# Chain123/RecGURU

Hardware: AMD Instinct MI355X
Metric: user-sequences/sec (AE+GAN step) (higher is better)
Workload: dtype bf16; 1 GPU; cross-domain RecGURU AE+GAN phase-2 iteration (5 critic + 1 generator update), two 100000-item domains; per_gpu_batch=4096, seq_len=200, d_model=128, n_head=4, n_blocks=3, d_ff=512, n_negs=30, user_lengths=U{5..220}, parallelism=dp1

## Files before the change

### include/recguru_hip.h

```cpp
#ifndef RECGURU_HIP_H
#define RECGURU_HIP_H
#include <stddef.h>
#include <stdint.h>
#ifdef __cplusplus
extern "C" {
#endif

#define RG_F32 0
#define RG_BF16 1
#define RG_X3 2

#define RG_ERR_INVALID (-1)
#define RG_ERR_UNSUPPORTED (-2)
#define RG_ERR_HIP (-3)

const char* rg_last_error(void);
int rg_version(void);

int rg_det_enabled(void);
int rg_det_set_arenas(void* fbase0, void* sbase0, unsigned long long bytes0, int bits0,
                      void* fbase1, void* sbase1, unsigned long long bytes1, int bits1);
int rg_det_fault(int clear);

#define RG_PRO_NONE 0
#define RG_PRO_GELU 1

#define RG_EPI_NONE 0
#define RG_EPI_RELU 1
#define RG_EPI_MUL_POSMASK 2
#define RG_EPI_GELU_GRAD 3
#define RG_EPI_ADD 4
#define RG_EPI_RESID_LN 5
#define RG_EPI_DROP_GELU 6

typedef struct {
  const void* A; int lda;
  const void* W; int ldw;
  const float* bias;
  void* C; int ldc;
  int c_is_f32;
  int M, N, K;
  int prologue, epilogue;
  const void* aux; int ldaux;
  const float* gamma; const float* beta; const float* rowmask; float* rstd_out; float ln_eps;
  int debug_ablate;
  float epi_scale;
  float epi_nonzero_scale;
  float drop_p; unsigned long long drop_seed;
  const int* live16;
  int skip_dead_fill;
  int c_hm_L;
  void* C2;
  int w_packed;
} rg_gemm_nt_args;
int rg_gemm_nt(const rg_gemm_nt_args* args , int dtype, void* stream);

typedef struct {
  const void* Y; int ldy;
  const void* X; int ldx;
  float* dW; int lddw;
  float* colsum;
  int T, N1, N2;
  int prologue_x;
  float scale;
  int splits;
  int use_tr;
  const int* live16;
  float* partials;
  int colsum_T;
} rg_gemm_tn_args;
int rg_gemm_tn(const rg_gemm_tn_args* args , int dtype, void* stream);
size_t rg_gemm_tn_workspace(const rg_gemm_tn_args* args , int dtype);
int rg_gemm_tn_layer_supported(const rg_gemm_tn_args* p , const int* wgs , int dtype);
size_t rg_gemm_tn_layer_workspace(int slot, int wgs);
int rg_gemm_tn_layer(const rg_gemm_tn_args* p , const int* wgs , int dtype, void* stream);
int rg_gemm_nt_plan(const rg_gemm_nt_args* args , int dtype, char* name, int cap);
int rg_gemm_tn_plan(const rg_gemm_tn_args* args , int dtype, char* name, int cap);


typedef struct {
  const void* qkv;
  const int64_t* key_ids; int64_t pad_value; int causal;
  void* ctx; float* lse;
  int B, L, H, dk;
  float scale;
  float drop_p; unsigned long long seed;
  const float* rowmask;
  const void* x; const void* wqkv; const float* bqkv; int d;
  int x_masked;
  const int* first_live;
  int qkv_hm;
  const void* pad_rows;
} rg_attn_args;
int rg_attn_fwd(const rg_attn_args* args , int dtype, void* stream);
int rg_attn_fwd_x_supported(int d, int dtype, float drop_p);

typedef struct {
  const void* qkv; const void* dctx; const void* ctx; const float* lse;
  const int64_t* key_ids; int64_t pad_value; int causal;
  void* dqkv;
  int B, L, H, dk;
  float scale;
  float drop_p; unsigned long long seed;
  const float* rowmask;
  const float* bqkv; int x_masked;
  const int* first_live;
  int qkv_hm;
} rg_attn_bwd_args;
int rg_attn_bwd(const rg_attn_bwd_args* args , int dtype, void* stream);

int rg_embed_pe_fwd(const void* table, const float* pe, const int64_t* ids, const float* mask, void* out,
                    long long ntok, int L, int d, float drop_p, unsigned long long seed, int dtype, void* stream);
int rg_embed_pe_fwd_rows(const void* table, long long table_rows, const float* pe, const int64_t* ids, const float* mask, void* out,
                         long long ntok, int L, int d, float drop_p, unsigned long long seed, int dtype, void* stream);
int rg_embed_pe_fwd2(const void* table, const float* pe, const int64_t* ids, const float* mask, void* out, void* out2,
                     long long ntok, int L, int d, float drop_p, unsigned long long seed, int dtype, void* stream);
int rg_embed_pe_fwd_split(const float* table_f32, const float* pe, const int64_t* ids, const float* mask, void* out,
                          void* out_lo, long long ntok, int L, int d, float drop_p, unsigned long long seed, void* stream);
int rg_embed_scatter_bwd(const void* dx, const int64_t* ids, const float* mask, float* dE, long long ntok, int d,
                         long long skip_row, float drop_p, unsigned long long seed, int dtype, void* stream);
size_t rg_embed_scatter_binned_workspace(long long ntok, int d, long long table_rows);
int rg_embed_scatter_bwd_binned(const void* dx, const int64_t* ids, const float* mask, float* dE, long long ntok, int d,
                                long long table_rows, long long skip_row, float drop_p, unsigned long long seed,
                                void* workspace, size_t workspace_bytes, int dtype, void* stream);

typedef struct {
  const void* dy; const void* y; const float* rstd; const float* gamma; const float* beta;
  const float* rowmask;
  void* dz; float* dgamma; float* dbeta;
  long long M; int N; int ld;
  void* dz_drop; float drop_p; unsigned long long drop_seed;
  const int* live16;
  float* dz_colsum;
  float* partials;
} rg_ln_bwd_args;
int rg_ln_bwd(const rg_ln_bwd_args* args , int dtype, void* stream);
size_t rg_ln_bwd_workspace(long long M, int N);

int rg_bcast_add_ln(const void* x, const float* o, const float* gamma, const float* beta, void* y, float* rstd,
                    long long M, int L, int N, float eps, int dtype, void* stream);
int rg_seq_sum(const void* x, void* out , int B, int L, int N, int dtype, void* stream);
int rg_pad_mask(const int64_t* ids, int64_t pad, float* out, long long n, void* stream);
int rg_last_rows(const void* x, const float* rowmask, void* x_last, float* m_last, int B, int L, int d, int dtype, void* stream);

int rg_colsum(const void* x, const void* aux , const float* coef , float* out,
              long long M, int N, int ld, float scale, int dtype,
              void* stream);
int rg_outer_posmask(const float* coef , const float* w , const void* aux, void* out,
                     long long M, int N, float scale, int dtype,
                     void* stream);
typedef struct {
  const void* real; const void* fake;
  const float* alpha;
  const void *W1, *W2, *W3, *W1t, *W2t, *W3t;
  const float *b1, *b2, *b3, *w4, *b4;
  int B, d, n1, n2, n3;
  float drop_p;
  unsigned long long seed_w[3];
  unsigned long long seed_g[3];
  float coef_real, coef_fake;
  float gp_coef;
  float* out;
  float* scalars;
  void *Y1, *X1, *Y2, *X2, *Y3, *X3;
  float *db1, *db2, *db3, *dw4, *db4;
  void* dx;
  void* hscratch;
  int need_wgrad;
  int debug_ablate;
  long long* stamps;
} rg_disc_args;
int rg_disc_supported(int d, int n1, int n2, int n3, int dtype);
int rg_disc_rows(const rg_disc_args* args , int dtype, void* stream);
int rg_interpolate(const float* alpha, const void* real, const void* fake, void* out, long long B, int d,
                   int dtype, void* stream);
int rg_gp_penalty(const float* g, void* dg, float* gp, long long B, int d, float lambda, int dtype,
                  void* stream);
int rg_sum(const float* x, float* out, long long n, float scale, void* stream);

int rg_adam(float* p, const float* g, float* m, float* v, void* shadow, int shadow_dtype, long long n, float lr,
            float beta1, float beta2, float eps, int step, void* stream);
typedef struct {
  float* p; const float* g; float* m; float* v;
  long long n;
  float step_lr; float inv_bc2_sqrt;
} rg_adam_seg;
int rg_adam_multi(const rg_adam_seg* segs , int nsegs, float beta1, float beta2, float eps, void* stream);
typedef struct {
  float* p; const float* g; float* m; float* v;
  long long n;
  long long step;
} rg_adam_seg_dev;
int rg_adam_multi_dev(rg_adam_seg_dev* segs , int nsegs, double lr, double beta1, double beta2,
                      double eps, void* stream);
#define RG_CAST_TRANSPOSE 1
#define RG_CAST_PACK 2
#define RG_CAST_SPLIT 4
int rg_cast(const float* src, void* dst, int R, int C, int transpose, int dtype, void* stream);
typedef struct {
  const float* src; void* dst;
  int R, C, ld, row_off, col_off, transpose;
} rg_cast_seg;
int rg_cast_multi(const rg_cast_seg* segs , const int* tiles , int ntiles,
                  int dtype, void* stream);

#define RG_LOSS_SAMPLED_CE 0
#define RG_LOSS_BPR 1
#define RG_LOSS_BPR_SAS 2
typedef struct {
  const void* h;
  const void* table;
  const int64_t* pos;
  const int64_t* neg;
  const float* mask;
  float* aux_tok;
  float* sums;
  const float* gout;
  void* dh; float* dE;
  long long ntok; int d; int k; int mode; long long skip_row;
} rg_item_loss_args;
int rg_item_loss_fwd(const rg_item_loss_args* args , int dtype, void* stream);
int rg_item_loss_bwd(const rg_item_loss_args* args , int dtype, void* stream);
size_t rg_item_loss_bwd_binned_workspace(long long ntok, int k, int d, long long table_rows);
int rg_item_loss_bwd_binned(const rg_item_loss_args* args , long long table_rows, void* workspace,
                            size_t workspace_bytes, int dtype, void* stream);
int rg_item_loss_train_supported(int k, int d);
int rg_item_loss_train(const rg_item_loss_args* args , float* coef, int dtype, void* stream);
int rg_item_loss_scatter_binned(const rg_item_loss_args* args , const float* coef, long long table_rows,
// ... 135 lines not shown
```

### recguru_amd/csrc/fused.hip

```cpp
#include <type_traits>
#include "rg_common.hip.h"
#include "rg_det.hip.h"
#include "../../include/recguru_hip.h"

#define FT_M 64
#include <stdlib.h>
#define FD 128
#define FPAD 8
#define FLD (FD + FPAD)

template <typename T> struct Tile {
  static constexpr int LD = sizeof(T) == 2 ? FD : FLD;
  static __device__ __forceinline__ int off(int row, int col) {
    if constexpr (sizeof(T) == 2) return row * FD + ((((col >> 3) ^ row) & 15) << 3) + (col & 7);
    else return row * FLD + col;
  }
};
template <> struct Tile<x3r> {
  static constexpr int LD = FD;
  static __device__ __forceinline__ int off(int row, int col) { return row * FD + ((((col >> 3) ^ row) & 15) << 3) + (col & 7); }
};

template <typename T> struct WSet { typename OpT<T>::type f[4][2]; };

// ... 637 lines not shown
#pragma unroll
    for (int ct = 0; ct < 2; ++ct)
#pragma unroll
      for (int rt = 0; rt < RT; ++rt)
#pragma unroll
        for (int r = 0; r < 4; ++r) acc2[ct][rt][r] *= rm4[rt];
    regs_to_tile<XT>(acc2, Aout, n0, li, lg);
    if constexpr (RES) regs_to_tile_lo<LT>(acc2, Ag, n0, li, lg);
    STAMP(9);
    lds_barrier();
    tile_to_hbm<T>(Aout, out, FD, 0, mb, a.M, tid);
    if constexpr (RES) tile_to_hbm<T>(Ag, outlo, FD, 0, mb, a.M, tid);
    lds_barrier();
    STAMP(10);
#pragma unroll
    for (int rt = 0; rt < RT; ++rt) mb[rt] = mbn[rt];
    have = have_next;
  }
  if (a.live16) {
    const int nrt = (a.M + 15) >> 4, ndead = nrt - a.live16[0];
    constexpr bool cross = CROSS;
    for (int j = RT * (int)blockIdx.x; j < ndead; j += RT * (int)gridDim.x) {
      int md[RT];
#pragma unroll
      for (int rt = 0; rt < RT; ++rt) md[rt] = j + rt < ndead ? a.live16[nrt - (j + rt)] * 16 : a.M;
      zero_to_hbm<T>(out, FD, 0, md, a.M, tid);
      if constexpr (RES) zero_to_hbm<T>(outlo, FD, 0, md, a.M, tid);
      if (a.skip_dead_saves) continue;
      if (ysave) zero_to_hbm<T>(ysave, FD, 0, md, a.M, tid);
      if (cross && y2save) zero_to_hbm<T>(y2save, FD, 0, md, a.M, tid);
      if (h1save)
        for (int ch = 0; ch < nchunk; ++ch) zero_to_hbm<T>(h1save, a.dff, ch * FD, md, a.M, tid);
      if (tid < FTM) {
        const int m = md[tid >> 4] + (tid & 15);
        if (m < a.M) {
          if (rstd1o) rstd1o[m] = 0.f;
          if (rstd2o) rstd2o[m] = 0.f;
          if (rstdco) rstdco[m] = 0.f;
        }
      }
    }
  }
#ifdef RG_STAMP
  if (a.rstd_c == nullptr && a.o_bcast == nullptr && a.y2_save != nullptr && (tid & 63) == 0) {
    unsigned long long* dbg = reinterpret_cast<unsigned long long*>(a.y2_save) + (size_t)(blockIdx.x * 4 + wave) * 12;
    for (int i = 0; i < 12; ++i) dbg[i] = tacc[i];
  }
#endif
}

static int act_tile_bytes(int dtype, int rows) {
  return dtype == RG_BF16 ? rows * FD * 2 : (dtype == RG_X3 ? rows * FD * 2 * 2 : rows * FLD * 4);
}

int rg_post_attn_fwd256(const rg_post_attn_args* a, int dtype, hipStream_t s);
int rg_post_attn_fwd_w8_try(const rg_post_attn_args* a, int dtype, hipStream_t s, int* rc);

extern "C" int rg_post_attn_fwd(const rg_post_attn_args* a, int dtype, void* stream) {
  if (!a || a->M <= 0) return 0;
  if (a->d == 256) return rg_post_attn_fwd256(a, dtype, (hipStream_t)stream);
  {
    int rc8 = 0;
    if (rg_post_attn_fwd_w8_try(a, dtype, (hipStream_t)stream, &rc8)) return rc8;
  }
  if (a->d != FD || a->P != FD || (a->dff % FD) != 0 || a->dff <= 0)
    return rg_set_error_msg(RG_ERR_UNSUPPORTED, "post_attn_fwd: needs d_model == n_heads*32 == 128 and d_ff % 128 == 0");
  if ((long long)a->M * a->dff * (dtype == RG_BF16 ? 2 : 4) >= (1ll << 32))
    return rg_set_error_msg(RG_ERR_UNSUPPORTED, "post_attn_fwd: M * d_ff * element size must be below 4 GiB (32-bit offsets)");
  if ((a->o_bcast || a->cross_s) && a->L <= 0) return rg_set_error_msg(RG_ERR_INVALID, "post_attn_fwd: cross stage needs L");
  if (a->cross_s && (!a->cross_oh || !a->cross_bo || a->H != 4)) return rg_set_error_msg(RG_ERR_INVALID, "post_attn_fwd: cross_s needs cross_oh, cross_bo, H == P / 32 == 4");
  hipStream_t s = (hipStream_t)stream;
  static const int x3_rt = [] { const char* e = getenv("RG_X3_PA_RT"); return (e && atoi(e) == 4) ? 4 : 2; }();
#ifdef RG_PA_RT2
  static const int rt_env = [] { const char* e = getenv("RG_PA_RT"); return e ? atoi(e) : 0; }();
  const int rt = dtype == RG_X3 ? x3_rt : (dtype != RG_BF16 ? 4 : (rt_env == 2 ? 2 : 4));
#else
  const int rt = dtype == RG_X3 ? x3_rt : 4;
#endif
  const int ftm = 16 * rt;
  const int ntiles = (a->M + ftm - 1) / ftm;
  const int act = act_tile_bytes(dtype, ftm);
  const int smem = 3 * act + (8 * FD + a->dff) * 4 + 2 * ftm * 4 * 4 + 64 * 4 + (a->h1_save ? act : 0);
  const int per_cu = (160 * 1024) / smem;
  const int cap_cu = dtype == RG_X3 ? 2 : 3;
  int grid = 256 * (per_cu < 1 ? 1 : (per_cu > cap_cu ? cap_cu : per_cu));
  if (grid > ntiles) grid = ntiles;
  const int dm = a->drop_p <= 0.f ? 0 : (a->drop_p == 0.5f ? 1 : 2);
  const bool cross = a->o_bcast || a->cross_s;
  const bool save = a->y_save || a->y2_save || a->h1_save || a->rstd1 || a->rstd2 || a->rstd_c;
  const bool res = a->x_lo || a->out_lo;
  if (res && (!a->x_lo || !a->out_lo || dtype != RG_BF16))
    return rg_set_error_msg(RG_ERR_INVALID, "post_attn_fwd: the split residual stream needs x_lo AND out_lo, bf16 tier");
  static const int pipe_on = [] { const char* e = getenv("RG_PA_PIPE"); return e ? atoi(e) : 0; }();
  if (pipe_on && dtype == RG_BF16 && !cross && !save && !res && a->dff >= 2 * FD) {
#define RG_PAP(DM)                                                                                                        \
  do {                                                                                                                    \
    hipFuncSetAttribute(reinterpret_cast<const void*>(post_attn_fwd_kernel<__bf16, DM, false, false, false, 4, true>), hipFuncAttributeMaxDynamicSharedMemorySize, smem); \
    hipLaunchKernelGGL((post_attn_fwd_kernel<__bf16, DM, false, false, false, 4, true>), dim3(grid), dim3(256), smem, s, *a); \
  } while (0)
    if (dm == 0) RG_PAP(0);
    else if (dm == 1) RG_PAP(1);
    else RG_PAP(2);
#undef RG_PAP
    RG_CHECK_LAUNCH();
    return 0;
  }
#define RG_PA4(T, DM, C, S, R, RTV)                                                                                       \
  do {                                                                                                                    \
    hipFuncSetAttribute(reinterpret_cast<const void*>(post_attn_fwd_kernel<T, DM, C, S, R, RTV>), hipFuncAttributeMaxDynamicSharedMemorySize, smem); \
    hipLaunchKernelGGL((post_attn_fwd_kernel<T, DM, C, S, R, RTV>), dim3(grid), dim3(256), smem, s, *a);                  \
  } while (0)
#ifdef RG_PA_RT2
#define RG_PA3(T, DM, C, S, R)                                                              \
  do {                                                                                      \
    if constexpr (sizeof(T) == 2 || std::is_same<T, x3>::value) { if (rt == 2) RG_PA4(T, DM, C, S, R, 2); else RG_PA4(T, DM, C, S, R, 4); } \
    else RG_PA4(T, DM, C, S, R, 4);                                                         \
  } while (0)
#else
#define RG_PA3(T, DM, C, S, R)                                                              \
  do {                                                                                      \
    if constexpr (std::is_same<T, x3>::value) { if (rt == 2) RG_PA4(T, DM, C, S, R, 2); else RG_PA4(T, DM, C, S, R, 4); } \
    else RG_PA4(T, DM, C, S, R, 4);                                                         \
  } while (0)
#endif
#define RG_PA2(T, DM, C, S)                                                                       \
  do {                                                                                            \
    if constexpr (sizeof(T) == 2) { if (res) RG_PA3(T, DM, C, S, true); else RG_PA3(T, DM, C, S, false); } \
    else RG_PA3(T, DM, C, S, false);                                                              \
  } while (0)
#define RG_PA(T, DM)                                  \
  do {                                                \
    if (cross) { if (save) RG_PA2(T, DM, true, true); else RG_PA2(T, DM, true, false); }      \
    else { if (save) RG_PA2(T, DM, false, true); else RG_PA2(T, DM, false, false); }          \
  } while (0)
#define RG_PA_T(T)                   \
  do {                               \
    if (dm == 0) RG_PA(T, 0);        \
    else if (dm == 1) RG_PA(T, 1);   \
    else RG_PA(T, 2);                \
  } while (0)
  if (dtype == RG_BF16) RG_PA_T(__bf16);
  else if (dtype == RG_F32) RG_PA_T(float);
  else if (dtype == RG_X3) RG_PA_T(x3);
  else return rg_set_error_msg(RG_ERR_INVALID, "post_attn_fwd: bad dtype");
#undef RG_PA_T
#undef RG_PA
#undef RG_PA2
#undef RG_PA3
#undef RG_PA4
  RG_CHECK_LAUNCH();
  return 0;
}

template <typename T, bool LNF>
__global__ __launch_bounds__(256, (sizeof(T) == 2 ? 2 : 1)) void ffn_bwd_data_kernel(rg_ffn_bwd_args a) {
  constexpr int PL = FT_M * FD * 2;
  typedef typename LdsT<T, PL>::type LT;
  constexpr int ACT_BYTES = FT_M * Tile<LT>::LD * (int)sizeof(LT) * LdsT<T, PL>::PLANES;
  extern __shared__ __align__(16) unsigned char smem[];
  LT* Adl = reinterpret_cast<LT*>(smem);
  typedef typename ResT<T, PL>::type XT;
  XT* Adz = reinterpret_cast<XT*>(smem + ACT_BYTES);
  LT* Adh = reinterpret_cast<LT*>(smem + 2 * ACT_BYTES);
  XT* Ah = reinterpret_cast<XT*>(smem + 3 * ACT_BYTES);
  XT* Ady = reinterpret_cast<XT*>(smem);
  const int tid = threadIdx.x, lane = tid & 63, wave = __builtin_amdgcn_readfirstlane(tid >> 6);
  const int li = lane & 15, lg = lane >> 4;
  const T* __restrict__ dl2 = reinterpret_cast<const T*>(LNF ? a.ln_dout : a.dl2);
  const T* __restrict__ dz = reinterpret_cast<const T*>(LNF ? a.ln_out : a.dz);
  T* __restrict__ dl2o = reinterpret_cast<T*>(a.dl2_out);
  const T* __restrict__ h1 = reinterpret_cast<const T*>(a.h1);
  const T* __restrict__ W2t = reinterpret_cast<const T*>(a.W2t);
  const T* __restrict__ W1t = reinterpret_cast<const T*>(a.W1t);
  T* __restrict__ dh1 = reinterpret_cast<T*>(a.dh1);
  T* __restrict__ dy = reinterpret_cast<T*>(a.dy);
  const int n0 = wave * 32;
  const int ntiles = (a.M + FT_M - 1) / FT_M;
  const int nchunk = a.dff / FD;
  const float nz = a.nz_scale;

  WSet<T> wp, wq;
  Frag<T> cpre[4], xpre[4], hpre[4];
  float rs_pre[4], rm_pre[4];
  float dg[8], db[8];
  const DropCfg ldrop = make_drop(a.ln_drop_p, a.ln_drop_seed);
  float* lnp = reinterpret_cast<float*>(smem + 4 * ACT_BYTES);
  if constexpr (LNF) {
#pragma unroll
    for (int j = 0; j < 8; ++j) { dg[j] = 0.f; db[j] = 0.f; }
    for (int i = tid; i < FD; i += 256) { lnp[i] = a.ln_gamma[i]; lnp[FD + i] = a.ln_beta[i]; lnp[2 * FD + i] = 1.f / a.ln_gamma[i]; }
  }

  LiveWalk lw;
  lw.init(a.live16, a.M);
  const int nwork = a.live16 ? (lw.nlive + 3) >> 2 : ntiles;
  int cur = (int)blockIdx.x, kcur = 0;
  auto next_group = [&](int (&g)[4]) -> bool {
    if (cur >= nwork) {
#pragma unroll
      for (int rt = 0; rt < 4; ++rt) g[rt] = a.M;
      return false;
    }
    if (!a.live16) {
#pragma unroll
      for (int rt = 0; rt < 4; ++rt) g[rt] = cur * FT_M + 16 * rt;
    } else {
      lw.group(kcur, g, a.M);
    }
    cur += gridDim.x;
    ++kcur;
    return true;
  };
  auto prefetch_h = [&](const int (&g)[4], int ch) {
#pragma unroll
    for (int i = 0; i < 4; ++i) {
      const int c8 = (tid & 15) * 8, m = min(g[i] + (tid >> 4), a.M - 1);
      load_frag(hpre[i], gofs(h1, (unsigned int)m * (unsigned int)a.dff + (unsigned int)(ch * FD + c8)));
    }
  };
  auto prefetch_rows = [&](const int (&g)[4]) {
#pragma unroll
    for (int i = 0; i < 4; ++i) {
      const int c8 = (tid & 15) * 8, m = min(g[i] + (tid >> 4), a.M - 1);
      load_frag(cpre[i], gofs(dl2, (unsigned int)(m * FD + c8)));
      load_frag(xpre[i], gofs(dz, (unsigned int)(m * FD + c8)));
      if constexpr (LNF) {
        const float* __restrict__ rmp = a.ln_rowmask ? a.ln_rowmask : a.ln_rstd;
        const float rv = rmp[m];
        rs_pre[i] = a.ln_rstd[m];
        rm_pre[i] = a.ln_rowmask ? rv : 1.f;
      }
    }
  };
  auto h_to_lds = [&]() {
#pragma unroll
    for (int i = 0; i < 4; ++i) {
      const int c = tid + 256 * i, r = c >> 4, c8 = (c & 15) * 8;
      stage8(Ah + Tile<XT>::off(r, c8), hpre[i]);
    }
  };
  int mb[4], mbn[4];
  bool have = next_group(mb);
  if (have) {
    load_wset(wp, W2t, FD, n0, 0, li, lg, a.w_packed);
    prefetch_rows(mb);
    prefetch_h(mb, 0);
  }
  for (; have;) {
    const bool have_next = next_group(mbn);
    if constexpr (LNF) {
      const int c8 = (tid & 15) * 8;
      float gam[8], bet[8], igam[8];
      load8(gam, lnp + c8);
      load8(bet, lnp + FD + c8);
      load8(igam, lnp + 2 * FD + c8);
#pragma unroll
      for (int i = 0; i < 4; ++i) {
        const int r = 16 * i + (tid >> 4), m = mb[i] + (tid >> 4);
        const bool live = m < a.M;
        const float rm = live ? rm_pre[i] : 0.f;
        float g[8], xh[8], s1 = 0.f, s2 = 0.f;
        if (rm != 0.f) {
          const float irm = 1.f / rm;
#pragma unroll
          for (int j = 0; j < 8; ++j) {
            const float d = (float)cpre[i].v[j] * rm;
            xh[j] = ((float)xpre[i].v[j] * irm - bet[j]) * igam[j];
            g[j] = d * gam[j];
            dg[j] += d * xh[j];
            db[j] += d;
            s1 += g[j];
            s2 += g[j] * xh[j];
          }
        } else {
#pragma unroll
          for (int j = 0; j < 8; ++j) { g[j] = 0.f; xh[j] = 0.f; }
        }
#pragma unroll
        for (int o = 1; o < 16; o <<= 1) { s1 += __shfl_xor(s1, o); s2 += __shfl_xor(s2, o); }
        const float rstd = rm != 0.f ? rs_pre[i] : 0.f;
        s1 *= 1.f / FD;
        s2 *= 1.f / FD;
        float o8[8];
#pragma unroll
        for (int j = 0; j < 8; ++j) o8[j] = rstd * (g[j] - s1 - xh[j] * s2);
        store8(Adz + Tile<XT>::off(r, c8), o8);
        if (ldrop.thresh != 0u || ldrop.onebit) {
          float k8[8];
          rg_keep8(ldrop, (unsigned int)m * (unsigned int)FD + (unsigned int)c8, k8);
#pragma unroll
          for (int j = 0; j < 8; ++j) o8[j] *= k8[j];
        }
        store8(Adl + Tile<LT>::off(r, c8), o8);
        if (live) store8(gofs(dl2o, (unsigned int)(m * FD + c8)), o8);
      }
    } else {
#pragma unroll
      for (int i = 0; i < 4; ++i) {
        const int c = tid + 256 * i, r = c >> 4, c8 = (c & 15) * 8;
        stage8(Adl + Tile<LT>::off(r, c8), cpre[i]);
        stage8(Adz + Tile<XT>::off(r, c8), xpre[i]);
      }
    }
    h_to_lds();
    lds_barrier();
    f32x4 acc[2][4], acc2[2][4];
#pragma unroll
    for (int ct = 0; ct < 2; ++ct)
#pragma unroll
      for (int rt = 0; rt < 4; ++rt) acc2[ct][rt] = (f32x4){0.f, 0.f, 0.f, 0.f};
#pragma unroll 1
    for (int ch = 0; ch < nchunk; ++ch) {
      load_wset(wq, W1t, a.dff, n0, ch * FD, li, lg, a.w_packed);
      {
        const bool last = ch + 1 == nchunk;
        int gs[4];
#pragma unroll
        for (int rt = 0; rt < 4; ++rt) gs[rt] = last ? mbn[rt] : mb[rt];
        prefetch_h(gs, last ? 0 : ch + 1);
      }
#pragma unroll
      for (int ct = 0; ct < 2; ++ct)
#pragma unroll
        for (int rt = 0; rt < 4; ++rt) acc[ct][rt] = (f32x4){0.f, 0.f, 0.f, 0.f};
      mma_wset<T>(acc, wp, Adl, li, lg);
      load_wset(wp, W2t + (unsigned int)((ch + 1 < nchunk) ? ch + 1 : 0) * (FD * FD), FD, n0, 0, li, lg, a.w_packed);
      if (ch > 0) lds_barrier();
#pragma unroll
      for (int ct = 0; ct < 2; ++ct)
#pragma unroll
        for (int rt = 0; rt < 4; ++rt) {
          float x4[4];
          load4t(x4, Ah + Tile<XT>::off(rt * 16 + li, n0 + ct * 16 + 4 * lg));
#pragma unroll
          for (int r = 0; r < 4; ++r) {
            float v = acc[ct][rt][r] * gelu_grad_t<Precise<T>::value>(x4[r]);
            if (nz > 0.f) v = x4[r] != 0.f ? v * nz : 0.f;
            acc[ct][rt][r] = v;
          }
        }
      regs_to_tile<LT>(acc, Adh, n0, li, lg);
      lds_barrier();
      if (ch + 1 < nchunk) h_to_lds();
      tile_to_hbm<T>(Adh, dh1, a.dff, ch * FD, mb, a.M, tid);
      mma_wset<T>(acc2, wq, Adh, li, lg);
    }
    prefetch_rows(mbn);
#pragma unroll
    for (int ct = 0; ct < 2; ++ct)
#pragma unroll
      for (int rt = 0; rt < 4; ++rt) {
        float r4[4];
        load4t(r4, Adz + Tile<XT>::off(rt * 16 + li, n0 + ct * 16 + 4 * lg));
#pragma unroll
        for (int r = 0; r < 4; ++r) acc2[ct][rt][r] += r4[r];
      }
    regs_to_tile<XT>(acc2, Ady, n0, li, lg);
    lds_barrier();
    tile_to_hbm<T>(Ady, dy, FD, 0, mb, a.M, tid);
    lds_barrier();
#pragma unroll
    for (int rt = 0; rt < 4; ++rt) mb[rt] = mbn[rt];
    have = have_next;
  }
  if (a.live16) {
    const int nrt = (a.M + 15) >> 4, ndead = nrt - a.live16[0];
    for (int j = 4 * (int)blockIdx.x; j < ndead; j += 4 * (int)gridDim.x) {
      int md[4];
#pragma unroll
      for (int rt = 0; rt < 4; ++rt) md[rt] = j + rt < ndead ? a.live16[nrt - (j + rt)] * 16 : a.M;
      zero_to_hbm<T>(dy, FD, 0, md, a.M, tid);
    }
  }
  if constexpr (LNF) {
#pragma unroll
    for (int o = 16; o < 64; o <<= 1)
#pragma unroll
      for (int j = 0; j < 8; ++j) { dg[j] += __shfl_xor(dg[j], o); db[j] += __shfl_xor(db[j], o); }
    float* red = reinterpret_cast<float*>(smem);
    __syncthreads();
    if (lane < 16) {
#pragma unroll
      for (int j = 0; j < 8; ++j) { red[(0 * 4 + wave) * FD + lane * 8 + j] = dg[j]; red[(1 * 4 + wave) * FD + lane * 8 + j] = db[j]; }
    }
    __syncthreads();
    const int w = tid >> 7, n = tid & 127;
    a.ln_partials[((size_t)blockIdx.x * 2 + w) * FD + n] = (red[(w * 4 + 0) * FD + n] + red[(w * 4 + 1) * FD + n]) + (red[(w * 4 + 2) * FD + n] + red[(w * 4 + 3) * FD + n]);
  }
}

__global__ __launch_bounds__(256) void ffn_bwd_ln_reduce_kernel(const float* __restrict__ partials, int nblocks,
                                                                float* __restrict__ dgamma, float* __restrict__ dbeta) {
  const int c = threadIdx.x;
  float* dst = c < FD ? dgamma : dbeta;
  if (!dst) return;
  float s0 = 0.f, s1 = 0.f;
  int b = blockIdx.x;
  for (; b + (int)gridDim.x < nblocks; b += 2 * gridDim.x) {
    s0 += partials[(size_t)b * 2 * FD + c];
    s1 += partials[(size_t)(b + gridDim.x) * 2 * FD + c];
  }
  if (b < nblocks) s0 += partials[(size_t)b * 2 * FD + c];
  rg_acc(dst + (c & (FD - 1)), s0 + s1);
}

extern "C" int rg_ffn_bwd_data_supported(int d, int dff) { return d == FD && dff > 0 && (dff % FD) == 0; }

static int ffn_bwd_grid(int M, int dtype) {
  const int ntiles = (M + FT_M - 1) / FT_M;
  const int smem = 4 * act_tile_bytes(dtype, FT_M);
  const int per_cu = (160 * 1024) / smem;
  const int grid = 256 * (per_cu < 1 ? 1 : (per_cu > 2 ? 2 : per_cu));
  return grid > ntiles ? ntiles : grid;
}
extern "C" size_t rg_ffn_bwd_ln_workspace(int M) { return (size_t)(M <= 0 ? 0 : 512) * 2 * FD * sizeof(float); }

extern "C" int rg_ffn_bwd_data(const rg_ffn_bwd_args* a, int dtype, void* stream) {
  if (!a || a->M <= 0) return 0;
  if (!rg_ffn_bwd_data_supported(a->d, a->dff))
    return rg_set_error_msg(RG_ERR_UNSUPPORTED, "ffn_bwd_data: needs d_model == 128 and d_ff % 128 == 0");
  if ((long long)a->M * a->dff * (dtype == RG_BF16 ? 2 : 4) >= (1ll << 32))
    return rg_set_error_msg(RG_ERR_UNSUPPORTED, "ffn_bwd_data: M * d_ff * element size must be below 4 GiB (32-bit offsets)");
  const bool lnf = a->ln_dout != nullptr;
  if ((!lnf && (!a->dl2 || !a->dz)) || !a->h1 || !a->W2t || !a->W1t || !a->dh1 || !a->dy)
    return rg_set_error_msg(RG_ERR_INVALID, "ffn_bwd_data: NULL operand");
  if (lnf && (!a->ln_out || !a->ln_rstd || !a->ln_gamma || !a->ln_beta || !a->dl2_out || !a->ln_partials))
    return rg_set_error_msg(RG_ERR_INVALID, "ffn_bwd_data: the fused LayerNorm backward needs ln_out, ln_rstd, ln_gamma, ln_beta, dl2_out, ln_partials");
  hipStream_t s = (hipStream_t)stream;
  const int ntiles = (a->M + FT_M - 1) / FT_M;
  const int smem = 4 * act_tile_bytes(dtype, FT_M) + (lnf ? 3 * FD * 4 : 0);
  const int grid = ffn_bwd_grid(a->M, dtype);
#define RG_FB(T, L)                                                                                                       \
  do {                                                                                                                    \
    hipFuncSetAttribute(reinterpret_cast<const void*>(ffn_bwd_data_kernel<T, L>), hipFuncAttributeMaxDynamicSharedMemorySize, smem); \
    hipLaunchKernelGGL((ffn_bwd_data_kernel<T, L>), dim3(grid), dim3(256), smem, s, *a);                                  \
  } while (0)
  if (dtype == RG_BF16) { if (lnf) RG_FB(__bf16, true); else RG_FB(__bf16, false); }
  else if (dtype == RG_F32) { if (lnf) RG_FB(float, true); else RG_FB(float, false); }
  else if (dtype == RG_X3) { if (lnf) RG_FB(x3, true); else RG_FB(x3, false); }
  else return rg_set_error_msg(RG_ERR_INVALID, "ffn_bwd_data: bad dtype");
#undef RG_FB
  if (lnf && (a->ln_dgamma || a->ln_dbeta))
    hipLaunchKernelGGL(ffn_bwd_ln_reduce_kernel, dim3(grid < 32 ? grid : 32), dim3(256), 0, s, a->ln_partials, grid, a->ln_dgamma, a->ln_dbeta);
  RG_CHECK_LAUNCH();
  return 0;
}

template <typename T>
__global__ __launch_bounds__(256, 2) void attn_out_bwd_kernel(rg_attn_out_bwd_args a) {
  constexpr int PL = FT_M * FD * 2;
  typedef typename LdsT<T, PL>::type LT;
  constexpr int ACT_BYTES = FT_M * Tile<LT>::LD * (int)sizeof(LT) * LdsT<T, PL>::PLANES;
  extern __shared__ __align__(16) unsigned char smem[];
  LT* Adz = reinterpret_cast<LT*>(smem);
  typedef typename ResT<T, PL>::type XT;
  XT* Aout = reinterpret_cast<XT*>(smem + ACT_BYTES);
  float* lnp = reinterpret_cast<float*>(smem + 2 * ACT_BYTES);
  const int tid = threadIdx.x, lane = tid & 63, wave = __builtin_amdgcn_readfirstlane(tid >> 6);
  const int li = lane & 15, lg = lane >> 4;
  const T* __restrict__ dy = reinterpret_cast<const T*>(a.dy);
  const T* __restrict__ y = reinterpret_cast<const T*>(a.y);
  T* __restrict__ dz = reinterpret_cast<T*>(a.dz);
  T* __restrict__ dctx = reinterpret_cast<T*>(a.dctx);
  const int n0 = wave * 32;
  const int ntiles = (a.M + FT_M - 1) / FT_M;
  for (int i = tid; i < FD; i += 256) { lnp[i] = a.gamma[i]; lnp[FD + i] = a.beta[i]; lnp[2 * FD + i] = 1.f / a.gamma[i]; }
  WSet<T> w;
  load_wset(w, reinterpret_cast<const T*>(a.Wot), FD, n0, 0, li, lg, a.w_packed);
  Frag<T> cpre[4], xpre[4];
  float rs_pre[4], rm_pre[4];
  float dg[8], db[8];
#pragma unroll
  for (int j = 0; j < 8; ++j) { dg[j] = 0.f; db[j] = 0.f; }
  LiveWalk lw;
  lw.init(a.live16, a.M);
  const int nwork = a.live16 ? (lw.nlive + 3) >> 2 : ntiles;
  int cur = (int)blockIdx.x, kcur = 0;
  auto next_group = [&](int (&g)[4]) -> bool {
    if (cur >= nwork) {
#pragma unroll
      for (int rt = 0; rt < 4; ++rt) g[rt] = a.M;
      return false;
    }
    if (!a.live16) {
#pragma unroll
      for (int rt = 0; rt < 4; ++rt) g[rt] = cur * FT_M + 16 * rt;
    } else {
      lw.group(kcur, g, a.M);
    }
    cur += gridDim.x;
    ++kcur;
    return true;
  };
  auto prefetch_rows = [&](const int (&g)[4]) {
    const float* __restrict__ rmp = a.rowmask ? a.rowmask : a.rstd;
#pragma unroll
    for (int i = 0; i < 4; ++i) {
      const int c8 = (tid & 15) * 8, m = min(g[i] + (tid >> 4), a.M - 1);
      load_frag(cpre[i], gofs(dy, (unsigned int)(m * FD + c8)));
      load_frag(xpre[i], gofs(y, (unsigned int)(m * FD + c8)));
      const float rv = rmp[m];
      rs_pre[i] = a.rstd[m];
      rm_pre[i] = a.rowmask ? rv : 1.f;
    }
  };
  int mb[4], mbn[4];
  bool have = next_group(mb);
  if (have) prefetch_rows(mb);
  __syncthreads();
  for (; have;) {
    const bool have_next = next_group(mbn);
    {
      const int c8 = (tid & 15) * 8;
      float gam[8], bet[8], igam[8];
      load8(gam, lnp + c8);
      load8(bet, lnp + FD + c8);
      load8(igam, lnp + 2 * FD + c8);
#pragma unroll
      for (int i = 0; i < 4; ++i) {
        const int r = 16 * i + (tid >> 4), m = mb[i] + (tid >> 4);
        const bool live = m < a.M;
        const float rm = live ? rm_pre[i] : 0.f;
        float g[8], xh[8], s1 = 0.f, s2 = 0.f;
        if (rm != 0.f) {
          const float irm = 1.f / rm;
#pragma unroll
          for (int j = 0; j < 8; ++j) {
            const float d = (float)cpre[i].v[j] * rm;
            xh[j] = ((float)xpre[i].v[j] * irm - bet[j]) * igam[j];
            g[j] = d * gam[j];
            dg[j] += d * xh[j];
            db[j] += d;
            s1 += g[j];
            s2 += g[j] * xh[j];
          }
        } else {
#pragma unroll
          for (int j = 0; j < 8; ++j) { g[j] = 0.f; xh[j] = 0.f; }
        }
#pragma unroll
        for (int o = 1; o < 16; o <<= 1) { s1 += __shfl_xor(s1, o); s2 += __shfl_xor(s2, o); }
        const float rstd = rm != 0.f ? rs_pre[i] : 0.f;
        s1 *= 1.f / FD;
        s2 *= 1.f / FD;
        float o8[8];
#pragma unroll
        for (int j = 0; j < 8; ++j) o8[j] = rstd * (g[j] - s1 - xh[j] * s2);
        store8(Adz + Tile<LT>::off(r, c8), o8);
        if (live) store8(gofs(dz, (unsigned int)(m * FD + c8)), o8);
      }
    }
    prefetch_rows(mbn);
    lds_barrier();
    f32x4 acc[2][4];
#pragma unroll
    for (int ct = 0; ct < 2; ++ct)
#pragma unroll
      for (int rt = 0; rt < 4; ++rt) acc[ct][rt] = (f32x4){0.f, 0.f, 0.f, 0.f};
    mma_wset<T>(acc, w, Adz, li, lg);
    regs_to_tile<XT>(acc, Aout, n0, li, lg);
    lds_barrier();
    tile_to_hbm<T>(Aout, dctx, FD, 0, mb, a.M, tid);
#pragma unroll
    for (int rt = 0; rt < 4; ++rt) mb[rt] = mbn[rt];
    have = have_next;
  }
#pragma unroll
  for (int o = 16; o < 64; o <<= 1)
#pragma unroll
    for (int j = 0; j < 8; ++j) { dg[j] += __shfl_xor(dg[j], o); db[j] += __shfl_xor(db[j], o); }
  float* red = reinterpret_cast<float*>(smem);
  __syncthreads();
  if (lane < 16) {
#pragma unroll
    for (int j = 0; j < 8; ++j) { red[(0 * 4 + wave) * FD + lane * 8 + j] = dg[j]; red[(1 * 4 + wave) * FD + lane * 8 + j] = db[j]; }
  }
  __syncthreads();
  const int wsel = tid >> 7, n = tid & 127;
  a.ln_partials[((size_t)blockIdx.x * 2 + wsel) * FD + n] = (red[(wsel * 4 + 0) * FD + n] + red[(wsel * 4 + 1) * FD + n]) + (red[(wsel * 4 + 2) * FD + n] + red[(wsel * 4 + 3) * FD + n]);
}

static int attn_out_bwd_grid(int M) {
  const int ntiles = (M + FT_M - 1) / FT_M;
  return ntiles < 512 ? ntiles : 512;
}
extern "C" size_t rg_attn_out_bwd_workspace(int M) { return (size_t)(M <= 0 ? 0 : 1024) * 2 * FD * sizeof(float); }

extern "C" int rg_attn_out_bwd(const rg_attn_out_bwd_args* a, int dtype, void* stream) {
  if (!a || a->M <= 0) return 0;
  if (a->d != FD || a->P != FD) return rg_set_error_msg(RG_ERR_UNSUPPORTED, "attn_out_bwd: needs d_model == n_heads*32 == 128");
// ... 22 lines not shown
```

### recguru_amd/csrc/gemm_tn_big.hip

```cpp
#include <cstdlib>
#include <type_traits>
#include "rg_common.hip.h"
#include "rg_det.hip.h"
#include "../../include/recguru_hip.h"

#define TB_T_BF16 64
#define TB_T_X3 32

__device__ __forceinline__ void frag_tr16(Frag<__bf16>& f, const __bf16* tile, int ld, int c0, int li, int lg) {
  typedef __attribute__((ext_vector_type(4))) short s16x4;
  typedef __attribute__((address_space(3))) s16x4 lds_s16x4;
  const int q = li >> 2, p = li & 3;
  const __bf16* p0 = tile + (8 * lg + q) * ld + c0 + 4 * p;
  const __bf16* p1 = p0 + 4 * ld;
  union { s16x4 s; bf16x4_t b; } u0, u1;
  u0.s = __builtin_amdgcn_ds_read_tr16_b64_v4i16((lds_s16x4*)p0);
  u1.s = __builtin_amdgcn_ds_read_tr16_b64_v4i16((lds_s16x4*)p1);
#pragma unroll
  for (int j = 0; j < 4; ++j) { f.v[j] = u0.b[j]; f.v[4 + j] = u1.b[j]; }
}

__device__ __forceinline__ void frag_tr_op(Frag<__bf16>& f, const __bf16* tile, int ld, int c0, int li, int lg, int lo_ofs) {
  frag_tr16(f, tile, ld, c0, li, lg);
}
// ... 232 lines not shown
    __syncthreads();
  }
  auto bases = [&](int chunk, int (&bb)[EPC]) {
    if (a.live16) {
      const unsigned int ad = (unsigned int)(size_t)(lst + EPC * (chunk - c_beg));
      if constexpr (EPC == 2) {
        long long v;
        asm volatile("ds_read_b64 %0, %1\n\ts_waitcnt lgkmcnt(0)" : "=v"(v) : "v"(ad) : "memory");
        bb[0] = (int)(v & 0xFFFFFFFFll);
        bb[1] = (int)(v >> 32);
      } else {
        typedef __attribute__((ext_vector_type(4))) int i32x4;
        i32x4 v;
        asm volatile("ds_read_b128 %0, %1\n\ts_waitcnt lgkmcnt(0)" : "=v"(v) : "v"(ad) : "memory");
#pragma unroll
        for (int e = 0; e < EPC; ++e) bb[e] = v[e];
      }
    } else {
#pragma unroll
      for (int e = 0; e < EPC; ++e) bb[e] = chunk * CT + 16 * e;
    }
  };
  auto issue = [&](int chunk) {
    int bb[EPC];
    bases(chunk, bb);
    unsigned char* stage = smem_td + (chunk % NST) * STG;
#pragma unroll
    for (int k = 0; k < NPER; ++k) {
      const bool isy = k < KY;
      const unsigned int ld2 = (unsigned int)(isy ? a.ldy : a.ldx) * 2u;
      int bsel = bb[0];
#pragma unroll
      for (int e = 1; e < EPC; ++e) bsel = (srow[k] >> 4) == e ? bb[e] : bsel;
      const int row = min(bsel + (srow[k] & 15), a.T - 1);
      const char* src = (isy ? Y : X) + (size_t)(unsigned int)row * ld2 + scb[k];
      __builtin_amdgcn_global_load_lds((const __attribute__((address_space(1))) void*)src,
                                       (__attribute__((address_space(3))) void*)(stage + (isy ? 0 : C::YB) + (wave + 8 * (isy ? k : k - KY)) * 1024),
                                       16, 0, 0);
    }
  };

  f32x4 acc[MT][NT];
  f32x4 cs[MT];
#pragma unroll
  for (int i = 0; i < MT; ++i) {
    cs[i] = (f32x4){0.f, 0.f, 0.f, 0.f};
#pragma unroll
    for (int j = 0; j < NT; ++j) acc[i][j] = (f32x4){0.f, 0.f, 0.f, 0.f};
  }
  Frag<T> ones;
  frag_fill(ones, 1.f);
  const int q = li >> 2, pp = li & 3;
  const unsigned int smem0 = (unsigned int)(size_t)smem_td;
  const unsigned int ly0 = (unsigned int)((8 * lg + q) * (2 * N1) + ((pp >> 1) << 4) + (pp & 1) * 8);
  const unsigned int lx0 = (unsigned int)((8 * lg + q) * (2 * N2) + ((pp >> 1) << 4) + (pp & 1) * 8) + (unsigned int)C::YB;
  typedef long long i64;
  auto rd_y = [&](i64& lo, i64& hi, unsigned int stage_ofs, int ti) {
    const unsigned int ad = smem0 + stage_ofs + ly0 + (((unsigned int)ti ^ (unsigned int)q) << 5);
    asm volatile("ds_read_b64_tr_b16 %0, %2\n\tds_read_b64_tr_b16 %1, %2 offset:%3" : "=&v"(lo), "=&v"(hi) : "v"(ad), "n"(8 * N1) : "memory");
  };
  auto rd_x = [&](i64& lo, i64& hi, unsigned int stage_ofs, int ti) {
    const unsigned int ad = smem0 + stage_ofs + lx0 + (((unsigned int)ti ^ (unsigned int)q) << 5);
    asm volatile("ds_read_b64_tr_b16 %0, %2\n\tds_read_b64_tr_b16 %1, %2 offset:%3" : "=&v"(lo), "=&v"(hi) : "v"(ad), "n"(8 * N2) : "memory");
  };
  auto to_frag = [&](Frag<T>& f, i64 lo, i64 hi, bool gelu) {
    union { i64 l; bf16x4_t b; } u0, u1;
    u0.l = lo; u1.l = hi;
#pragma unroll
    for (int j = 0; j < 4; ++j) {
      f.v[j] = gelu ? (T)gelu_t<false>((float)u0.b[j]) : u0.b[j];
      f.v[4 + j] = gelu ? (T)gelu_t<false>((float)u1.b[j]) : u1.b[j];
    }
  };

#pragma unroll 1
  for (int c = c_beg; c < c_end && c < c_beg + NST - 1; ++c) issue(c);
#pragma unroll 1
  for (int chunk = c_beg; chunk < c_end; ++chunk) {
    wait_chunks<NPER, NST - 2>(min(NST - 2, c_end - 1 - chunk));
    lds_barrier();
    if (chunk + NST - 1 < c_end) issue(chunk + NST - 1);
    unsigned char* stage = smem_td + (chunk % NST) * STG;
    if (chunk == nchunks - 1) {
      int bb[EPC];
      bases(chunk, bb);
      bool partial = false;
#pragma unroll
      for (int e = 0; e < EPC; ++e) { bb[e] = __builtin_amdgcn_readfirstlane(bb[e]); partial = partial || bb[e] + 16 > a.T; }
      if (partial) {
        for (int i = tid; i < CT * N1 / 8; i += 512) {
          const int r = i / (N1 / 8);
          int bsel = bb[0];
#pragma unroll
          for (int e = 1; e < EPC; ++e) bsel = (r >> 4) == e ? bb[e] : bsel;
          const int row = bsel + (r & 15);
          if (row >= a.T) *reinterpret_cast<uint4*>(stage + i * 16) = make_uint4(0u, 0u, 0u, 0u);
        }
        lds_barrier();
      }
    }
    const unsigned int sofs0 = (unsigned int)((chunk % NST) * STG);
#pragma unroll
    for (int ks = 0; ks < KS; ++ks) {
    i64 ya[MT][2], xb[NT][2];
#pragma unroll
    for (int i = 0; i < MT; ++i) rd_y(ya[i][0], ya[i][1], sofs0 + ks * 32 * 2 * N1, (m1 >> 4) + i);
    rd_x(xb[0][0], xb[0][1], sofs0 + ks * 32 * 2 * N2, m2 >> 4);
    Frag<T> af[MT];
#pragma unroll
    for (int j = 0; j < NT; ++j) {
      if (j + 1 < NT) {
        rd_x(xb[j + 1][0], xb[j + 1][1], sofs0 + ks * 32 * 2 * N2, (m2 >> 4) + j + 1);
        asm volatile("s_waitcnt lgkmcnt(2)" : "+v"(xb[j][0]), "+v"(xb[j][1]));
      } else {
        asm volatile("s_waitcnt lgkmcnt(0)" : "+v"(xb[j][0]), "+v"(xb[j][1]));
      }
      if (j == 0) {
#pragma unroll
        for (int i = 0; i < MT; ++i) {
          asm volatile("" : "+v"(ya[i][0]), "+v"(ya[i][1]));
          to_frag(af[i], ya[i][0], ya[i][1], false);
          if (do_cs) mma(af[i], ones, cs[i]);
        }
      }
      Frag<T> bf;
      to_frag(bf, xb[j][0], xb[j][1], GELU_X);
#pragma unroll
      for (int i = 0; i < MT; ++i) mma(af[i], bf, acc[i][j]);
    }
    }
  }
  float* __restrict__ part = a.partials ? a.partials + (size_t)bid * (N1 * N2) + tid : nullptr;
#pragma unroll
  for (int i = 0; i < MT; ++i) {
#pragma unroll
    for (int j = 0; j < NT; ++j)
#pragma unroll
      for (int r = 0; r < 4; ++r) {
        if (part) part[((i * NT + j) * 4 + r) * 512] = acc[i][j][r];
        else rg_acc(a.dW + (size_t)(m1 + i * 16 + 4 * lg + r) * a.lddw + m2 + j * 16 + li, acc[i][j][r] * a.scale);
      }
    if (do_cs && li == 0) {
#pragma unroll
      for (int r = 0; r < 4; ++r) rg_acc(a.colsum + m1 + i * 16 + 4 * lg + r, cs[i][r] * a.scale);
    }
  }
}

template <int N1, int N2, bool GELU_X>
__global__ __launch_bounds__(512) void gemm_tn_dma_kernel(rg_gemm_tn_args a) {
  tn_dma_body<N1, N2, GELU_X>(a, (int)blockIdx.x, (int)gridDim.x);
}

struct rg_tn_layer_args {
  rg_gemm_tn_args p[4];
  int end[4];
};
__global__ __launch_bounds__(512) void gemm_tn_layer_x3_kernel(rg_tn_layer_args m) {
  const int bid = (int)blockIdx.x;
  if (bid < m.end[0]) tn_big_body<x3, 128, 512, true>(m.p[0], bid, m.end[0]);
  else if (bid < m.end[1]) tn_big_body<x3, 512, 128, false>(m.p[1], bid - m.end[0], m.end[1] - m.end[0]);
  else if (bid < m.end[2]) tn_big_body<x3, 384, 128, false>(m.p[2], bid - m.end[1], m.end[2] - m.end[1]);
  else tn_big_body<x3, 128, 128, false>(m.p[3], bid - m.end[2], m.end[3] - m.end[2]);
}
__global__ __launch_bounds__(512) void gemm_tn_layer_kernel(rg_tn_layer_args m) {
  const int bid = (int)blockIdx.x;
  if (bid < m.end[0]) tn_dma_body<128, 512, true>(m.p[0], bid, m.end[0]);
  else if (bid < m.end[1]) tn_dma_body<512, 128, false>(m.p[1], bid - m.end[0], m.end[1] - m.end[0]);
  else if (bid < m.end[2]) tn_dma_body<384, 128, false>(m.p[2], bid - m.end[1], m.end[2] - m.end[1]);
  else tn_dma_body<128, 128, false>(m.p[3], bid - m.end[2], m.end[3] - m.end[2]);
}

template <int N1, int N2>
__device__ __forceinline__ void tn_reduce_body(const rg_gemm_tn_args& a, int grid1, int ct, const int bx, const int by, const int ny) {
  constexpr bool SPLIT1 = N1 >= N2;
  constexpr int NT = SPLIT1 ? N2 / 16 : N2 / 128;
  const int nchunks = a.live16 ? (a.live16[0] + ct / 16 - 1) / (ct / 16) : (a.T + ct - 1) / ct;
  if (nchunks <= 0) return;
  const int per = (nchunks + grid1 - 1) / grid1;
  const int nact = (nchunks + per - 1) / per;
  const int e = bx * 256 + threadIdx.x;
  const int b0 = (int)((long long)nact * by / ny), b1 = (int)((long long)nact * (by + 1) / ny);
  const float* __restrict__ p = a.partials + e;
  float s0 = 0.f, s1 = 0.f, s2 = 0.f, s3 = 0.f;
  int b = b0;
  for (; b + 4 <= b1; b += 4) {
    s0 += p[(size_t)b * (N1 * N2)];
    s1 += p[(size_t)(b + 1) * (N1 * N2)];
    s2 += p[(size_t)(b + 2) * (N1 * N2)];
    s3 += p[(size_t)(b + 3) * (N1 * N2)];
  }
  for (; b < b1; ++b) s0 += p[(size_t)b * (N1 * N2)];
  const int tid = e & 511, slot = e >> 9, r = slot & 3, j = (slot >> 2) % NT, i = (slot >> 2) / NT;
  const int wave = tid >> 6, li = tid & 15, lg = (tid >> 4) & 3;
  constexpr int MT = SPLIT1 ? N1 / 128 : N1 / 16;
  const int m1 = SPLIT1 ? wave * MT * 16 : 0, m2 = SPLIT1 ? 0 : wave * NT * 16;
  rg_acc(a.dW + (size_t)(m1 + i * 16 + 4 * lg + r) * a.lddw + m2 + j * 16 + li, ((s0 + s1) + (s2 + s3)) * a.scale);
}

template <int N1, int N2>
__global__ __launch_bounds__(256) void tn_big_reduce_kernel(rg_gemm_tn_args a, int grid1, int ct) {
  tn_reduce_body<N1, N2>(a, grid1, ct, (int)blockIdx.x, (int)blockIdx.y, (int)gridDim.y);
}
struct rg_tn_layer_reduce_args {
  rg_gemm_tn_args p[4];
  int grid1[4], ct[4], gx[4], gy[4], end[4];
};
__global__ __launch_bounds__(256) void tn_layer_reduce_kernel(rg_tn_layer_reduce_args m) {
  const int bid = (int)blockIdx.x;
  const int i = (bid >= m.end[0]) + (bid >= m.end[1]) + (bid >= m.end[2]);
  const int r = bid - (i ? m.end[i - 1] : 0);
  const int bx = r % m.gx[i], by = r / m.gx[i];
  if (i == 0) tn_reduce_body<128, 512>(m.p[0], m.grid1[0], m.ct[0], bx, by, m.gy[0]);
  else if (i == 1) tn_reduce_body<512, 128>(m.p[1], m.grid1[1], m.ct[1], bx, by, m.gy[1]);
  else if (i == 2) tn_reduce_body<384, 128>(m.p[2], m.grid1[2], m.ct[2], bx, by, m.gy[2]);
  else tn_reduce_body<128, 128>(m.p[3], m.grid1[3], m.ct[3], bx, by, m.gy[3]);
}

static int tn_use_dma() {
  static int v = -1;
  if (v < 0) { const char* e = getenv("RG_TN_REGSTAGE"); v = (e && e[0] == '1') ? 0 : 1; }
  return v;
}

template <int N1, int N2, typename T = __bf16>
static int launch_big(const rg_gemm_tn_args& a, hipStream_t s) {
  constexpr bool X3 = std::is_same<T, x3>::value;
  const bool dma = !X3 && tn_use_dma() != 0 && (long long)TnDma<N1, N2>::NST * TnDma<N1, N2>::STG + ((a.T + 31) / 32 / 256 + 2) * 8 <= 160 * 1024;
  const int ct = dma ? TnDma<N1, N2>::CT : (X3 ? TB_T_X3 : TB_T_BF16);
  const int nchunks = (a.T + ct - 1) / ct;
  static const int grid_cap = [] { const char* e = getenv("RG_TN_GRID"); const int v = e ? atoi(e) : 0; return v > 0 && v <= 256 ? v : 192; }();
  int grid = nchunks < grid_cap ? nchunks : grid_cap;
  const int per = (nchunks + grid - 1) / grid;
  const int smem = dma ? TnDma<N1, N2>::NST * TnDma<N1, N2>::STG + (TnDma<N1, N2>::CT / 16) * per * 4
                       : (X3 ? TB_T_X3 * (N1 + 8 + N2 + 8) * 2 * 2 : TB_T_BF16 * (N1 + 8 + N2 + 8) * 2);
#define RG_TNB(KERN)                                                                                                     \
  do {                                                                                                                    \
    hipFuncSetAttribute(reinterpret_cast<const void*>(KERN), hipFuncAttributeMaxDynamicSharedMemorySize, smem);           \
    hipLaunchKernelGGL((KERN), dim3(grid), dim3(512), smem, s, a);                                                        \
  } while (0)
  if constexpr (X3) {
    if (a.prologue_x == RG_PRO_GELU) RG_TNB((gemm_tn_big_kernel<T, N1, N2, true>));
    else RG_TNB((gemm_tn_big_kernel<T, N1, N2, false>));
  } else if (a.prologue_x == RG_PRO_GELU) {
    if (dma) RG_TNB((gemm_tn_dma_kernel<N1, N2, true>));
    else RG_TNB((gemm_tn_big_kernel<T, N1, N2, true>));
  } else {
    if (dma) RG_TNB((gemm_tn_dma_kernel<N1, N2, false>));
    else RG_TNB((gemm_tn_big_kernel<T, N1, N2, false>));
  }
#undef RG_TNB
  if (a.partials) {
    const int gx = N1 * N2 / 256;
    const int gy = gx >= 256 ? 4 : (gx >= 128 ? 8 : 16);
    hipLaunchKernelGGL((tn_big_reduce_kernel<N1, N2>), dim3(gx, gy), dim3(256), 0, s, a, grid, ct);
  }
  RG_CHECK_LAUNCH();
  return 0;
}

static bool tn_native(int N1, int N2) {
  return (N2 == 128 && (N1 == 512 || N1 == 384 || N1 == 256 || N1 == 128)) || (N1 == 128 && N2 == 512);
}

static bool tn_blocks(int N1, int N2, int* b1, int* b2) {
  if (tn_native(N1, N2)) { *b1 = N1; *b2 = N2; return true; }
  if ((N1 & 127) || (N2 & 127) || N1 > 1024 || N2 > 512) return false;
  if (N2 == 512 && N1 <= 512) { *b1 = 128; *b2 = 512; return true; }
  *b2 = 128;
  *b1 = (N1 % 512 == 0) ? 512 : (N1 % 384 == 0) ? 384 : (N1 % 256 == 0) ? 256 : 128;
  return true;
}

int rg_gemm_tn_big_select(const rg_gemm_tn_args* a, int dtype) {
  if ((dtype != RG_BF16 && dtype != RG_X3) || !a->use_tr || a->T < 8192 || (a->ldy & 7) || (a->ldx & 7) || a->colsum_T > 0) return 0;
  int b1, b2;
  return tn_blocks(a->N1, a->N2, &b1, &b2) ? 1 : 0;
}

const char* rg_gemm_tn_big_name(const rg_gemm_tn_args* a) {
  const bool fits = (long long)3 * 40 * 1024 + ((a->T + 31) / 32 / 256 + 2) * 8 <= 160 * 1024;
  return tn_use_dma() && fits ? "gemm_tn_dma_kernel" : "gemm_tn_big_kernel";
}

size_t rg_gemm_tn_big_workspace(const rg_gemm_tn_args* a, int dtype) {
  if (!rg_gemm_tn_big_select(a, dtype)) return 0;
  int b1, b2;
  tn_blocks(a->N1, a->N2, &b1, &b2);
  return (size_t)256 * b1 * b2 * sizeof(float);
}

static int tn_big_native(const rg_gemm_tn_args* a, int dtype, hipStream_t s);

int rg_gemm_tn_big_try(const rg_gemm_tn_args* a, int dtype, hipStream_t s) {
  if (!rg_gemm_tn_big_select(a, dtype)) return 1;
  int b1, b2;
  tn_blocks(a->N1, a->N2, &b1, &b2);
  if (b1 == a->N1 && b2 == a->N2) return tn_big_native(a, dtype, s);
  const size_t esz = dtype == RG_BF16 ? 2 : 4;
  for (int i = 0; i < a->N1 / b1; ++i)
    for (int j = 0; j < a->N2 / b2; ++j) {
      rg_gemm_tn_args t = *a;
      t.Y = (const char*)a->Y + (size_t)i * b1 * esz;
      t.X = (const char*)a->X + (size_t)j * b2 * esz;
      t.dW = a->dW + (size_t)i * b1 * a->lddw + (size_t)j * b2;
      t.colsum = (a->colsum && j == 0) ? a->colsum + (size_t)i * b1 : nullptr;
      t.N1 = b1;
      t.N2 = b2;
      const int rc = tn_big_native(&t, dtype, s);
      if (rc) return rc < 0 ? rc : rg_set_error_msg(RG_ERR_INVALID, "gemm_tn: block launch refused");
    }
  return 0;
}

static int tn_big_native(const rg_gemm_tn_args* a, int dtype, hipStream_t s) {
  if (dtype == RG_X3) {
    if (a->N1 == 512 && a->N2 == 128) return launch_big<512, 128, x3>(*a, s);
    if (a->N1 == 128 && a->N2 == 512) return launch_big<128, 512, x3>(*a, s);
    if (a->N1 == 384 && a->N2 == 128) return launch_big<384, 128, x3>(*a, s);
    if (a->N1 == 256 && a->N2 == 128) return launch_big<256, 128, x3>(*a, s);
    if (a->N1 == 128 && a->N2 == 128) return launch_big<128, 128, x3>(*a, s);
    return 1;
  }
  if (a->N1 == 512 && a->N2 == 128) return launch_big<512, 128>(*a, s);
  if (a->N1 == 128 && a->N2 == 512) return launch_big<128, 512>(*a, s);
  if (a->N1 == 384 && a->N2 == 128) return launch_big<384, 128>(*a, s);
  if (a->N1 == 256 && a->N2 == 128) return launch_big<256, 128>(*a, s);
  if (a->N1 == 128 && a->N2 == 128) return launch_big<128, 128>(*a, s);
  return 1;
}

static const int LAYER_N1[4] = {128, 512, 384, 128}, LAYER_N2[4] = {512, 128, 128, 128};

static int layer_ct(int i, int dtype = RG_BF16) { return dtype == RG_X3 ? TB_T_X3 : i == 3 ? TnDma<128, 128>::CT : (i == 2 ? TnDma<384, 128>::CT : (i == 1 ? TnDma<512, 128>::CT : TnDma<128, 512>::CT)); }
static int layer_ring(int i) {
  return i == 3 ? TnDma<128, 128>::NST * TnDma<128, 128>::STG : (i == 2 ? TnDma<384, 128>::NST * TnDma<384, 128>::STG :
         (i == 1 ? TnDma<512, 128>::NST * TnDma<512, 128>::STG : TnDma<128, 512>::NST * TnDma<128, 512>::STG));
}
static int layer_lds(const rg_gemm_tn_args& a, int i, int g, int dtype) {
  if (dtype == RG_X3) return TB_T_X3 * (a.N1 + 8 + a.N2 + 8) * 2 * 2;
  const int ct = layer_ct(i), nchunks = (a.T + ct - 1) / ct;
  if (g > nchunks) g = nchunks;
  const int per = (nchunks + g - 1) / g;
  return layer_ring(i) + (ct / 16) * per * 4;
}

extern "C" int rg_gemm_tn_layer_supported(const rg_gemm_tn_args* p, const int* wgs, int dtype) {
  if (!p || !wgs || (dtype != RG_BF16 && dtype != RG_X3) || (dtype == RG_BF16 && !tn_use_dma())) return 0;
  int tot = 0;
  for (int i = 0; i < 4; ++i) {
    const rg_gemm_tn_args& a = p[i];
    if (a.T == 0) continue;
    if (a.N1 != LAYER_N1[i] || a.N2 != LAYER_N2[i] || (a.prologue_x == RG_PRO_GELU) != (i == 0)) return 0;
    if (!rg_gemm_tn_big_select(&a, dtype) || !a.partials || !a.Y || !a.X || !a.dW || wgs[i] <= 0) return 0;
    if (layer_lds(a, i, wgs[i], dtype) > 160 * 1024) return 0;
    tot += wgs[i];
  }
  return tot <= 256;
}

extern "C" size_t rg_gemm_tn_layer_workspace(int slot, int wgs) { return (size_t)wgs * LAYER_N1[slot] * LAYER_N2[slot] * sizeof(float); }

extern "C" int rg_gemm_tn_layer(const rg_gemm_tn_args* p, const int* wgs, int dtype, void* stream) {
  if (!rg_gemm_tn_layer_supported(p, wgs, dtype)) return rg_set_error_msg(RG_ERR_UNSUPPORTED, "gemm_tn_layer: needs the bf16 / bf16x3 tier and the four layer "
                                                                     "shapes (128x512 gelu, 512x128, 384x128, 128x128; T >= 8192; partials)");
  hipStream_t s = (hipStream_t)stream;
  rg_tn_layer_args m;
  rg_tn_layer_reduce_args r;
  int tot = 0, rtot = 0, smem = 0;
  for (int i = 0; i < 4; ++i) {
    m.p[i] = p[i];
    r.p[i] = p[i];
    const int ct = layer_ct(i, dtype);
    int g = p[i].T > 0 ? wgs[i] : 0;
    if (p[i].T > 0) {
      const int nchunks = (p[i].T + ct - 1) / ct;
      if (g > nchunks) g = nchunks;
      const int need = layer_lds(p[i], i, g, dtype);
      if (need > smem) smem = need;
    }
    tot += g;
    m.end[i] = tot;
    r.grid1[i] = g;
    r.ct[i] = ct;
    r.gx[i] = LAYER_N1[i] * LAYER_N2[i] / 256;
    r.gy[i] = g == 0 ? 0 : (r.gx[i] >= 256 ? 4 : (r.gx[i] >= 128 ? 8 : 16));
    rtot += r.gx[i] * r.gy[i];
    r.end[i] = rtot;
  }
  if (tot == 0) return 0;
  if (tot > 256 || smem > 160 * 1024) return rg_set_error_msg(RG_ERR_INVALID, "gemm_tn_layer: more than 256 workgroups, or a token range too long for the list slice in LDS");
  if (dtype == RG_X3) {
    hipFuncSetAttribute(reinterpret_cast<const void*>(gemm_tn_layer_x3_kernel), hipFuncAttributeMaxDynamicSharedMemorySize, smem);
    hipLaunchKernelGGL(gemm_tn_layer_x3_kernel, dim3(tot), dim3(512), smem, s, m);
  } else {
    hipFuncSetAttribute(reinterpret_cast<const void*>(gemm_tn_layer_kernel), hipFuncAttributeMaxDynamicSharedMemorySize, smem);
    hipLaunchKernelGGL(gemm_tn_layer_kernel, dim3(tot), dim3(512), smem, s, m);
  }
  hipLaunchKernelGGL(tn_layer_reduce_kernel, dim3(rtot), dim3(256), 0, s, r);
  RG_CHECK_LAUNCH();
  return 0;
}
```

### recguru_amd/hip.py

```python
import ctypes
import os

import torch

_HERE = os.path.dirname(os.path.abspath(__file__))
DETERMINISTIC = os.environ.get("RG_DETERMINISTIC", "0") not in ("", "0")
LIB_PATH = os.environ.get("RG_HIP_LIB") or os.path.join(_HERE, "librecguru_hip_det.so" if DETERMINISTIC else "librecguru_hip.so")
_lib = None

F32, BF16, X3 = 0, 1, 2
SPLIT_OPERANDS = False
PRO_NONE, PRO_GELU = 0, 1
EPI_NONE, EPI_RELU, EPI_MUL_POSMASK, EPI_GELU_GRAD, EPI_ADD, EPI_RESID_LN, EPI_DROP_GELU = 0, 1, 2, 3, 4, 5, 6

c_p, c_i, c_f, c_l = ctypes.c_void_p, ctypes.c_int, ctypes.c_float, ctypes.c_int64
c_u64 = ctypes.c_uint64


class GemmNtArgs(ctypes.Structure):
    _fields_ = [("A", c_p), ("lda", c_i), ("W", c_p), ("ldw", c_i), ("bias", c_p), ("C", c_p), ("ldc", c_i),
                ("c_is_f32", c_i), ("M", c_i), ("N", c_i), ("K", c_i), ("prologue", c_i), ("epilogue", c_i),
                ("aux", c_p), ("ldaux", c_i), ("gamma", c_p), ("beta", c_p), ("rowmask", c_p),
                ("rstd_out", c_p), ("ln_eps", c_f), ("debug_ablate", c_i), ("epi_scale", c_f),
                ("epi_nonzero_scale", c_f), ("drop_p", c_f), ("drop_seed", c_u64), ("live16", c_p),
                ("skip_dead_fill", c_i), ("c_hm_L", c_i), ("C2", c_p), ("w_packed", c_i)]


class GemmTnArgs(ctypes.Structure):
    _fields_ = [("Y", c_p), ("ldy", c_i), ("X", c_p), ("ldx", c_i), ("dW", c_p), ("lddw", c_i), ("colsum", c_p),
                ("T", c_i), ("N1", c_i), ("N2", c_i), ("prologue_x", c_i), ("scale", c_f), ("splits", c_i),
                ("use_tr", c_i), ("live16", c_p), ("partials", c_p), ("colsum_T", c_i)]


class AttnArgs(ctypes.Structure):
    _fields_ = [("qkv", c_p), ("key_ids", c_p), ("pad_value", c_l), ("causal", c_i), ("ctx", c_p), ("lse", c_p),
                ("B", c_i), ("L", c_i), ("H", c_i), ("dk", c_i), ("scale", c_f), ("drop_p", c_f), ("seed", c_u64), ("rowmask", c_p),
                ("x", c_p), ("wqkv", c_p), ("bqkv", c_p), ("d", c_i), ("x_masked", c_i), ("first_live", c_p),
                ("qkv_hm", c_i), ("pad_rows", c_p)]


class AttnBwdArgs(ctypes.Structure):
    _fields_ = [("qkv", c_p), ("dctx", c_p), ("ctx", c_p), ("lse", c_p), ("key_ids", c_p), ("pad_value", c_l),
                ("causal", c_i), ("dqkv", c_p), ("B", c_i), ("L", c_i), ("H", c_i), ("dk", c_i), ("scale", c_f),
                ("drop_p", c_f), ("seed", c_u64), ("rowmask", c_p), ("bqkv", c_p), ("x_masked", c_i), ("first_live", c_p),
                ("qkv_hm", c_i)]


class PostAttnArgs(ctypes.Structure):
    _fields_ = [("ctx", c_p), ("x", c_p), ("Wo", c_p), ("bo", c_p), ("g1", c_p), ("be1", c_p),
                ("o_bcast", c_p), ("gc", c_p), ("bec", c_p), ("L", c_i),
                ("W1", c_p), ("b1", c_p), ("W2", c_p), ("b2", c_p), ("g2", c_p), ("be2", c_p),
                ("rowmask", c_p), ("out", c_p),
                ("y_save", c_p), ("rstd1", c_p), ("y2_save", c_p), ("rstd_c", c_p), ("h1_save", c_p), ("rstd2", c_p),
                ("M", c_i), ("d", c_i), ("P", c_i), ("dff", c_i), ("eps", c_f),
                ("drop_p", c_f), ("seed_h1", c_u64), ("seed_out", c_u64),
                ("cross_s", c_p), ("cross_oh", c_p), ("cross_bo", c_p), ("H", c_i), ("live16", c_p),
                ("skip_dead_saves", c_i), ("w_packed", c_i), ("x_lo", c_p), ("out_lo", c_p)]


class FfnBwdArgs(ctypes.Structure):
    _fields_ = [("dl2", c_p), ("dz", c_p), ("h1", c_p), ("W2t", c_p), ("W1t", c_p), ("dh1", c_p), ("dy", c_p),
                ("M", c_i), ("d", c_i), ("dff", c_i), ("w_packed", c_i), ("nz_scale", c_f), ("live16", c_p),
                ("ln_dout", c_p), ("ln_out", c_p), ("ln_rstd", c_p), ("ln_gamma", c_p), ("ln_beta", c_p), ("ln_rowmask", c_p),
                ("dl2_out", c_p), ("ln_dgamma", c_p), ("ln_dbeta", c_p), ("ln_partials", c_p),
                ("ln_drop_p", c_f), ("ln_drop_seed", c_u64)]


class AttnOutBwdArgs(ctypes.Structure):
    _fields_ = [("dy", c_p), ("y", c_p), ("rstd", c_p), ("gamma", c_p), ("beta", c_p), ("rowmask", c_p), ("Wot", c_p),
                ("dz", c_p), ("dctx", c_p), ("dgamma", c_p), ("dbeta", c_p), ("ln_partials", c_p),
                ("M", c_i), ("d", c_i), ("P", c_i), ("w_packed", c_i), ("live16", c_p)]


SYMBOLS = ["rg_last_error", "rg_version", "rg_gemm_nt", "rg_gemm_tn", "rg_attn_fwd", "rg_attn_bwd",
           "rg_embed_pe_fwd", "rg_embed_pe_fwd_rows", "rg_embed_scatter_bwd", "rg_ln_bwd", "rg_bcast_add_ln", "rg_seq_sum", "rg_colsum",
           "rg_outer_posmask", "rg_interpolate", "rg_gp_penalty", "rg_sum", "rg_adam", "rg_cast",
           "rg_item_loss_fwd", "rg_item_loss_bwd", "rg_post_attn_fwd",
           "rg_attn_lastq_fwd", "rg_attn_lastq_bwd",
           "rg_cross_drop_scale", "rg_seq_wsum", "rg_gemm_nt_plan", "rg_gemm_tn_plan", "rg_gemm_tn_workspace", "rg_gemm_tn_layer", "rg_gemm_tn_layer_supported", "rg_gemm_tn_layer_workspace", "rg_ln_bwd_workspace", "rg_cast_multi",
           "rg_item_loss_bwd_binned_workspace", "rg_item_loss_bwd_binned", "rg_adam_multi", "rg_rank_scores",
           "rg_assemble_batch", "rg_sample_negatives", "rg_sample_negatives_alias", "rg_dropout", "rg_cross_rows", "rg_live_tiles",
           "rg_adam_multi_dev", "rg_disc_rows", "rg_disc_supported", "rg_attn_fwd_x_supported", "rg_pad_mask", "rg_last_rows",
           "rg_ffn_bwd_data", "rg_ffn_bwd_data_supported", "rg_ffn_bwd_ln_workspace", "rg_first_live",
           "rg_attn_out_bwd", "rg_attn_out_bwd_workspace",
           "rg_item_loss_train_supported", "rg_item_loss_train", "rg_item_loss_scatter_binned", "rg_scale_dev",
           "rg_attn_lastq_x_supported", "rg_attn_lastq_x_fwd", "rg_attn_lastq_x_bwd", "rg_attn_lastq_xf_fwd", "rg_attn_lastq_xf_bwd",
           "rg_embed_scatter_binned_workspace", "rg_embed_scatter_bwd_binned", "rg_embed_pe_fwd_split", "rg_mse",
           "rg_dropout_gelu", "rg_add_drop_ln", "rg_cross_add_ln", "rg_embed_pe_fwd2",
           "rg_det_enabled", "rg_det_set_arenas", "rg_det_fault",
           "rg_full_ce_supported", "rg_full_ce_fwd", "rg_full_ce_dw"]
LOSS_SAMPLED_CE, LOSS_BPR, LOSS_BPR_SAS = 0, 1, 2
c_ll = ctypes.c_longlong


class LnBwdArgs(ctypes.Structure):
    _fields_ = [("dy", c_p), ("y", c_p), ("rstd", c_p), ("gamma", c_p), ("beta", c_p), ("rowmask", c_p),
                ("dz", c_p), ("dgamma", c_p), ("dbeta", c_p), ("M", c_ll), ("N", c_i), ("ld", c_i),
                ("dz_drop", c_p), ("drop_p", c_f), ("drop_seed", c_u64), ("live16", c_p), ("dz_colsum", c_p), ("partials", c_p)]


class ItemLossArgs(ctypes.Structure):
    _fields_ = [("h", c_p), ("table", c_p), ("pos", c_p), ("neg", c_p), ("mask", c_p), ("aux_tok", c_p),
                ("sums", c_p), ("gout", c_p), ("dh", c_p), ("dE", c_p), ("ntok", c_ll), ("d", c_i), ("k", c_i),
                ("mode", c_i), ("skip_row", c_ll)]


def _check_screened(path):
    if os.environ.get("RG_ALLOW_UNSCREENED") or os.environ.get("RG_HIP_LIB"):
        return
    info_path = os.path.join(_HERE, "build", "BUILD_INFO_det.json" if os.path.basename(path) == "librecguru_hip_det.so" else "BUILD_INFO.json")
    try:
        import json
        with open(info_path) as f:
            info = json.load(f)
    except (OSError, ValueError):
        return
    import hashlib
    with open(path, "rb") as f:
        sha = hashlib.sha256(f.read()).hexdigest()
    if info.get("screen_bypassed") or info.get("library_sha256") != sha:
        raise RuntimeError("recguru_amd: %s is not the library the ISA screen passed (build/BUILD_INFO.json: %s) -- rebuild with "
                           "`python -m recguru_amd.build` (RG_ALLOW_UNSCREENED=1 loads it anyway)"
                           % (path, "screen bypassed" if info.get("screen_bypassed") else "hash mismatch"))


def lib():
    global _lib
    if _lib is None:
        if not os.path.exists(LIB_PATH):
            raise RuntimeError("recguru_amd: %s is missing -- run `python -m recguru_amd.build` "
                               "(there is no CPU fallback)" % LIB_PATH)
        _check_screened(LIB_PATH)
        _lib = ctypes.CDLL(LIB_PATH)
        _lib.rg_last_error.restype = ctypes.c_char_p
        for name in SYMBOLS:
            getattr(_lib, name)
    return _lib


def _check(rc, what):
    if rc != 0:
        raise RuntimeError("%s failed (%d): %s" % (what, rc, lib().rg_last_error().decode()))


def dt_of(t):
    if t.dtype == torch.float32:
        return F32
    if t.dtype == torch.bfloat16:
        return BF16
    raise TypeError("recguru_amd: activations must be float32 or bfloat16, got %s" % t.dtype)


def mt_of(t):
    d = dt_of(t)
    return X3 if (d == F32 and SPLIT_OPERANDS) else d


def _p(t):
    if t is None:
        return None
    if not t.is_cuda:
        raise RuntimeError("recguru_amd: tensor is not on the GPU (there is no CPU path)")
    return t.data_ptr()


def _stream():
    return ctypes.c_void_p(torch.cuda.current_stream().cuda_stream)


def _rowmajor(t):
    assert t.dim() == 2 and t.stride(1) == 1, "expected a row-major 2-D view"
    return t.stride(0)


DET_BITS = {"g": 46, "s": 30}


class _DetArena(object):
    _per_device = {}

    def __init__(self, dev):
        self.dev = dev
        self.top = {"g": 0, "s": 0}
        self.last_stream = None
        self.wrapped = torch.zeros((), device=dev, dtype=torch.int32)
        self.resize(int(os.environ.get("RG_DET_ARENA_MFLOATS", "32")) << 20)

    def resize(self, ng):
        assert self.top["g"] == 0 and self.top["s"] == 0
        torch.cuda.synchronize(self.dev)
        self.n = {"g": ng, "s": 4096}
        self.f = self.s = None
        self.f = {k: torch.zeros(n, device=self.dev, dtype=torch.float32) for k, n in self.n.items()}
        self.s = {k: torch.zeros(n, device=self.dev, dtype=torch.int64) for k, n in self.n.items()}
        fn = lib().rg_det_set_arenas
        fn.argtypes = [c_p, c_p, ctypes.c_ulonglong, c_i, c_p, c_p, ctypes.c_ulonglong, c_i]
        with torch.cuda.device(self.dev):
            _check(fn(self.f["g"].data_ptr(), self.s["g"].data_ptr(), self.n["g"] * 4, DET_BITS["g"],
                      self.f["s"].data_ptr(), self.s["s"].data_ptr(), self.n["s"] * 4, DET_BITS["s"]), "rg_det_set_arenas")

    @classmethod
    def all(cls):
        return list(cls._per_device.values())

    @classmethod
    def of(cls, dev):
        a = cls._per_device.get(dev.index)
        if a is None:
            if not lib().rg_det_enabled():
                raise RuntimeError("recguru_amd: RG_DETERMINISTIC needs librecguru_hip_det.so, %s is the float-atomic build" % LIB_PATH)
            a = cls._per_device[dev.index] = cls(dev)
        return a

    def holds(self, t):
        p = t.data_ptr()
        return any(f.data_ptr() <= p < f.data_ptr() + f.numel() * 4 for f in self.f.values())


class _DetScope(object):
    def __init__(self):
        self.arena, self.items, self.mark = None, [], None

    def take(self, t, kind="g", load=False):
        if t is None:
            return None
        assert t.dtype == torch.float32 and t.is_cuda
        if self.arena is None:
            self.arena = _DetArena.of(t.device)
            self.mark = dict(self.arena.top)
        a = self.arena
        if a.holds(t):
            return t
# ... 15 lines not shown
        self.items.append((t, kind, off, n, f))
        return f

    def commit(self):
        for t, kind, off, n, f in self.items:
            sh = self.arena.s[kind][off:off + n]
            self.arena.wrapped.add_((sh.abs() > (1 << 62)).any().to(torch.int32))
            t.add_(sh.to(torch.float64).mul_(2.0 ** -DET_BITS[kind]).to(torch.float32).view(t.shape))
        if self.arena is not None:
            self.arena.top.update(self.mark)
        self.items = []

    def back(self, r):
        if isinstance(r, torch.Tensor):
            for t, _, _, _, f in self.items:
                if r is f:
                    return t
            return r
        if isinstance(r, tuple):
            return tuple(self.back(x) for x in r)
        return r


def _det_accum(**spec):
    def deco(fn):
        if not DETERMINISTIC:
            return fn
        import functools
        import inspect
        sig = inspect.signature(fn)

        @functools.wraps(fn)
        def wrapped(*args, **kw):
            ba = sig.bind(*args, **kw)
            ba.apply_defaults()
            sc = _DetScope()
            for name, kind in spec.items():
                ba.arguments[name] = sc.take(ba.arguments.get(name), kind.lower(), load=kind == "S")
            try:
                r = fn(*ba.args, **ba.kwargs)
                r = sc.back(r)
            finally:
                sc.commit()
            return r
        return wrapped
    return deco


def det_fault(clear=True):
    torch.cuda.synchronize()
    v = int(lib().rg_det_fault(1 if clear else 0))
    for a in _DetArena.all():
        if int(a.wrapped.item()):
            v = max(v, 2)
            if clear:
                a.wrapped.zero_()
    return v


POISON_UNWRITTEN = False


def gemm_nt(A, W, bias=None, out=None, out_f32=False, prologue=PRO_NONE, epilogue=EPI_NONE, aux=None,
            gamma=None, beta=None, rowmask=None, rstd_out=None, eps=1e-8, debug_ablate=0, epi_scale=0.0,
            epi_nonzero_scale=0.0, drop_p=0.0, drop_seed=0, live=None, skip_dead_fill=False, headmajor_L=0, out2=None):
    M, K = A.shape
    N = W.shape[0]
    assert W.shape[1] == K and W.dtype == A.dtype
    if out is None:
        out = torch.empty(M, N, device=A.device, dtype=torch.float32 if out_f32 else A.dtype)
        if POISON_UNWRITTEN and live is not None and skip_dead_fill == 1:
            out.fill_(float("nan"))
    if M == 0:
        return out
    if headmajor_L:
        assert N % 384 == 0 and M % headmajor_L == 0 and out.is_contiguous() and not out_f32
    w_packed = 0
    if (PRESPLIT_WS_X3 and SPLIT_OPERANDS and A.dtype == torch.float32 and K == 256 and N % 128 == 0 and N <= 1024 and M >= 4096
            and prologue == PRO_NONE and epilogue != EPI_RESID_LN and not headmajor_L and not out_f32 and not (debug_ablate & 16)
            and not (epilogue == EPI_DROP_GELU and (out2 is None or aux is not None or live is not None))
            and (epilogue in (EPI_NONE, EPI_RELU, EPI_DROP_GELU) or aux is not None) and not (epilogue == EPI_RELU and drop_p > 0)):
        W = cast(W.contiguous(), torch.float32, transpose=CAST_PACK | CAST_SPLIT)
        w_packed = 1
    a = GemmNtArgs(_p(A), _rowmajor(A), _p(W), _rowmajor(W), _p(bias), _p(out), _rowmajor(out),
                   1 if out.dtype == torch.float32 else 0,
                   M, N, K, prologue, epilogue, _p(aux), _rowmajor(aux) if aux is not None else 0,
                   _p(gamma), _p(beta), _p(rowmask), _p(rstd_out), eps, debug_ablate, epi_scale, epi_nonzero_scale,
                   drop_p, drop_seed, _p(live), int(skip_dead_fill) if live is not None else 0, int(headmajor_L), _p(out2), w_packed)
    if _PROF is not None:
        _note_plan(lib().rg_gemm_nt_plan, a, mt_of(A))
    _check(lib().rg_gemm_nt(ctypes.byref(a), mt_of(A), _stream()), "rg_gemm_nt")
    if headmajor_L:
        return out.view(3, M // headmajor_L, N // 96, headmajor_L, 32)
    return out


_TN_WS = {}


def _tn_workspace(dev, nbytes, kind="tn"):
    key = (kind, dev.index, torch.cuda.current_stream(dev).cuda_stream)
    ws = _TN_WS.get(key)
    if ws is None or ws.numel() * 4 < nbytes:
        ws = torch.empty((nbytes + 3) // 4, device=dev, dtype=torch.float32)
        _TN_WS[key] = ws
    return ws


def gemm_tn(Y, X, dW=None, colsum=None, prologue_x=PRO_NONE, scale=1.0, splits=0, use_tr=1, live=None, partials=True,
            colsum_rows=0):
    if dW is None:
        dW = torch.zeros(Y.shape[1], X.shape[1], device=Y.device, dtype=torch.float32)
    return _gemm_tn(Y, X, dW, colsum, prologue_x, scale, splits, use_tr, live, partials, colsum_rows)


@_det_accum(dW="g", colsum="g")
def _gemm_tn(Y, X, dW, colsum, prologue_x, scale, splits, use_tr, live, partials, colsum_rows):
    T, N1 = Y.shape
    N2 = X.shape[1]
    assert X.shape[0] == T and X.dtype == Y.dtype
    if T == 0:
        return dW
    a = GemmTnArgs(_p(Y), _rowmajor(Y), _p(X), _rowmajor(X), _p(dW), _rowmajor(dW), _p(colsum), T, N1, N2,
                   prologue_x, scale, splits, use_tr, _p(live), None, int(colsum_rows))
    if partials:
        fn = lib().rg_gemm_tn_workspace
        fn.restype = ctypes.c_size_t
        need = int(fn(ctypes.byref(a), mt_of(Y)))
        if need:
            a.partials = _p(_tn_workspace(Y.device, need))
    if _PROF is not None:
        _note_plan(lib().rg_gemm_tn_plan, a, mt_of(Y))
    _check(lib().rg_gemm_tn(ctypes.byref(a), mt_of(Y), _stream()), "rg_gemm_tn")
    return dW


LAYER_SLOTS = ((128, 512, PRO_GELU), (512, 128, PRO_NONE), (384, 128, PRO_NONE), (128, 128, PRO_NONE))
LAYER_WGS = int(os.environ.get("RG_TN_LAYER_WGS", "256"))
_LC = os.environ.get("RG_TN_LAYER_COST")
LAYER_COST = {False: tuple(float(x) for x in (_LC or "1.45,1,1,1").split(",")),
              True: tuple(float(x) for x in (_LC or os.environ.get("RG_TN_LAYER_COST_X3", "1,1,1,1")).split(","))}


class _TnLayerArgs(ctypes.Structure):
    _fields_ = [("p", GemmTnArgs * 4)]


def gemm_tn_layer_slot(Y, X, prologue_x):
    key = (Y.shape[1], X.shape[1], prologue_x)
    ok = Y.dtype == torch.bfloat16 or (Y.dtype == torch.float32 and SPLIT_OPERANDS)
    return LAYER_SLOTS.index(key) if (key in LAYER_SLOTS and ok and Y.shape[0] >= 8192) else None


def gemm_tn_layer(probs):
    args = _TnLayerArgs()
    w = [0.0] * 4
    sc = _DetScope() if DETERMINISTIC else None
    for i, pr in enumerate(probs):
        if pr is None:
            continue
        Y, X, dW, colsum, live = pr
        if sc is not None:
            dW, colsum = sc.take(dW), sc.take(colsum)
        N1, N2, pro = LAYER_SLOTS[i]
        assert Y.shape[1] == N1 and X.shape == (Y.shape[0], N2) and Y.dtype == X.dtype
        args.p[i] = GemmTnArgs(_p(Y), _rowmajor(Y), _p(X), _rowmajor(X), _p(dW), _rowmajor(dW), _p(colsum), Y.shape[0], N1, N2,
                               pro, 1.0, 0, 1, _p(live), None, 0)
        w[i] = Y.shape[0] * (N1 + N2) * (0.6 if live is not None else 1.0) * LAYER_COST[Y.dtype == torch.float32][i]
    tot = sum(w)
    if tot == 0:
        return True
    wgs = [max(8, int(round(LAYER_WGS * x / tot))) if x > 0 else 0 for x in w]
    while sum(wgs) > LAYER_WGS:
        wgs[wgs.index(max(wgs))] -= 1
    fn = lib().rg_gemm_tn_layer_workspace
    fn.restype = ctypes.c_size_t
    need = [int(fn(i, wgs[i])) for i in range(4)]
    dev = next(pr[0].device for pr in probs if pr is not None)
    ws = _tn_workspace(dev, sum(need), "tn_layer")
    off = 0
    for i in range(4):
        if wgs[i]:
            args.p[i].partials = ws.data_ptr() + off
            off += need[i]
    dt = mt_of(next(pr[0] for pr in probs if pr is not None))
    cw = (ctypes.c_int * 4)(*wgs)
    if not lib().rg_gemm_tn_layer_supported(ctypes.byref(args), cw, dt):
        if sc is not None:
            sc.commit()
        return False
    try:
        _check(lib().rg_gemm_tn_layer(ctypes.byref(args), cw, dt, _stream()), "rg_gemm_tn_layer")
    finally:
        if sc is not None:
            sc.commit()
    return True


def attn_fwd(qkv, key_ids, pad_value, causal, H, need_lse=True, drop_p=0.0, seed=0, rowmask=None, x_masked=False, bqkv=None,
             pad_rows=None):
    hm = qkv.dim() == 5
    if hm:
        _, B, Hq, L, dk = qkv.shape
        assert Hq == H and dk == 32 and pad_rows is not None and pad_rows.shape == (3 * H + 1, 32) and pad_rows.dtype == qkv.dtype
        assert qkv.is_contiguous() and key_ids.dtype == torch.int64 and key_ids.is_contiguous()
    else:
        B, L, P3 = qkv.shape
        assert P3 == 3 * H * 32 and qkv.is_contiguous() and key_ids.dtype == torch.int64 and key_ids.is_contiguous()
    ctx = torch.empty(B, L, H * 32, device=qkv.device, dtype=qkv.dtype)
    lse = torch.empty(B, H, L, device=qkv.device, dtype=torch.float32) if need_lse else None
    a = AttnArgs(_p(qkv), _p(key_ids), int(pad_value), int(bool(causal)), _p(ctx), _p(lse), B, L, H, 32,
                 1.0 / (32 ** 0.5), drop_p, seed, _p(rowmask), None, None, _p(bqkv) if x_masked else None, 0,
                 (2 if bqkv is not None else 1) if (x_masked and rowmask is not None) else 0,
                 _p(first_live(rowmask, B, L)) if (x_masked and rowmask is not None and bqkv is not None) else None,
                 1 if hm else 0, _p(pad_rows) if hm else None)
    _check(lib().rg_attn_fwd(ctypes.byref(a), mt_of(qkv), _stream()), "rg_attn_fwd")
    return ctx, lse


def attn_fwd_x_supported(d, dtype, drop_p):
    return bool(lib().rg_attn_fwd_x_supported(int(d), BF16 if dtype == torch.bfloat16 else F32, c_f(drop_p)))


def attn_fwd_x(x, wqkv, bqkv, key_ids, pad_value, causal, H, drop_p=0.0, seed=0, rowmask=None, x_masked=False):
    B, L, d = x.shape
    assert x.is_contiguous() and wqkv.is_contiguous() and wqkv.shape == (3 * H * 32, d) and wqkv.dtype == x.dtype
    assert bqkv.dtype == torch.float32 and bqkv.numel() == 3 * H * 32 and key_ids.dtype == torch.int64 and key_ids.is_contiguous()
    ctx = torch.empty(B, L, H * 32, device=x.device, dtype=x.dtype)
    a = AttnArgs(None, _p(key_ids), int(pad_value), int(bool(causal)), _p(ctx), None, B, L, H, 32,
                 1.0 / (32 ** 0.5), drop_p, seed, _p(rowmask), _p(x), _p(wqkv), _p(bqkv), d, int(bool(x_masked)), None, 0, None)
    _check(lib().rg_attn_fwd(ctypes.byref(a), mt_of(x), _stream()), "rg_attn_fwd")
    return ctx


def attn_bwd(qkv, dctx, ctx, lse, key_ids, pad_value, causal, H, drop_p=0.0, seed=0, rowmask=None, bqkv=None):
    hm = qkv.dim() == 5
    B, L = (qkv.shape[1], qkv.shape[3]) if hm else qkv.shape[:2]
    assert dctx.is_contiguous() and ctx.is_contiguous() and qkv.is_contiguous()
    dqkv = torch.empty(B, L, 3 * H * 32, device=qkv.device, dtype=qkv.dtype)
    sub = bqkv is not None and rowmask is not None
    a = AttnBwdArgs(_p(qkv), _p(dctx), _p(ctx), _p(lse), _p(key_ids), int(pad_value), int(bool(causal)),
                    _p(dqkv), B, L, H, 32, 1.0 / (32 ** 0.5), drop_p, seed, _p(rowmask), _p(bqkv) if sub else None, 2 if sub else 0,
                    _p(first_live(rowmask, B, L)) if sub else None, 1 if hm else 0)
    _check(lib().rg_attn_bwd(ctypes.byref(a), mt_of(qkv), _stream()), "rg_attn_bwd")
    return dqkv


def _vp(t):
    return ctypes.c_void_p(_p(t))


def embed_pe_fwd(table, pe, ids, mask, L, drop_p=0.0, seed=0, mirror=False):
    ntok, d = ids.numel(), table.shape[1]
    assert ids.dtype == torch.int64 and ids.is_contiguous() and mask.dtype == torch.float32 and mask.numel() == ntok
    assert pe.dtype == torch.float32 and pe.shape[1] == d and pe.is_contiguous() and table.is_contiguous()
    out = torch.empty(ntok, d, device=table.device, dtype=table.dtype)
    if mirror:
        out2 = torch.empty(ntok, d, device=table.device, dtype=torch.bfloat16)
        _check(lib().rg_embed_pe_fwd2(_vp(table), _vp(pe), _vp(ids), _vp(mask), _vp(out), _vp(out2), c_ll(ntok), L, d, c_f(drop_p),
                                      c_u64(seed), dt_of(table), _stream()), "rg_embed_pe_fwd2")
        return out, out2
    _check(lib().rg_embed_pe_fwd_rows(_vp(table), c_ll(table.shape[0]), _vp(pe), _vp(ids), _vp(mask), _vp(out), c_ll(ntok), L, d, c_f(drop_p),
                                      c_u64(seed), dt_of(table), _stream()), "rg_embed_pe_fwd_rows")
    return out


def embed_pe_fwd_split(table_f32, pe, ids, mask, L, drop_p=0.0, seed=0):
    ntok, d = ids.numel(), table_f32.shape[1]
    assert ids.dtype == torch.int64 and ids.is_contiguous() and mask.dtype == torch.float32 and mask.numel() == ntok
    assert pe.dtype == torch.float32 and pe.shape[1] == d and pe.is_contiguous()
    assert table_f32.dtype == torch.float32 and table_f32.is_contiguous()
    out = torch.empty(ntok, d, device=table_f32.device, dtype=torch.bfloat16)
    lo = torch.empty_like(out)
    _check(lib().rg_embed_pe_fwd_split(_vp(table_f32), _vp(pe), _vp(ids), _vp(mask), _vp(out), _vp(lo), c_ll(ntok), L, d,
                                       c_f(drop_p), c_u64(seed), _stream()), "rg_embed_pe_fwd_split")
    return out, lo


@_det_accum(dE="g")
def embed_scatter_bwd(dx, ids, mask, dE, skip_row=-1, drop_p=0.0, seed=0):
    ntok, d = ids.numel(), dx.shape[-1]
    assert dx.is_contiguous() and dE.dtype == torch.float32 and dE.is_contiguous()
    _check(lib().rg_embed_scatter_bwd(_vp(dx), _vp(ids), _vp(mask), _vp(dE), c_ll(ntok), d, c_ll(skip_row),
                                      c_f(drop_p), c_u64(seed), dt_of(dx), _stream()), "rg_embed_scatter_bwd")
    return dE


def embed_scatter_binned_supported(ntok, d, table_rows):
    fn = lib().rg_embed_scatter_binned_workspace
    fn.restype = ctypes.c_size_t
    return int(fn(c_ll(ntok), int(d), c_ll(table_rows)))


def embed_scatter_bwd_binned(dx, ids, mask, dE, skip_row=-1, drop_p=0.0, seed=0):
    ntok, d = ids.numel(), dx.shape[-1]
    need = embed_scatter_binned_supported(ntok, d, dE.shape[0])
    if not need:
        raise RuntimeError("embed_scatter_bwd_binned: unsupported shape (d=%d, rows=%d)" % (d, dE.shape[0]))
    assert dx.is_contiguous() and dE.dtype == torch.float32 and dE.is_contiguous() and mask.dtype == torch.float32
    ws = _BIN_WS.get(dx.device)
    if ws is None or ws.numel() < need:
        ws = torch.empty(need, device=dx.device, dtype=torch.uint8)
        _BIN_WS[dx.device] = ws
    _check(lib().rg_embed_scatter_bwd_binned(_vp(dx), _vp(ids), _vp(mask), _vp(dE), c_ll(ntok), d, c_ll(dE.shape[0]),
                                             c_ll(skip_row), c_f(drop_p), c_u64(seed), _vp(ws), ctypes.c_size_t(need),
                                             dt_of(dx), _stream()), "rg_embed_scatter_bwd_binned")
    return dE


@_det_accum(dgamma="g", dbeta="g", dz_colsum="g")
def ln_bwd(dy, y, rstd, gamma, beta, rowmask, dgamma, dbeta, drop_p=0.0, drop_seed=0, live=None, dz_colsum=None):
    M, N = dy.shape
    assert dy.is_contiguous() and y.is_contiguous() and dy.dtype == y.dtype
    dz = torch.empty_like(dy)
    dzd = torch.empty_like(dy) if drop_p > 0 else None
    if POISON_UNWRITTEN and live is not None:
        dz.fill_(float("nan"))
        if dzd is not None:
            dzd.fill_(float("nan"))
    ws = None
    if M >= 4096 and (dgamma is not None or dbeta is not None or dz_colsum is not None):
        fn = lib().rg_ln_bwd_workspace
        fn.restype = ctypes.c_size_t
        ws = _tn_workspace(dy.device, int(fn(c_ll(M), N)), "ln")
    a = LnBwdArgs(_p(dy), _p(y), _p(rstd), _p(gamma), _p(beta), _p(rowmask), _p(dz), _p(dgamma), _p(dbeta), M, N, N,
                  _p(dzd), drop_p, drop_seed, _p(live), _p(dz_colsum), _p(ws))
    _check(lib().rg_ln_bwd(ctypes.byref(a), dt_of(dy), _stream()), "rg_ln_bwd")
    return (dz, dzd) if drop_p > 0 else dz


def bcast_add_ln(x, o, gamma, beta, L, eps=1e-8):
    M, N = x.shape
    assert x.is_contiguous() and o.dtype == torch.float32 and o.is_contiguous()
    y = torch.empty_like(x)
    rstd = torch.empty(M, device=x.device, dtype=torch.float32)
    _check(lib().rg_bcast_add_ln(_vp(x), _vp(o), _vp(gamma), _vp(beta), _vp(y), _vp(rstd), c_ll(M), L, N,
                                 c_f(eps), dt_of(x), _stream()), "rg_bcast_add_ln")
    return y, rstd


def dropout_(x, drop_p, seed):
    assert x.is_contiguous() and x.dim() == 2
    _check(lib().rg_dropout(_vp(x), c_ll(x.shape[0]), x.shape[1], c_f(drop_p), c_u64(seed), dt_of(x), _stream()), "rg_dropout")
    return x


def dropout_gelu(x, drop_p, seed):
    assert x.is_contiguous() and x.dim() == 2
    g = torch.empty_like(x)
# ... 424 lines not shown
                ("pad_value", ctypes.c_int64), ("first_live", c_p), ("ctx", c_p), ("dctx", c_p), ("dx", c_p), ("dq", c_p),
                ("ym_v", c_p), ("ym_q", c_p), ("xbar", c_p), ("dqp", c_p), ("dbv", c_p),
                ("B", c_i), ("L", c_i), ("scale", c_f), ("drop_p", c_f), ("seed", c_u64)]


def attn_lastq_x_supported(d, P, H, L, dtype):
    return bool(lib().rg_attn_lastq_x_supported(int(d), int(P), int(H), int(L), BF16 if dtype == torch.bfloat16 else F32))


def _lastq_x_args(x, q_last, wk, wv, bk, bv, key_ids, pad_value, drop_p, seed, rowmask):
    B, L, d = x.shape
    assert x.is_contiguous() and q_last.is_contiguous() and wk.is_contiguous() and wv.is_contiguous() and key_ids.is_contiguous()
    assert wk.dtype == x.dtype and wv.dtype == x.dtype and bk.dtype == torch.float32 and bv.dtype == torch.float32
    assert q_last.dtype == x.dtype and x.dtype in (torch.bfloat16, torch.float32)
    fl = first_live(rowmask, B, L) if rowmask is not None else None
    a = LastqXArgs(_p(x), _p(q_last), _p(wk), _p(wv), _p(bk), _p(bv), _p(key_ids), int(pad_value), _p(fl))
    a.B, a.L, a.scale, a.drop_p, a.seed = B, L, 32 ** -0.5, drop_p, seed
    return a, fl


def attn_lastq_x_fwd(x, q_last, wk, wv, bk, bv, key_ids, pad_value, drop_p=0.0, seed=0, rowmask=None):
    a, keep = _lastq_x_args(x, q_last, wk, wv, bk, bv, key_ids, pad_value, drop_p, seed, rowmask)
    ctx = torch.empty_like(q_last)
    a.ctx = _p(ctx)
    fn = lib().rg_attn_lastq_x_fwd if x.dtype == torch.bfloat16 else lib().rg_attn_lastq_xf_fwd
    _check(fn(ctypes.byref(a), _stream()), "rg_attn_lastq_x_fwd")
    return ctx


@_det_accum(dbv="g")
def attn_lastq_x_bwd(x, q_last, dctx, wk, wv, bk, bv, key_ids, pad_value, dbv, drop_p=0.0, seed=0, rowmask=None):
    a, keep = _lastq_x_args(x, q_last, wk, wv, bk, bv, key_ids, pad_value, drop_p, seed, rowmask)
    B, L, d = x.shape
    assert dctx.is_contiguous() and dctx.dtype == x.dtype and dbv.dtype == torch.float32
    dx = torch.empty_like(x)
    dq = torch.empty_like(q_last)
    ops4 = torch.empty(4, B * 4, d, device=x.device, dtype=x.dtype)
    a.dctx, a.dx, a.dq, a.dbv = _p(dctx), _p(dx), _p(dq), _p(dbv)
    a.ym_v, a.xbar, a.ym_q, a.dqp = _p(ops4[0]), _p(ops4[1]), _p(ops4[2]), _p(ops4[3])
    fn = lib().rg_attn_lastq_x_bwd if x.dtype == torch.bfloat16 else lib().rg_attn_lastq_xf_bwd
    _check(fn(ctypes.byref(a), _stream()), "rg_attn_lastq_x_bwd")
    return dx, dq, ops4[0], ops4[1], ops4[2], ops4[3]


PRESPLIT_WS_X3 = not os.environ.get("RG_NO_PRESPLIT_WS")
FUSE_BLOCK_256 = not os.environ.get("RG_NO_PA256")


def post_attn_supported(d, P, dff, dtype=None, M=None):
    if d == 128 and P == 128 and dff % 128 == 0 and dff > 0:
        return True
    if not (FUSE_BLOCK_256 and d == 256 and P == 256 and dff % 256 == 0 and dff > 0 and dtype == torch.bfloat16 and not SPLIT_OPERANDS):
        return False
    act = 64 * 256 * 2
    smem = 4 * act + (8 * 256 + dff) * 4 + 2 * 64 * 8 * 4 + 64 * 4
    return smem <= 160 * 1024 and (M is None or M * dff * 2 < (1 << 32))


_LIVE = {}
COMPACT_MIN_ROWS = 16384


def live_tiles(rowmask, M):
    key = (rowmask.data_ptr(), rowmask._version, M, rowmask.dtype)
    hit = _LIVE.get(key)
    if hit is not None:
        return hit[1]
    flags = torch.empty(1 + 2 * ((M + 15) // 16) + 4, device=rowmask.device, dtype=torch.int32)
    _check(lib().rg_live_tiles(_vp(rowmask), c_ll(M), _vp(flags), _stream()), "rg_live_tiles")
    if len(_LIVE) >= 32:
        _LIVE.pop(next(iter(_LIVE)))
    _LIVE[key] = (rowmask, flags)
    return flags


_FIRST = {}


def first_live(rowmask, B, L):
    key = (rowmask.data_ptr(), rowmask._version, B, L)
    hit = _FIRST.get(key)
    if hit is not None:
        return hit[1]
    out = torch.empty(B, device=rowmask.device, dtype=torch.int32)
    _check(lib().rg_first_live(_vp(rowmask), B, L, _vp(out), _stream()), "rg_first_live")
    if len(_FIRST) >= 32:
        _FIRST.pop(next(iter(_FIRST)))
    _FIRST[key] = (rowmask, out)
    return out


def post_attn_fwd(ctx, x, Wo, bo, g1, be1, W1, b1, W2, b2, g2, be2, rowmask, save=False, cross=None, L=0, eps=1e-8,
                  drop_p=0.0, seed_h1=0, seed_out=0, cross_drop=None, compact=True, skip_dead_saves=False, w_packed=False,
                  x_lo=None):
    M, P = ctx.shape
    d = x.shape[1]
    dff = W1.shape[0]
    dev = ctx.device
    live16 = None
    if rowmask is not None and M >= COMPACT_MIN_ROWS and compact:
        live16 = live_tiles(rowmask, M)
    out = torch.empty(M, d, device=dev, dtype=ctx.dtype)
    sv = {}
    if save:
        sv["y"] = torch.empty(M, d, device=dev, dtype=ctx.dtype)
        sv["rstd1"] = torch.empty(M, device=dev, dtype=torch.float32)
        sv["h1"] = torch.empty(M, dff, device=dev, dtype=ctx.dtype)
        sv["rstd2"] = torch.empty(M, device=dev, dtype=torch.float32)
        if cross is not None:
            sv["y2"] = torch.empty(M, d, device=dev, dtype=ctx.dtype)
            sv["rstd_c"] = torch.empty(M, device=dev, dtype=torch.float32)
        if POISON_UNWRITTEN and live16 is not None and skip_dead_saves:
            for t in sv.values():
                t.fill_(float("nan"))
    o, gc, bec = cross if cross is not None else (None, None, None)
    cs, coh, cbo, cH = cross_drop if cross_drop is not None else (None, None, None, 0)
    out_lo = None
    if x_lo is not None:
        assert x_lo.shape == x.shape and x_lo.dtype == x.dtype == torch.bfloat16 and x_lo.is_contiguous()
        out_lo = sv["out_lo"] = torch.empty_like(out)
    a = PostAttnArgs(_p(ctx), _p(x), _p(Wo), _p(bo), _p(g1), _p(be1), _p(o), _p(gc), _p(bec), L,
                     _p(W1), _p(b1), _p(W2), _p(b2), _p(g2), _p(be2), _p(rowmask), _p(out),
                     _p(sv.get("y")), _p(sv.get("rstd1")), _p(sv.get("y2")), _p(sv.get("rstd_c")), _p(sv.get("h1")),
                     _p(sv.get("rstd2")), M, d, P, dff, eps, drop_p, seed_h1, seed_out, _p(cs), _p(coh), _p(cbo), cH,
                     _p(live16), 1 if (live16 is not None and skip_dead_saves) else 0, 1 if w_packed else 0,
                     _p(x_lo), _p(out_lo))
    _check(lib().rg_post_attn_fwd(ctypes.byref(a), mt_of(ctx), _stream()), "rg_post_attn_fwd")
    return out, sv


@_det_accum(dgamma="g", dbeta="g")
def attn_out_bwd(dy, y, rstd, gamma, beta, rowmask, dgamma, dbeta, Wot, live=None, w_packed=False):
    M, d = dy.shape
    P = d
    assert dy.is_contiguous() and y.is_contiguous() and dy.dtype == y.dtype
    dz = torch.empty_like(dy)
    dctx = torch.empty(M, P, device=dy.device, dtype=dy.dtype)
    if POISON_UNWRITTEN and live is not None:
        dz.fill_(float("nan"))
        dctx.fill_(float("nan"))
    fn = lib().rg_attn_out_bwd_workspace
    fn.restype = ctypes.c_size_t
    ws = _tn_workspace(dy.device, int(fn(M)), "attn_out_ln")
    a = AttnOutBwdArgs(_p(dy), _p(y), _p(rstd), _p(gamma), _p(beta), _p(rowmask), _p(Wot), _p(dz), _p(dctx),
                       _p(dgamma), _p(dbeta), _p(ws), M, d, P, 1 if w_packed else 0, _p(live))
    _check(lib().rg_attn_out_bwd(ctypes.byref(a), mt_of(dy), _stream()), "rg_attn_out_bwd")
    return dz, dctx


def ffn_bwd_data_supported(d, dff):
    return bool(lib().rg_ffn_bwd_data_supported(int(d), int(dff)))


def ffn_bwd_data(dl2, dz, h1, W2t, W1t, nz_scale=0.0, live=None, w_packed=False, ln=None):
    src = ln[0] if ln is not None else dl2
    M, d = src.shape
    dff = h1.shape[1]
    dh1 = torch.empty(M, dff, device=src.device, dtype=src.dtype)
    if POISON_UNWRITTEN and live is not None:
        dh1.fill_(float("nan"))
    dy = torch.empty(M, d, device=src.device, dtype=src.dtype)
    a = FfnBwdArgs(_p(dl2), _p(dz), _p(h1), _p(W2t), _p(W1t), _p(dh1), _p(dy), M, d, dff, 1 if w_packed else 0,
                   float(nz_scale), _p(live))
    dl2o, sc = None, None
    if ln is not None:
        dout, out, rstd, gamma, beta, rowmask, dgamma, dbeta, drop_p, drop_seed = ln
        if DETERMINISTIC:
            sc = _DetScope()
            dgamma, dbeta = sc.take(dgamma), sc.take(dbeta)
        assert dout.is_contiguous() and out.is_contiguous() and dout.dtype == out.dtype
        dl2o = torch.empty(M, d, device=src.device, dtype=src.dtype)
        if POISON_UNWRITTEN and live is not None:
            dl2o.fill_(float("nan"))
        fn = lib().rg_ffn_bwd_ln_workspace
        fn.restype = ctypes.c_size_t
        ws = _tn_workspace(src.device, int(fn(M)), "ffn_ln")
        a.ln_dout, a.ln_out, a.ln_rstd, a.ln_gamma, a.ln_beta, a.ln_rowmask = _p(dout), _p(out), _p(rstd), _p(gamma), _p(beta), _p(rowmask)
        a.dl2_out, a.ln_dgamma, a.ln_dbeta, a.ln_partials = _p(dl2o), _p(dgamma), _p(dbeta), _p(ws)
        a.ln_drop_p, a.ln_drop_seed = float(drop_p), int(drop_seed)
    try:
        _check(lib().rg_ffn_bwd_data(ctypes.byref(a), mt_of(src), _stream()), "rg_ffn_bwd_data")
    finally:
        if sc is not None:
            sc.commit()
    return (dh1, dy, dl2o) if ln is not None else (dh1, dy)


class Profiler(object):
    def __init__(self):
        self.records = []

    @staticmethod
    def _live_frac(ref, cache):
        if ref is None:
            return 1.0
        key = (ref.data_ptr(), ref.numel(), ref.dtype)
        if key not in cache:
            if ref.dtype == torch.int32:
                nt = (ref.numel() - 5) // 2
                cache[key] = float(ref[0]) / max(nt, 1)
            else:
                m = ref.reshape(-1)
                pad = (-m.numel()) % 16
                if pad:
                    m = torch.cat([m, m.new_zeros(pad)])
                cache[key] = float((m.view(-1, 16).abs().amax(1) > 0).float().mean())
        return cache[key]

    def summary(self):
        torch.cuda.synchronize()
        agg, cache = {}, {}
        for name, fl, by, e0, e1, ref in self.records:
            a = agg.setdefault(name, {"launches": 0, "ms": 0.0, "flops": 0.0, "bytes": 0.0, "flops_exec": 0.0, "bytes_exec": 0.0})
            a["launches"] += 1
            a["ms"] += e0.elapsed_time(e1)
            for f1, b1, r1 in (zip(fl, by, ref) if isinstance(fl, list) else ((fl, by, ref),)):
                a["flops"] += f1
                a["bytes"] += b1
                if isinstance(r1, tuple) and r1 and r1[0] == "exec":
                    a["flops_exec"] += r1[1]
                    a["bytes_exec"] += r1[2]
                    continue
                if isinstance(r1, tuple) and r1 and r1[0] == "exec_rows":
                    key = ("rows", r1[1].data_ptr(), r1[1].numel())
                    if key not in cache:
                        cache[key] = float((r1[1].reshape(-1) != 0).sum())
                    a["bytes_exec"] += cache[key] * r1[2] + r1[3]
                    continue
                lf = self._live_frac(r1, cache)
                a["flops_exec"] += f1 * lf
                a["bytes_exec"] += b1 * lf
        return agg


_PROF = None
_ORIG = {}
_PLAN_NAME = None


def _note_plan(fn, args, dtype):
    global _PLAN_NAME
    buf = ctypes.create_string_buffer(64)
    _check(fn(ctypes.byref(args), dtype, buf, 64), "rg_gemm_plan")
    _PLAN_NAME = buf.value.decode()


def _esize(t):
    return t.element_size()


def _tn(t):
    return "bf16" if t.dtype == torch.bfloat16 else ("x3" if SPLIT_OPERANDS else "f32")


def _work_gemm_nt(A, W, *a, **k):
    M, K = A.shape
    N = W.shape[0]
    epi = k.get("epilogue", EPI_NONE)
    ntw = (1 if N <= 64 else (2 if N <= 128 else 4)) if epi == EPI_RESID_LN else (1 if N <= 64 else 2)
    by = (M * K + N * K + M * N) * _esize(A) + (M * N * _esize(A) if k.get("aux") is not None else 0)
    return "gemm_nt_kernel<%s,%d>" % ("bf16" if A.dtype == torch.bfloat16 else "f32", ntw), 2.0 * M * N * K, by


def _work_gemm_tn(Y, X, *a, **k):
    T, N1 = Y.shape
    N2 = X.shape[1]
    return ("gemm_tn_kernel<%s>" % _tn(Y), 2.0 * T * N1 * N2,
            T * (N1 + N2) * _esize(Y) + N1 * N2 * 4)


def _work_attn_fwd(qkv, key_ids, pad_value, causal, H, *a, **k):
    if qkv.dim() == 5:
        B, L, P3 = qkv.shape[1], qkv.shape[3], 3 * qkv.shape[2] * 32
    else:
        B, L, P3 = qkv.shape
    return ("attn_fwd_kernel<%s>" % _tn(qkv), 4.0 * B * H * L * L * 32,
            B * L * (P3 + P3 // 3) * _esize(qkv))


def _work_attn_bwd(qkv, dctx, ctx, lse, key_ids, pad_value, causal, H, *a, **k):
    if qkv.dim() == 5:
        B, L, P3 = qkv.shape[1], qkv.shape[3], 3 * qkv.shape[2] * 32
    else:
        B, L, P3 = qkv.shape
    return ("attn_bwd_kernel<%s>" % _tn(qkv), 10.0 * B * H * L * L * 32,
            B * L * (2 * P3 + 2 * P3 // 3) * _esize(qkv))


def _work_embed_fwd(table, pe, ids, mask, L, *a, **k):
    n, d = ids.numel(), table.shape[1]
    es = _esize(table)
    return "embed_pe_fwd_kernel", 0.0, n * d * 2 * es + n * 12, ("exec_rows", mask, d * es, n * d * es + n * 12)


def _work_item_loss(h, table, pos, neg, mask, k, mode, *a, **kw):
    n, d = h.shape
    return "item_loss_kernel", 2.0 * n * (k + 1) * d, n * (k + 2) * d * _esize(table) + n * (k + 1) * 8


def _work_post_attn(ctx, x, Wo, bo, g1, be1, W1, *a, **k):
    M, P = ctx.shape
    d, dff = x.shape[1], W1.shape[0]
    by = M * (P + 2 * d) * _esize(ctx) + (M * (d + dff) * _esize(ctx) if k.get("save") else 0)
    return ("post_attn_fwd_kernel<%s>" % _tn(ctx),
            2.0 * M * (d * P + 2 * d * dff), by)


def _work_attn_fwd_x(x, wqkv, bqkv, key_ids, pad_value, causal, H, *a, **k):
    B, L, d = x.shape
    P3 = wqkv.shape[0]
    return ("attn_fwd_kernel<bf16,x-input>", 4.0 * B * H * L * L * 32 + 2.0 * B * L * d * P3,
            B * L * (d + P3 // 3) * _esize(x) + P3 * d * _esize(x))


def _work_ffn_bwd(dl2, dz, h1, *a, **k):
    src = k["ln"][0] if k.get("ln") is not None else dl2
    M, d = src.shape
    dff = h1.shape[1]
    return ("ffn_bwd_data_kernel<%s>" % _tn(src), 4.0 * M * d * dff,
            M * ((4 if k.get("ln") is not None else 3) * d + 2 * dff) * _esize(src))


def _work_lastq_x_fwd(x, q_last, *a, **k):
    B, L, d = x.shape
    return "attn_lastq_x_fwd_kernel", B * (4 * 2.0 * L * d * 2 + 4 * 2.0 * 32 * d * 2), B * L * d * _esize(x) + 2 * B * d * _esize(x)


def _work_lastq_x_bwd(x, q_last, *a, **k):
    B, L, d = x.shape
    return "attn_lastq_x_bwd_kernel", B * (4 * 2.0 * L * d * 5 + 4 * 2.0 * 32 * d * 3), 2 * B * L * d * _esize(x) + 11 * B * d * _esize(x)


def _work_item_loss_train(h, table, pos, neg, mask, k, mode, *a, **kw):
    n, d = h.shape
    nl = float(mask.sum())
    return ("item_loss_train_rows_kernel", 4.0 * nl * (k + 1) * d,
            nl * (k + 2) * d * _esize(table) + n * d * _esize(table) + nl * (k + 1) * 12 + n * 4)


def _work_item_loss_scatter(h, table_rows, pos, neg, mask, k, coef, gout, dE, *a, **kw):
    n, d = h.shape
    nl = float(mask.sum())
    pairs = nl * (k + 1)
    return "item_loss_scatter_binned_kernel", 2.0 * pairs * d, pairs * (d * _esize(h) + 2 * 12 + 2 * 8)


def _work_gemm_tn_layer(probs):
    fl, by, refs = [], [], []
    for i, pr in enumerate(probs):
        if pr is None:
            continue
        Y, X, dW, colsum, live = pr
        T, N1, N2 = Y.shape[0], Y.shape[1], X.shape[1]
        fl.append(2.0 * T * N1 * N2)
        by.append(T * (N1 + N2) * _esize(Y) + N1 * N2 * 4)
        refs.append(live)
    x3 = any(pr is not None and pr[0].dtype == torch.float32 for pr in probs)
    return "gemm_tn_layer_x3_kernel" if x3 else "gemm_tn_layer_kernel", fl, by, refs


def _work_attn_out_bwd(dy, y, rstd, *a, **k):
    M, d = dy.shape
    return "attn_out_bwd_kernel", 2.0 * M * d * d, 4 * M * d * _esize(dy) + M * 4


def _work_ln_bwd(dy, y, rstd, *a, **k):
    M, N = dy.shape
    return "ln_bwd_kernel", 0.0, 3 * M * N * _esize(dy) + M * 4


def _work_full_ce_fwd(h, w, labels, mask, live, sums, train=True):
    n, d = h.shape
    C = w.shape[0]
    nl = float(mask.sum())
    wgs = -(-int(live[0]) // (8 * (2 if d <= 128 else 1)))
    return ("full_ce_fwd_kernel<%s,%s>" % (_tn(h), "train" if train else "infer"), 2.0 * nl * C * d * (2 if train else 1),
            wgs * C * d * _esize(w) + nl * d * _esize(h) + (n * d * _esize(h) if train else 0) + n * 16)


def _work_full_ce_dw(h, w, labels, mask, live, lse, sums, gout, dw):
    n, d = h.shape
    C = w.shape[0]
    nl = float(mask.sum())
    rows_wg = 16 * 8 * (2 if d <= 128 else 1)
    return ("full_ce_dw_kernel<%s>" % _tn(h), 4.0 * nl * C * d,
            (C / rows_wg + 1) * nl * (d * _esize(h) + 16) + C * d * (_esize(w) + 8))


_WORK = {"full_ce_fwd": _work_full_ce_fwd, "full_ce_dw": _work_full_ce_dw, "attn_out_bwd": _work_attn_out_bwd, "ln_bwd": _work_ln_bwd, "gemm_tn_layer": _work_gemm_tn_layer, "item_loss_scatter_binned": _work_item_loss_scatter, "attn_lastq_x_fwd": _work_lastq_x_fwd, "attn_lastq_x_bwd": _work_lastq_x_bwd, "item_loss_train": _work_item_loss_train,
         "ffn_bwd_data": _work_ffn_bwd, "attn_fwd_x": _work_attn_fwd_x, "post_attn_fwd": _work_post_attn, "gemm_nt": _work_gemm_nt, "gemm_tn": _work_gemm_tn, "attn_fwd": _work_attn_fwd, "attn_bwd": _work_attn_bwd,
         "embed_pe_fwd": _work_embed_fwd, "item_loss_fwd": _work_item_loss, "item_loss_bwd": _work_item_loss}
_PLAIN = ["dropout_", "cross_rows", "adam_multi", "adam_multi_dev", "disc_rows", "item_loss_bwd_binned", "embed_scatter_bwd", "bcast_add_ln", "seq_sum", "colsum", "outer_posmask", "interpolate",
          "gp_penalty", "sum_into", "adam", "cast", "attn_lastq_fwd", "attn_lastq_bwd", "cross_drop_scale", "seq_wsum",
          "embed_scatter_bwd_binned", "scale_dev", "dropout_gelu", "add_drop_ln", "mse", "cross_add_ln"]


def start_profile():
    global _PROF
    import sys
    mod = sys.modules[__name__]
    _PROF = Profiler()

    def wrap(name, fn, work):
        def timed(*a, **k):
            e0 = torch.cuda.Event(enable_timing=True)
            e1 = torch.cuda.Event(enable_timing=True)
            wk = work(*a, **k) if work else (name + "_kernel", 0.0, 0.0)
            kname, fl, by = wk[:3]
            if name in ("item_loss_fwd", "item_loss_bwd"):
                rows = "_rows" if a[0].shape[1] in (64, 128, 256) else ""
                kname = "%s%s_kernel" % (name, rows)
                if name == "item_loss_bwd":
                    fl = fl * 2
            global _PLAN_NAME
            _PLAN_NAME = None
            e0.record()
            out = fn(*a, **k)
            e1.record()
            if _PLAN_NAME is not None:
                kname = _PLAN_NAME
            ref = k.get("live")
            if ref is None:
                ref = k.get("rowmask")
            if ref is None and name == "post_attn_fwd" and len(a) > 12:
                ref = a[12]
                if ref is not None and (a[0].shape[0] < COMPACT_MIN_ROWS or not k.get("compact", True)):
                    ref = None
            if ref is None and name == "ln_bwd" and len(a) > 5 and k.get("live") is None:
                ref = None
            if len(wk) > 3:
                ref = wk[3]
            _PROF.records.append((kname, fl, by, e0, e1, ref))
            return out
        return timed
    for name in list(_WORK) + _PLAIN:
        _ORIG[name] = getattr(mod, name)
        setattr(mod, name, wrap(name, _ORIG[name], _WORK.get(name)))
    return _PROF


def stop_profile():
    global _PROF
    import sys
    mod = sys.modules[__name__]
    for name, fn in _ORIG.items():
        setattr(mod, name, fn)
    _ORIG.clear()
    p, _PROF = _PROF, None
    return p
```

### recguru_amd/ops.py

```python
import weakref

import torch

from . import hip

_COMPUTE = torch.bfloat16
LN_EPS = 1e-8
GP_LAMBDA = 0.1


def set_compute_dtype(dt):
    global _COMPUTE, _MIXED
    _MIXED = dt == "mixed"
    x3 = dt in ("bf16x3", "mixed")
    if x3:
        dt = torch.float32
    elif dt == "bf16":
        dt = torch.bfloat16
    elif dt == "f32":
        dt = torch.float32
    assert dt in (torch.float32, torch.bfloat16)
    _COMPUTE = dt
    hip.SPLIT_OPERANDS = x3
    _SHADOWS.clear()
# ... 97 lines not shown
    key = (tuple(id(p) for p in ps), "bias_cat")
    ver = tuple(_ver(p) for p in ps)
    ent = _SHADOWS.get(key)
    if ent is None or ent[0] != ver or any(r() is not p for r, p in zip(ent[2], ps)):
        ent = (ver, torch.cat([p.detach() for p in ps]), tuple(weakref.ref(p) for p in ps))
        _SHADOWS[key] = ent
    return ent[1]


def pad_rows_cat(ps, H):
    key = (tuple(id(p) for p in ps), _COMPUTE, "pad_rows")
    ver = tuple(_ver(p) for p in ps)
    ent = _SHADOWS.get(key)
    if ent is None or ent[0] != ver or any(r() is not p for r, p in zip(ent[2], ps)):
        b = torch.cat([p.detach().reshape(H, 32) for p in ps] + [torch.zeros(1, 32, device=ps[0].device)], 0)
        ent = (ver, b.to(_COMPUTE).contiguous(), tuple(weakref.ref(p) for p in ps))
        _SHADOWS[key] = ent
    return ent[1]


def refresh_shadows(params):
    import numpy as np
    ids = set(id(p) for p in params)
    todo, dead = [], []
    for key, ent in _SHADOWS.items():
        ps = tuple(r() for r in ent[2])
        if any(p is None for p in ps):
            dead.append(key)
            continue
        if key[-1] in ("bias_cat", "pad_rows"):
            continue
        if key[2] != _COMPUTE or not any(id(p) in ids for p in ps) or ps[0].dim() != 2 or not ps[0].is_cuda:
            continue
        if ent[0] == (_ver(ps[0]) if len(key) == 3 else tuple(_ver(p) for p in ps)):
            continue
        todo.append((key, ps))
    for key in dead:
        del _SHADOWS[key]
    if not todo:
        return
    dev = todo[0][1][0].device
    sig = tuple((key, tuple((p.data_ptr(), tuple(p.shape)) for p in ps)) for key, ps in todo)
    ent = _REFRESH_CACHE.get(sig)
    if ent is None:
        if len(_REFRESH_CACHE) >= 16:
            _REFRESH_CACHE.pop(next(iter(_REFRESH_CACHE)))
        gens = []
        shapes = []
        for _ in range(2):
            segs, outs = [], []
            for key, ps in todo:
                mode = int(key[1])
                transpose = mode & 1
                R = sum(p.shape[0] for p in ps)
                C = ps[0].shape[1]
                dst = torch.empty((C, R) if transpose else (R, C), device=dev, dtype=_COMPUTE)
                outs.append(dst)
                ld = R if transpose else C
                off = 0
                for p in ps:
                    src = p.detach()
                    assert src.is_contiguous() and src.dtype == torch.float32 and src.shape[1] == C
                    segs.append((src.data_ptr(), dst.data_ptr(), p.shape[0], C, ld, 0 if transpose else off,
                                 off if transpose else 0, mode))
                    if not gens:
                        shapes.append((p.shape[0], C))
                    off += p.shape[0]
            host = torch.from_numpy(np.array(segs, dtype=hip.CAST_SEG_DTYPE).view(np.uint8).copy()).pin_memory()
            gens.append((outs, host.to(dev, non_blocking=True), host))
        rows = []
        for i, (r, c) in enumerate(shapes):
            n = ((r + 31) // 32) * ((c + 31) // 32)
            rows.append(np.stack([np.full(n, i, dtype=np.int32), np.arange(n, dtype=np.int32)], 1))
        tiles = torch.from_numpy(np.concatenate(rows, 0)).to(dev)
        ent = _REFRESH_CACHE[sig] = {"gens": gens, "tiles": tiles, "turn": 0, "dtype": _COMPUTE}
    outs, tbl, _ = ent["gens"][ent["turn"]]
    ent["turn"] ^= 1
    hip.cast_multi(tbl, ent["tiles"], ent["tiles"].shape[0], _COMPUTE)
    for (key, ps), dst in zip(todo, outs):
        ver = _ver(ps[0]) if len(key) == 3 else tuple(_ver(p) for p in ps)
        _SHADOWS[key] = (ver, dst, tuple(weakref.ref(p) for p in ps))


_REFRESH_CACHE = {}


_EYES = {}


def _head_eye(H, like):
    key = (H, like.dtype, like.device)
    e = _EYES.get(key)
    if e is None:
        e = _EYES[key] = torch.eye(H, device=like.device, dtype=like.dtype).view(1, H, H, 1)
    return e


def _os_env(name):
    import os
    return os.environ.get(name)


def _z(n, like):
    return torch.zeros(n, device=like.device, dtype=torch.float32)


def _lists_ok():
    return _COMPUTE == torch.bfloat16 or hip.SPLIT_OPERANDS


def _unwritten_qkv_ok():
    return _COMPUTE == torch.bfloat16


def _lists_everywhere(W1, M):
    wide = LISTS_256 and W1.shape[1] == 256 and _COMPUTE == torch.bfloat16
    return _lists_ok() and W1.shape[0] == 512 and (W1.shape[1] == 128 or wide) and M >= max(hip.COMPACT_MIN_ROWS, 8192)


def _live(rowmask, M, shapes_ok=True):
    if rowmask is None or M < max(hip.COMPACT_MIN_ROWS, 8192) or not _lists_ok() or not shapes_ok:
        return None
    return hip.live_tiles(rowmask, M)


def _live_tn(rowmask, M, n1, n2):
    if not TN_LIST_WIDE or n1 % 128 or n2 % 128 or n1 > 1024 or n2 > 1024:
        return None
    return _live(rowmask, M, True)


TN_LIST_WIDE = True
LISTS_256 = not _os_env("RG_NO_LISTS_256")

import os as _os1
TN_PER_LAYER = not _os1.environ.get("RG_NO_TN_LAYER")
import threading as _threading
_TN_TLS = _threading.local()


class _tn_layer(object):
    def __enter__(self):
        self.prev = getattr(_TN_TLS, "batch", None)
        _TN_TLS.batch = [] if TN_PER_LAYER else None
        return self

    def __exit__(self, et, ev, tb):
        batch, _TN_TLS.batch = _TN_TLS.batch, self.prev
        if et is None and batch:
            _flush_tn(batch)


def _flush_tn(batch):
    slots, rest = [None] * 4, []
    for e in batch:
        Y, X, dW, colsum, pro, live = e
        i = hip.gemm_tn_layer_slot(Y, X, pro)
        if i is None or slots[i] is not None:
            rest.append(e)
        else:
            slots[i] = (Y, X, dW, colsum, live)
    if sum(x is not None for x in slots) >= 2 and hip.gemm_tn_layer(slots):
        slots = [None] * 4
    for i, x in enumerate(slots):
        if x is not None:
            hip.gemm_tn(x[0], x[1], x[2], x[3], prologue_x=hip.LAYER_SLOTS[i][2], live=x[4])
    for Y, X, dW, colsum, pro, live in rest:
        hip.gemm_tn(Y, X, dW, colsum, prologue_x=pro, live=live)


def _tn(Y, X, dW, colsum=None, prologue_x=hip.PRO_NONE, live=None):
    batch = getattr(_TN_TLS, "batch", None)
    if batch is None:
        return hip.gemm_tn(Y, X, dW, colsum, prologue_x=prologue_x, live=live)
    batch.append((Y, X, dW, colsum, prologue_x, live))


def _direct(p):
    return p.is_leaf and p.requires_grad and p.dtype == torch.float32


def _adopt(p):
    if p.grad is None:
        buf = getattr(p, "_rg_gbuf", None)
        if buf is None or buf.shape != p.shape:
            buf = torch.zeros(p.shape, device=p.device, dtype=torch.float32)
        elif not getattr(p, "_rg_gclean", False):
            buf.zero_()
        p._rg_gbuf, p._rg_gclean = buf, False
        p.grad = buf
    return p.grad


def _gt(p):
    if _direct(p):
        return _adopt(p), None
    z = torch.zeros(p.shape, device=p.device, dtype=torch.float32)
    return z, z


def _gt_cat(ps):
    rows = [p.shape[0] for p in ps]
    shape = (sum(rows),) + tuple(ps[0].shape[1:])
    if all(_direct(p) for p in ps):
        base = getattr(ps[0], "_rg_gbase", None)
        ok = base is not None and tuple(base.shape) == shape and all(getattr(p, "_rg_gbase", None) is base for p in ps)
        if all(p.grad is None for p in ps):
            if not ok:
                base = torch.zeros(shape, device=ps[0].device, dtype=torch.float32)
            elif not all(getattr(p, "_rg_gclean", False) for p in ps):
                base.zero_()
            off = 0
            for p, r in zip(ps, rows):
                p._rg_gbase, p._rg_gbuf, p._rg_gclean = base, base[off:off + r], False
                p.grad = p._rg_gbuf
                off += r
            return base, [None] * len(ps)
        if ok:
            off, same = 0, True
            for p, r in zip(ps, rows):
                same = same and p.grad is not None and p.grad.data_ptr() == base[off:off + r].data_ptr()
                off += r
            if same:
                return base, [None] * len(ps)
    z = torch.zeros(shape, device=ps[0].device, dtype=torch.float32)
    out, off = [], 0
    for r in rows:
        out.append(z[off:off + r])
        off += r
    return z, out


def release_grads(params):
    bufs = {}
    for p in params:
        g = p.grad
        if g is None:
            continue
        base = getattr(p, "_rg_gbase", None)
        if base is not None and getattr(p, "_rg_gbuf", None) is not None and g.data_ptr() == p._rg_gbuf.data_ptr():
            bufs[id(base)] = base
        else:
            p._rg_gbase = None
            p._rg_gbuf = g if g.dtype == torch.float32 and g.shape == p.shape else None
            if p._rg_gbuf is not None:
                bufs[id(g)] = g
        p._rg_gclean = True
        p.grad = None
    if bufs:
        torch._foreach_zero_(list(bufs.values()))


_SEED = {"base": 0x5EED, "ctr": 0}


def manual_seed(seed, rank=0):
    _SEED["base"] = (int(seed) * 1000003 + int(rank) * 7919 + 1) & 0xFFFFFFFF
    _SEED["ctr"] = 0


def _draw():
    _SEED["ctr"] += 1
    return ((_SEED["base"] << 32) | (_SEED["ctr"] & 0xFFFFFFFF)) & 0x7FFFFFFFFFFFFFFF


def _inv_keep(p):
    return 1.0 / (1.0 - p) if p > 0 else 0.0


_GRAD_MODE = True
_LO_IN = None
_LO_OUT = None
FUSE_QKV_INFERENCE = False
import os as _os
_DEBUG = bool(_os.environ.get("RG_DEBUG"))
_X_MASKED = False


class masked_input(object):

    def __init__(self, on=True):
        self.on = bool(on)

    def __enter__(self):
        global _X_MASKED
        self.prev, _X_MASKED = _X_MASKED, self.on

    def __exit__(self, *a):
        global _X_MASKED
        _X_MASKED = self.prev


class _Fn(torch.autograd.Function):

    @classmethod
    def run(cls, *args):
        global _GRAD_MODE, _LO_IN, _LO_OUT
        prev = (_GRAD_MODE, _LO_IN, _LO_OUT)
        _GRAD_MODE = torch.is_grad_enabled()
        _LO_IN = getattr(args[0], "_rg_lo", None) if (args and torch.is_tensor(args[0]) and _split_resid()) else None
        _LO_OUT = None
        try:
            out = cls.apply(*args)
            if _LO_OUT is not None:
                out._rg_lo = _LO_OUT
            return out
        finally:
            _GRAD_MODE, _LO_IN, _LO_OUT = prev


def _needs_grad(ctx):
    return _GRAD_MODE and any(ctx.needs_input_grad)


class EmbedPE(_Fn):

    @staticmethod
    def forward(ctx, table, pe, ids, mask, skip_row, drop_p):
        B, L = ids.shape
        ids = ids.contiguous()
        mask = mask.reshape(-1).contiguous()
# ... 55 lines not shown
    return _COMPUTE == torch.bfloat16 or (hip.SPLIT_OPERANDS and WS_WIDE_X3)


WS_WIDE_X3 = not _os_env("RG_NO_WS_WIDE_X3")


def _fusable(x2, Wo, W1):
    return hip.post_attn_supported(x2.shape[1], Wo.shape[1], W1.shape[0], x2.dtype, M=x2.shape[0]) and not (x2.shape[1] == 256 and _split_resid())


def _lo_in(x2, rows=None):
    if not _split_resid():
        return None
    lo = _LO_IN
    if lo is None:
        return torch.zeros_like(x2)
    lo = rows(lo) if rows is not None else lo
    return lo.contiguous().view(x2.shape)


def _lo_out(sv, shape):
    global _LO_OUT
    lo = sv.pop("out_lo", None)
    if lo is not None:
        _LO_OUT = lo.view(shape)


QKV_BIAS_ROWS_IN_ATTENTION = True
import os as _os0
QKV_HEAD_MAJOR = not _os0.environ.get("RG_NO_HM")
QKV_HEAD_MAJOR_TRAIN = not _os0.environ.get("RG_NO_HM_TRAIN")
EMBED_SCATTER_BINNED = True
FUSE_ITEM_LOSS_TRAIN = True
FUSE_ATTN_OUT_BWD = True
LASTQ_FROM_X = not _os_env("RG_NO_LASTQ_X")
LASTQ_FOLD_PREFIX = True


def _zero_rows_live(rowmask, M, x_masked, K=128, N=384):
    if not x_masked or rowmask is None or not _lists_ok() or M < max(hip.COMPACT_MIN_ROWS, 4096):
        return None
    if not ((K == 128 and N in (128, 256, 384, 512)) or (K in (256, 384, 512) and N % 128 == 0 and 128 <= N <= 1024)):
        return None
    return hip.live_tiles(rowmask, M)


def _qkv_attn_fwd(x2, B, L, key_ids, pad_value, causal, H, Wq, bq, Wk, bk, Wv, bv, need_grad, drop_p=0.0, seed=0,
                  rowmask=None, x_masked=False, allow_unwritten=False):
    wqkv = shadow_cat((Wq, Wk, Wv))
    bqkv = bias_cat((bq, bk, bv))
    if not need_grad and FUSE_QKV_INFERENCE and hip.attn_fwd_x_supported(x2.shape[1], _COMPUTE, drop_p):
        ctx_ = hip.attn_fwd_x(x2.view(B, L, -1), wqkv, bqkv, key_ids, pad_value, causal, H, drop_p=drop_p, seed=seed,
                              rowmask=rowmask, x_masked=x_masked and rowmask is not None)
        return None, ctx_, None
    live = _zero_rows_live(rowmask, x2.shape[0], x_masked, x2.shape[1], wqkv.shape[0])
    sub = live is not None and QKV_BIAS_ROWS_IN_ATTENTION and allow_unwritten and _unwritten_qkv_ok()
    if (QKV_HEAD_MAJOR and _COMPUTE == torch.bfloat16 and (H, x2.shape[1]) in ((4, 128), (8, 256)) and x2.shape[0] >= 4096
            and 16 <= L <= 416 and (not need_grad or QKV_HEAD_MAJOR_TRAIN)):
        qkv = hip.gemm_nt(x2, wqkv, bqkv, live=live, skip_dead_fill=1 if sub else 2, headmajor_L=L)
        ctx_, lse = hip.attn_fwd(qkv, key_ids, pad_value, causal, H, need_lse=need_grad, drop_p=drop_p, seed=seed, rowmask=rowmask,
                                 x_masked=x_masked, bqkv=bqkv if sub else None, pad_rows=pad_rows_cat((bq, bk, bv), H))
        return qkv, ctx_, lse
    qkv = hip.gemm_nt(x2, wqkv, bqkv, live=live, skip_dead_fill=1 if sub else 2)
    ctx_, lse = hip.attn_fwd(qkv.view(B, L, -1), key_ids, pad_value, causal, H, need_lse=need_grad, drop_p=drop_p, seed=seed,
                             rowmask=rowmask, x_masked=x_masked, bqkv=bqkv if sub else None)
    return qkv, ctx_, lse


def _attn_block_fwd(x2, B, L, key_ids, pad_value, causal, H, Wq, bq, Wk, bk, Wv, bv, Wo, bo, g, be, need_grad,
                    drop_p=0.0, seed=0, rowmask=None, x_masked=False):
    qkv, ctx_, lse = _qkv_attn_fwd(x2, B, L, key_ids, pad_value, causal, H, Wq, bq, Wk, bk, Wv, bv, need_grad, drop_p, seed,
                                   rowmask, x_masked)
    M, d = x2.shape
    P = Wo.shape[1]
    if (WS_PROJ_PLUS_LN and _ws_tier() and M >= 4096 and d % 128 == 0 and P % 128 == 0 and d > 128
            and P // 128 <= 4 and d // 128 <= 8):
        lf = _live(rowmask, M, LISTS_256 and d == 256 and P == 256)
        z = hip.gemm_nt(ctx_.view(B * L, -1), shadow(Wo), bo.detach(), epilogue=hip.EPI_ADD, aux=x2, live=lf)
        y, rstd = hip.bcast_add_ln(z, _zero_row(d, z.device), g.detach(), be.detach(), M, LN_EPS)
        return y, (qkv, ctx_, lse, rstd)
    rstd = torch.empty(x2.shape[0], device=x2.device, dtype=torch.float32)
    y = hip.gemm_nt(ctx_.view(B * L, -1), shadow(Wo), bo.detach(), epilogue=hip.EPI_RESID_LN, aux=x2,
                    gamma=g.detach(), beta=be.detach(), rstd_out=rstd, eps=LN_EPS)
    return y, (qkv, ctx_, lse, rstd)


def _attn_block_bwd(dy, x2, y, saved, B, L, key_ids, pad_value, causal, H, prm, drop_p=0.0, seed=0, rowmask=None,
                    x_masked=False):
    Wq, bq, Wk, bk, Wv, bv, Wo, bo, g, be = prm
    qkv, ctx_, lse, rstd = saved
    d = x2.shape[1]
    P = Wo.shape[1]
    (dg, rg), (dbe, rbe) = _gt(g), _gt(be)
    live = _live(rowmask, dy.shape[0], (d == 128 and P == 128) or (LISTS_256 and d == 256 and P == 256 and _ws_tier()))
    (dWo, rWo), (dbo, rbo) = _gt(Wo), _gt(bo)
    if FUSE_ATTN_OUT_BWD and d == 128 and P == 128:
        dz, dctx = hip.attn_out_bwd(dy, y, rstd, g.detach(), be.detach(), rowmask, dg, dbe,
                                    shadow(Wo, transpose=True, pack=True, split=True), live=live, w_packed=True)
        _tn(dz, ctx_.view(B * L, P), dWo, dbo, live=live)
    else:
        dz = hip.ln_bwd(dy, y, rstd, g.detach(), be.detach(), rowmask, dg, dbe, live=live)
        hip.gemm_tn(dz, ctx_.view(B * L, P), dWo, dbo, live=live if live is not None else _live_tn(rowmask, dz.shape[0], P, d))
        dctx = hip.gemm_nt(dz, shadow(Wo, transpose=True), live=live, skip_dead_fill=True)
    sub = (QKV_BIAS_ROWS_IN_ATTENTION and x_masked == 2 and _unwritten_qkv_ok()
           and _zero_rows_live(rowmask, x2.shape[0], True, d, 3 * P) is not None)
    dqkv = hip.attn_bwd(qkv if qkv.dim() == 5 else qkv.view(B, L, -1), dctx.view(B, L, P), ctx_, lse, key_ids, pad_value, causal, H,
                        drop_p=drop_p, seed=seed, rowmask=rowmask, bqkv=bias_cat((bq, bk, bv)) if sub else None)
    dqkv2 = dqkv.view(B * L, 3 * P)
    (dWqkv, rW), (dbqkv, rb) = _gt_cat((Wq, Wk, Wv)), _gt_cat((bq, bk, bv))
    _tn(dqkv2, x2, dWqkv, dbqkv)
    Wt = shadow_cat((Wq, Wk, Wv), transpose=True)
    if (WS_SPLIT_K_DX and _ws_tier() and dqkv2.shape[0] >= 4096 and 3 * P == 768 and d % 128 == 0
            and 128 < d <= 1024):
        dx = hip.gemm_nt(dqkv2[:, :384], Wt[:, :384], epilogue=hip.EPI_ADD, aux=dz, live=live)
        dx = hip.gemm_nt(dqkv2[:, 384:], Wt[:, 384:], epilogue=hip.EPI_ADD, aux=dx, out=dx, live=live)
    else:
        dx = hip.gemm_nt(dqkv2, Wt, epilogue=hip.EPI_ADD, aux=dz, live=live)
    return dx, (rW[0], rb[0], rW[1], rb[1], rW[2], rb[2], rWo, rbo, rg, rbe)


def _ffn_block_fwd(y, rowmask, W1, b1, W2, b2, g, be, drop_p=0.0, seed_h1=0, seed_out=0):
    M, d = y.shape
    dff = W1.shape[0]
    wide = WS_PROJ_PLUS_LN and _ws_tier() and M >= 4096 and d == 256 and dff % 128 == 0 and dff // 128 <= 4
    if wide and WS_DROP_GELU_EPILOGUE:
        gact = torch.empty(M, dff, device=y.device, dtype=y.dtype)
        h1 = hip.gemm_nt(y, shadow(W1), b1.detach(), epilogue=hip.EPI_DROP_GELU, drop_p=drop_p, drop_seed=seed_h1, out2=gact)
        lf = _live(rowmask, M, LISTS_256 and dff == 512)
        l2 = hip.gemm_nt(gact, shadow(W2), b2.detach(), live=lf)
        out, rstd = hip.add_drop_ln(y, l2, g.detach(), be.detach(), rowmask, drop_p, seed_out, LN_EPS)
        return out, (h1, rstd)
    h1 = hip.gemm_nt(y, shadow(W1), b1.detach())
    if wide:
        gact = hip.dropout_gelu(h1, drop_p, seed_h1)
        l2 = hip.gemm_nt(gact, shadow(W2), b2.detach())
        out, rstd = hip.add_drop_ln(y, l2, g.detach(), be.detach(), rowmask, drop_p, seed_out, LN_EPS)
        return out, (h1, rstd)
    if drop_p > 0:
        hip.dropout_(h1, drop_p, seed_h1)
        l2 = hip.gemm_nt(h1, shadow(W2), b2.detach(), prologue=hip.PRO_GELU, out_f32=True)
        hip.dropout_(l2, drop_p, seed_out)
        out, rstd = hip.bcast_add_ln(y, l2, g.detach(), be.detach(), 1, LN_EPS)
        if rowmask is not None:
            out = out * rowmask.to(out.dtype).unsqueeze(1)
        return out, (h1, rstd)
    rstd = torch.empty(y.shape[0], device=y.device, dtype=torch.float32)
    out = hip.gemm_nt(h1, shadow(W2), b2.detach(), prologue=hip.PRO_GELU, epilogue=hip.EPI_RESID_LN, aux=y,
                      gamma=g.detach(), beta=be.detach(), rowmask=rowmask, rstd_out=rstd, eps=LN_EPS)
    return out, (h1, rstd)


FUSE_FFN_BWD = True
FUSE_FFN_BWD_LN = True


def _ffn_block_bwd(dout, y, out, saved, rowmask, prm, drop_p=0.0, seed_h1=0, seed_out=0):
    W1, b1, W2, b2, g, be = prm
    h1, rstd = saved
    d, dff = W2.shape
    live = _live(rowmask, dout.shape[0], (d == 128 and dff == 512) or (LISTS_256 and d == 256 and dff == 512 and _ws_tier()))
    (dg, rg), (dbe, rbe) = _gt(g), _gt(be)
    (dW2, rW2), (db2, rb2) = _gt(W2), _gt(b2)
    (dW1, rW1), (db1, rb1) = _gt(W1), _gt(b1)
    if FUSE_FFN_BWD and FUSE_FFN_BWD_LN and hip.ffn_bwd_data_supported(d, dff):
        dh1, dy, dl2 = hip.ffn_bwd_data(None, None, h1, shadow(W2, transpose=True, pack=True, split=True), shadow(W1, transpose=True, pack=True, split=True),
                                        nz_scale=_inv_keep(drop_p), live=live, w_packed=True,
                                        ln=(dout, out, rstd, g.detach(), be.detach(), rowmask, dg, dbe, drop_p, seed_out))
        _tn(dl2, h1, dW2, db2, prologue_x=hip.PRO_GELU, live=live)
        _tn(dh1, y, dW1, db1, live=live)
        return dy, (rW1, rb1, rW2, rb2, rg, rbe)
    if drop_p > 0:
        dz, dl2 = hip.ln_bwd(dout, out, rstd, g.detach(), be.detach(), rowmask, dg, dbe, drop_p, seed_out, live=live)
    else:
        dz = dl2 = hip.ln_bwd(dout, out, rstd, g.detach(), be.detach(), rowmask, dg, dbe, live=live)
    live_tn = live if live is not None else _live_tn(rowmask, dout.shape[0], d, dff)
    hip.gemm_tn(dl2, h1, dW2, db2, prologue_x=hip.PRO_GELU, live=live_tn)
    if FUSE_FFN_BWD and hip.ffn_bwd_data_supported(d, dff):
        dh1, dy = hip.ffn_bwd_data(dl2, dz, h1, shadow(W2, transpose=True, pack=True, split=True), shadow(W1, transpose=True, pack=True, split=True),
                                   nz_scale=_inv_keep(drop_p), live=live, w_packed=True)
        hip.gemm_tn(dh1, y, dW1, db1, live=live)
        return dy, (rW1, rb1, rW2, rb2, rg, rbe)
    dh1 = hip.gemm_nt(dl2, shadow(W2, transpose=True), epilogue=hip.EPI_GELU_GRAD, aux=h1,
                      epi_nonzero_scale=_inv_keep(drop_p), live=live, skip_dead_fill=True)
    hip.gemm_tn(dh1, y, dW1, db1, live=live_tn)
    dy = hip.gemm_nt(dh1, shadow(W1, transpose=True), epilogue=hip.EPI_ADD, aux=dz, live=live)
    return dy, (rW1, rb1, rW2, rb2, rg, rbe)


class EncoderLayerFn(_Fn):

    @staticmethod
    def forward(ctx, x, key_ids, rowmask, pad_value, causal, H, drop_p,
                Wq, bq, Wk, bk, Wv, bv, Wo, bo, g1, be1, W1, b1, W2, b2, g2, be2):
        B, L, d = x.shape
        need = _needs_grad(ctx)
        x2 = x.contiguous().view(B * L, d)
        key_ids = key_ids.contiguous()
        rowmask = rowmask.reshape(-1).contiguous()
        seeds = (_draw(), _draw(), _draw()) if drop_p > 0 else (0, 0, 0)
        xm = _X_MASKED
        if _fusable(x2, Wo, W1):
            unw = d == 128
            qkv, ctx_, lse = _qkv_attn_fwd(x2, B, L, key_ids, pad_value, causal, H, Wq, bq, Wk, bk, Wv, bv, need,
                                           drop_p, seeds[0], rowmask, xm, allow_unwritten=unw)
            xm = (2 if xm else 0) if unw else xm
            out, sv = hip.post_attn_fwd(ctx_.view(B * L, -1), x2, shadow(Wo, pack=True, split=True), bo.detach(), g1.detach(), be1.detach(),
                                        shadow(W1, pack=True, split=True), b1.detach(), shadow(W2, pack=True, split=True), b2.detach(), g2.detach(),
                                        be2.detach(),
                                        rowmask, w_packed=True, save=need, eps=LN_EPS, drop_p=drop_p, seed_h1=seeds[1], seed_out=seeds[2],
                                        skip_dead_saves=_lists_everywhere(W1, B * L), x_lo=_lo_in(x2))
            _lo_out(sv, (B, L, d))
            if need:
                y, sa, sf = sv["y"], (qkv, ctx_, lse, sv["rstd1"]), (sv["h1"], sv["rstd2"])
        else:
            y, sa = _attn_block_fwd(x2, B, L, key_ids, pad_value, causal, H, Wq, bq, Wk, bk, Wv, bv, Wo, bo, g1, be1, need,
                                    drop_p, seeds[0], rowmask, xm)
            out, sf = _ffn_block_fwd(y, rowmask, W1, b1, W2, b2, g2, be2, drop_p, seeds[1], seeds[2])
        ctx.mixed = _MIXED
        if need:
            if _MIXED:
                ctx.save_for_backward(_b16(x2), key_ids, rowmask, _b16(y), _b16(out), _b16(sa[0]), _b16(sa[1]), sa[2], sa[3],
                                      _b16(sf[0]), sf[1])
                xm = 1 if xm else 0
            else:
                ctx.save_for_backward(x2, key_ids, rowmask, y, out, *sa, *sf)
            ctx.prm = (Wq, bq, Wk, bk, Wv, bv, Wo, bo, g1, be1, W1, b1, W2, b2, g2, be2)
            ctx.meta = (B, L, pad_value, causal, H, drop_p, seeds, xm)
        return out.view(B, L, d)

    @staticmethod
    def backward(ctx, dout):
        if ctx.mixed:
            with _bf16_backward():
                return EncoderLayerFn._backward(ctx, dout.to(torch.bfloat16))
        return EncoderLayerFn._backward(ctx, dout)

    @staticmethod
    def _backward(ctx, dout):
        x2, key_ids, rowmask, y, out, qkv, ctx_, lse, rstd1, h1, rstd2 = ctx.saved_tensors
        B, L, pad_value, causal, H, drop_p, seeds, xm = ctx.meta
        d = x2.shape[1]
        with _tn_layer():
            dy, gf = _ffn_block_bwd(dout.contiguous().view(B * L, d), y, out, (h1, rstd2), rowmask, ctx.prm[10:],
                                    drop_p, seeds[1], seeds[2])
            dx, ga = _attn_block_bwd(dy, x2, y, (qkv, ctx_, lse, rstd1), B, L, key_ids, pad_value, causal, H,
                                     ctx.prm[:10], drop_p, seeds[0], rowmask, xm)
        return (dx.view(B, L, d), None, None, None, None, None, None) + ga + gf


class EncoderLastLayerFn(_Fn):

    @staticmethod
    def forward(ctx, x, key_ids, rowmask, pad_value, H, drop_p,
                Wq, bq, Wk, bk, Wv, bv, Wo, bo, g1, be1, W1, b1, W2, b2, g2, be2):
        B, L, d = x.shape
        need = _needs_grad(ctx)
        x = x.contiguous()
        x2 = x.view(B * L, d)
        key_ids = key_ids.contiguous()
        rmf = rowmask.reshape(-1).to(torch.float32).contiguous()
        x_last, rm_last = hip.last_rows(x, rmf)
        seeds = (_draw(), _draw(), _draw()) if drop_p > 0 else (0, 0, 0)
        bkv = bias_cat((bk, bv))
        P = Wk.shape[0]
        q_last = hip.gemm_nt(x_last, shadow(Wq), bq.detach())
        fold = bool(_X_MASKED) and LASTQ_FOLD_PREFIX
        from_x = LASTQ_FROM_X and hip.attn_lastq_x_supported(d, P, H, L, x.dtype)
        if from_x:
            wkv = shadow_cat((Wk, Wv))
            kv = None
            c_last = hip.attn_lastq_x_fwd(x, q_last, wkv[:P], wkv[P:], bkv[:P], bkv[P:], key_ids, pad_value, drop_p, seeds[0],
                                          rowmask=rmf if _X_MASKED else None)
        else:
            kv = hip.gemm_nt(x2, shadow_cat((Wk, Wv)), bkv,
                             live=_zero_rows_live(rmf, B * L, _X_MASKED, d, 2 * P), skip_dead_fill=2)
            c_last = hip.attn_lastq_fwd(q_last, kv.view(B, L, -1), key_ids, pad_value, H, drop_p, seeds[0],
                                        rowmask=rmf if fold else None, bkv=bkv if fold else None)
        out_lo = None
        if _fusable(x_last, Wo, W1):
            out, sv = hip.post_attn_fwd(c_last, x_last, shadow(Wo, pack=True, split=True), bo.detach(), g1.detach(), be1.detach(),
                                        shadow(W1, pack=True, split=True), b1.detach(), shadow(W2, pack=True, split=True), b2.detach(), g2.detach(),
                                        be2.detach(),
                                        rm_last, w_packed=True, save=need, eps=LN_EPS, drop_p=drop_p, seed_h1=seeds[1], seed_out=seeds[2],
                                        x_lo=_lo_in(x_last, rows=lambda t: t.reshape(B, L, d)[:, -1, :]))
            out_lo = sv.pop("out_lo", None)
            if need:
                y, rstd1, sf = sv["y"], sv["rstd1"], (sv["h1"], sv["rstd2"])
        else:
            rstd1 = torch.empty(B, device=x.device, dtype=torch.float32)
            y = hip.gemm_nt(c_last, shadow(Wo), bo.detach(), epilogue=hip.EPI_RESID_LN, aux=x_last,
                            gamma=g1.detach(), beta=be1.detach(), rstd_out=rstd1, eps=LN_EPS)
            out, sf = _ffn_block_fwd(y, rm_last, W1, b1, W2, b2, g2, be2, drop_p, seeds[1], seeds[2])
        ctx.mixed = _MIXED
        if need:
            if _MIXED:
                ctx.save_for_backward(_b16(x2), _b16(x_last), key_ids, rm_last, _b16(kv), _b16(q_last), _b16(c_last), _b16(y), _b16(out),
                                      rstd1, _b16(sf[0]), sf[1], rmf)
            else:
                ctx.save_for_backward(x2, x_last, key_ids, rm_last, kv, q_last, c_last, y, out, rstd1, *sf, rmf)
            ctx.prm = (Wq, bq, Wk, bk, Wv, bv, Wo, bo, g1, be1, W1, b1, W2, b2, g2, be2)
            ctx.meta = (B, L, pad_value, H, drop_p, seeds, fold, from_x, bool(_X_MASKED))
        if out_lo is not None:
            return out.to(torch.float32) + out_lo.to(torch.float32)
        return out

    @staticmethod
    def backward(ctx, dout):
        if ctx.mixed:
            with _bf16_backward():
                return EncoderLastLayerFn._backward(ctx, dout.to(torch.bfloat16))
        return EncoderLastLayerFn._backward(ctx, dout)

    @staticmethod
    def _backward(ctx, dout):
        x2, x_last, key_ids, rm_last, kv, q_last, c_last, y, out, rstd1, h1, rstd2, rmf = ctx.saved_tensors
        Wq, bq, Wk, bk, Wv, bv, Wo, bo, g1, be1 = ctx.prm[:10]
        B, L, pad_value, H, drop_p, seeds, fold, from_x, xm = ctx.meta
        d = x2.shape[1]
        P = Wo.shape[1]
        dy, gf = _ffn_block_bwd(dout.to(out.dtype).contiguous(), y, out, (h1, rstd2), rm_last, ctx.prm[10:], drop_p, seeds[1], seeds[2])
# ... 429 lines not shown
```

Measured before the change: 867,500 user-sequences/sec.

## Recompute dh1 inside merged FFN weight-gradient kernel instead of storing it

For bf16 with d_ff=512, the fused FFN backward-data kernel can now skip writing the M x 512 dh1 activation gradient to HBM. A new merged weight-gradient body recomputes dh1 per chunk from dl2, h1 and register-resident W2t via MFMA plus the GELU-grad epilogue, then accumulates dW2 and dW1 (and their bias column sums) in one pass. This trades a large HBM write and read of dh1 for extra matrix work and a more complex, register-heavy kernel with new workgroup partitioning and cost weighting.

```diff
diff --git a/include/recguru_hip.h b/include/recguru_hip.h
--- a/include/recguru_hip.h
+++ b/include/recguru_hip.h
@@ -74,6 +74,9 @@
 int rg_gemm_tn_layer_supported(const rg_gemm_tn_args* p , const int* wgs , int dtype);
 size_t rg_gemm_tn_layer_workspace(int slot, int wgs);
 int rg_gemm_tn_layer(const rg_gemm_tn_args* p , const int* wgs , int dtype, void* stream);
+int rg_gemm_tn_layer_ffn_supported(const rg_gemm_tn_args* p , const int* wgs , int dtype);
+int rg_gemm_tn_layer_ffn(const rg_gemm_tn_args* p , const int* wgs , const void* W2t_packed, float nz_scale,
+                         int dtype, void* stream);
 int rg_gemm_nt_plan(const rg_gemm_nt_args* args , int dtype, char* name, int cap);
 int rg_gemm_tn_plan(const rg_gemm_tn_args* args , int dtype, char* name, int cap);
 
diff --git a/recguru_amd/csrc/fused.hip b/recguru_amd/csrc/fused.hip
--- a/recguru_amd/csrc/fused.hip
+++ b/recguru_amd/csrc/fused.hip
@@ -813,7 +813,7 @@
   return 0;
 }
 
-template <typename T, bool LNF>
+template <typename T, bool LNF, bool ST = true>
 __global__ __launch_bounds__(256, (sizeof(T) == 2 ? 2 : 1)) void ffn_bwd_data_kernel(rg_ffn_bwd_args a) {
   constexpr int PL = FT_M * FD * 2;
   typedef typename LdsT<T, PL>::type LT;
@@ -1003,7 +1003,7 @@
       regs_to_tile<LT>(acc, Adh, n0, li, lg);
       lds_barrier();
       if (ch + 1 < nchunk) h_to_lds();
-      tile_to_hbm<T>(Adh, dh1, a.dff, ch * FD, mb, a.M, tid);
+      if constexpr (ST) tile_to_hbm<T>(Adh, dh1, a.dff, ch * FD, mb, a.M, tid);
       mma_wset<T>(acc2, wq, Adh, li, lg);
     }
     prefetch_rows(mbn);
@@ -1083,20 +1083,21 @@
   if ((long long)a->M * a->dff * (dtype == RG_BF16 ? 2 : 4) >= (1ll << 32))
     return rg_set_error_msg(RG_ERR_UNSUPPORTED, "ffn_bwd_data: M * d_ff * element size must be below 4 GiB (32-bit offsets)");
   const bool lnf = a->ln_dout != nullptr;
-  if ((!lnf && (!a->dl2 || !a->dz)) || !a->h1 || !a->W2t || !a->W1t || !a->dh1 || !a->dy)
-    return rg_set_error_msg(RG_ERR_INVALID, "ffn_bwd_data: NULL operand");
+  const bool nostore = !a->dh1 && lnf && dtype == RG_BF16 && a->dff == 512;
+  if ((!lnf && (!a->dl2 || !a->dz)) || !a->h1 || !a->W2t || !a->W1t || (!a->dh1 && !nostore) || !a->dy)
+    return rg_set_error_msg(RG_ERR_INVALID, "ffn_bwd_data: NULL operand (dh1 may be NULL only for bf16, d_ff = 512, with the fused LayerNorm backward)");
   if (lnf && (!a->ln_out || !a->ln_rstd || !a->ln_gamma || !a->ln_beta || !a->dl2_out || !a->ln_partials))
     return rg_set_error_msg(RG_ERR_INVALID, "ffn_bwd_data: the fused LayerNorm backward needs ln_out, ln_rstd, ln_gamma, ln_beta, dl2_out, ln_partials");
   hipStream_t s = (hipStream_t)stream;
   const int ntiles = (a->M + FT_M - 1) / FT_M;
   const int smem = 4 * act_tile_bytes(dtype, FT_M) + (lnf ? 3 * FD * 4 : 0);
   const int grid = ffn_bwd_grid(a->M, dtype);
-#define RG_FB(T, L)                                                                                                       \
+#define RG_FB(T, ...)                                                                                                     \
   do {                                                                                                                    \
-    hipFuncSetAttribute(reinterpret_cast<const void*>(ffn_bwd_data_kernel<T, L>), hipFuncAttributeMaxDynamicSharedMemorySize, smem); \
-    hipLaunchKernelGGL((ffn_bwd_data_kernel<T, L>), dim3(grid), dim3(256), smem, s, *a);                                  \
+    hipFuncSetAttribute(reinterpret_cast<const void*>(ffn_bwd_data_kernel<T, __VA_ARGS__>), hipFuncAttributeMaxDynamicSharedMemorySize, smem); \
+    hipLaunchKernelGGL((ffn_bwd_data_kernel<T, __VA_ARGS__>), dim3(grid), dim3(256), smem, s, *a);                        \
   } while (0)
-  if (dtype == RG_BF16) { if (lnf) RG_FB(__bf16, true); else RG_FB(__bf16, false); }
+  if (dtype == RG_BF16) { if (nostore) RG_FB(__bf16, true, false); else if (lnf) RG_FB(__bf16, true); else RG_FB(__bf16, false); }
   else if (dtype == RG_F32) { if (lnf) RG_FB(float, true); else RG_FB(float, false); }
   else if (dtype == RG_X3) { if (lnf) RG_FB(x3, true); else RG_FB(x3, false); }
   else return rg_set_error_msg(RG_ERR_INVALID, "ffn_bwd_data: bad dtype");
diff --git a/recguru_amd/csrc/gemm_tn_big.hip b/recguru_amd/csrc/gemm_tn_big.hip
--- a/recguru_amd/csrc/gemm_tn_big.hip
+++ b/recguru_amd/csrc/gemm_tn_big.hip
@@ -408,9 +408,283 @@
   tn_dma_body<N1, N2, GELU_X>(a, (int)blockIdx.x, (int)gridDim.x);
 }
 
+struct TnFfn {
+  static constexpr int CT = 32, HF = 256;
+  static constexpr int YB = CT * 128 * 2, HB = CT * HF * 2, XB = CT * 128 * 2, STG = YB + HB + XB;
+  static constexpr int NPER = STG / 8192, NST = 4;
+  static constexpr int SLD = 36;
+  static constexpr int SCR = CT * SLD * 2;
+  static constexpr int RING = NST * STG + 8 * SCR;
+};
+
+__device__ __forceinline__ void tn_ffn_body(const rg_gemm_tn_args& a, const rg_gemm_tn_args& a1, const void* __restrict__ W2tp, const float nz,
+                                            const int bid, const int nwg) {
+  typedef __bf16 T;
+  typedef TnFfn C;
+  typedef long long i64;
+  typedef __attribute__((ext_vector_type(4))) int i32x4;
+  constexpr int CT = C::CT, NPER = C::NPER, NST = C::NST, STG = C::STG, EPC = CT / 16, YB = C::YB, HB = C::HB;
+  static_assert(NPER == 4 && (NST - 1) * NPER < 64, "ring depth / vmcnt range");
+  extern __shared__ __align__(16) unsigned char smem_td[];
+  const int tid = threadIdx.x, lane = tid & 63, wave = __builtin_amdgcn_readfirstlane(tid >> 6);
+  const int li = lane & 15, lg = lane >> 4;
+  const int hf = bid & 1, rb = bid >> 1, nb = nwg >> 1;
+  const char* __restrict__ Y = reinterpret_cast<const char*>(a.Y);
+  const char* __restrict__ H = reinterpret_cast<const char*>(a.X) + hf * (C::HF * 2);
+  const char* __restrict__ X = reinterpret_cast<const char*>(a1.X);
+  const int nlive = a.live16 ? a.live16[0] : 0;
+  const int nchunks = a.live16 ? (nlive + EPC - 1) / EPC : (a.T + CT - 1) / CT;
+  const int per = (nchunks + nb - 1) / nb;
+  const int c_beg = rb * per, c_end = min(nchunks, c_beg + per);
+  if (c_beg >= c_end) return;
+
+  i32x4 w2[4][2];
+  {
+    const i32x4* wp = reinterpret_cast<const i32x4*>(W2tp);
+#pragma unroll
+    for (int ks = 0; ks < 4; ++ks)
+#pragma unroll
+      for (int ct = 0; ct < 2; ++ct) w2[ks][ct] = wp[(((16 * hf + 2 * wave + ct) * 4 + ks) << 6) + lane];
+#pragma unroll
+    for (int ks = 0; ks < 4; ++ks)
+#pragma unroll
+      for (int ct = 0; ct < 2; ++ct) asm volatile("" : "+v"(w2[ks][ct]));
+  }
+
+  const int r0 = wave * 4 + lg, r1 = wave * 2 + (lane >> 5);
+  const int rl0 = r0 & 15, e0 = wave >> 2;
+  const unsigned int cb0 = (unsigned int)((li ^ ((r0 & 3) << 1)) * 16), cb1 = (unsigned int)(((lane & 31) ^ ((r1 & 3) << 1)) * 16);
+  int* lst = reinterpret_cast<int*>(smem_td + C::RING);
+  if (a.live16) {
+    for (int i = tid; i < EPC * (c_end - c_beg); i += 512) {
+      const int e = EPC * c_beg + i;
+      lst[i] = e < nlive ? a.live16[1 + min(e, nlive - 1)] * 16 : a.T;
+    }
+    __syncthreads();
+  }
+  auto bases = [&](int chunk, int (&bb)[EPC]) {
+    if (a.live16) {
+      const unsigned int ad = (unsigned int)(size_t)(lst + EPC * (chunk - c_beg));
+      i64 v;
+      asm volatile("ds_read_b64 %0, %1\n\ts_waitcnt lgkmcnt(0)" : "=v"(v) : "v"(ad) : "memory");
+      bb[0] = (int)(v & 0xFFFFFFFFll);
+      bb[1] = (int)(v >> 32);
+    } else {
+      bb[0] = chunk * CT;
+      bb[1] = chunk * CT + 16;
+    }
+  };
+  auto issue = [&](int chunk) {
+    int bb[EPC];
+    bases(chunk, bb);
+    unsigned char* stage = smem_td + (chunk % NST) * STG;
+    const int b0 = e0 ? bb[1] : bb[0];
+    const int row0 = min(b0 + rl0, a.T - 1), rowa = min(bb[0] + r1, a.T - 1), rowb = min(bb[1] + r1, a.T - 1);
+#pragma unroll
+    for (int k = 0; k < NPER; ++k) {
+      const char* src = k == 0 ? Y + (size_t)(unsigned int)row0 * ((unsigned int)a.ldy * 2u) + cb0
+                      : k == 3 ? X + (size_t)(unsigned int)row0 * ((unsigned int)a1.ldx * 2u) + cb0
+                               : H + (size_t)(unsigned int)(k == 1 ? rowa : rowb) * ((unsigned int)a.ldx * 2u) + cb1;
+      const int dst = (k == 0 ? 0 : (k == 3 ? YB + HB : YB + (k == 2 ? 8192 : 0))) + wave * 1024;
+      __builtin_amdgcn_global_load_lds((const __attribute__((address_space(1))) void*)src,
+                                       (__attribute__((address_space(3))) void*)(stage + dst), 16, 0, 0);
+    }
+  };
+
+  f32x4 acc2[8][2], acc1[2][8], cs2, cs1[2];
+  cs2 = (f32x4){0.f, 0.f, 0.f, 0.f};
+#pragma unroll
+  for (int i = 0; i < 8; ++i) {
+#pragma unroll
+    for (int j = 0; j < 2; ++j) { acc2[i][j] = (f32x4){0.f, 0.f, 0.f, 0.f}; acc1[j][i] = (f32x4){0.f, 0.f, 0.f, 0.f}; }
+  }
+  cs1[0] = cs1[1] = (f32x4){0.f, 0.f, 0.f, 0.f};
+  const bool do_cs2 = a.colsum != nullptr && hf == 0;
+  const bool do_cs1 = a1.colsum != nullptr;
+  Frag<T> ones;
+  frag_fill(ones, 1.f);
+  const int q = li >> 2, pp = li & 3;
+  const unsigned int smem0 = (unsigned int)(size_t)smem_td;
+  const unsigned int swz = (unsigned int)((li & 3) << 1);
+  const unsigned int t128 = (unsigned int)((8 * lg + q) * 256 + ((pp >> 1) << 4) + (pp & 1) * 8);
+  const unsigned int t256 = (unsigned int)((8 * lg + q) * 512 + ((pp >> 1) << 4) + (pp & 1) * 8) + (unsigned int)YB;
+  auto rd128 = [&](i64& lo, i64& hi, unsigned int img, int ti) {
+    const unsigned int ad = smem0 + img + t128 + (((unsigned int)ti ^ (unsigned int)q) << 5);
+    asm volatile("ds_read_b64_tr_b16 %0, %2\n\tds_read_b64_tr_b16 %1, %2 offset:1024" : "=&v"(lo), "=&v"(hi) : "v"(ad) : "memory");
+  };
+  auto rd256 = [&](i64& lo, i64& hi, unsigned int img, int ti) {
+    const unsigned int ad = smem0 + img + t256 + (((unsigned int)ti ^ (unsigned int)q) << 5);
+    asm volatile("ds_read_b64_tr_b16 %0, %2\n\tds_read_b64_tr_b16 %1, %2 offset:2048" : "=&v"(lo), "=&v"(hi) : "v"(ad) : "memory");
+  };
+  const unsigned int scr0 = smem0 + (unsigned int)(NST * STG + wave * C::SCR);
+  const unsigned int scr_rd = scr0 + (unsigned int)(((8 * lg + q) * C::SLD + 4 * pp) * 2);
+  auto to_frag = [&](Frag<T>& f, i64 lo, i64 hi, bool gelu) {
+    union { i64 l; bf16x4_t b; } u0, u1;
+    u0.l = lo; u1.l = hi;
+#pragma unroll
+    for (int j = 0; j < 4; ++j) {
+      f.v[j] = gelu ? (T)gelu_t<false>((float)u0.b[j]) : u0.b[j];
+      f.v[4 + j] = gelu ? (T)gelu_t<false>((float)u1.b[j]) : u1.b[j];
+    }
+  };
+
+#pragma unroll 1
+  for (int c = c_beg; c < c_end && c < c_beg + NST - 1; ++c) issue(c);
+#pragma unroll 1
+  for (int chunk = c_beg; chunk < c_end; ++chunk) {
+    wait_chunks<NPER, NST - 2>(min(NST - 2, c_end - 1 - chunk));
+    lds_barrier();
+    if (chunk + NST - 1 < c_end) issue(chunk + NST - 1);
+    unsigned char* stage = smem_td + (chunk % NST) * STG;
+    if (chunk == nchunks - 1) {
+      int bb[EPC];
+      bases(chunk, bb);
+      bb[0] = __builtin_amdgcn_readfirstlane(bb[0]);
+      bb[1] = __builtin_amdgcn_readfirstlane(bb[1]);
+      if (bb[0] + 16 > a.T || bb[1] + 16 > a.T) {
+        const int r = tid >> 4;
+        const int row = ((r >> 4) == 1 ? bb[1] : bb[0]) + (r & 15);
+        if (row >= a.T) *reinterpret_cast<uint4*>(stage + tid * 16) = make_uint4(0u, 0u, 0u, 0u);
+        lds_barrier();
+      }
+    }
+    const unsigned int sofs0 = (unsigned int)((chunk % NST) * STG);
+
+    f32x4 dacc[2][2];
+#pragma unroll
+    for (int ct = 0; ct < 2; ++ct)
+#pragma unroll
+      for (int rt = 0; rt < 2; ++rt) dacc[ct][rt] = (f32x4){0.f, 0.f, 0.f, 0.f};
+#pragma unroll
+    for (int ks = 0; ks < 4; ++ks) {
+      i32x4 bf[2];
+#pragma unroll
+      for (int rt = 0; rt < 2; ++rt) {
+        const unsigned int ad = smem0 + sofs0 + (unsigned int)((rt * 16 + li) * 256) + ((((unsigned int)(ks * 4 + lg)) ^ swz) << 4);
+        asm volatile("ds_read_b128 %0, %1" : "=v"(bf[rt]) : "v"(ad) : "memory");
+      }
+      asm volatile("s_waitcnt lgkmcnt(0)" : "+v"(bf[0]), "+v"(bf[1]));
+#pragma unroll
+      for (int rt = 0; rt < 2; ++rt)
+#pragma unroll
+        for (int ct = 0; ct < 2; ++ct) {
+          union { i32x4 i; bf16x8_t b; } ua, ub;
+          ua.i = w2[ks][ct];
+          ub.i = bf[rt];
+          dacc[ct][rt] = __builtin_amdgcn_mfma_f32_16x16x32_bf16(ua.b, ub.b, dacc[ct][rt], 0, 0, 0);
+        }
+    }
+    i64 hx[2][2];
+#pragma unroll
+    for (int ct = 0; ct < 2; ++ct)
+#pragma unroll
+      for (int rt = 0; rt < 2; ++rt) {
+        const unsigned int ad = smem0 + sofs0 + (unsigned int)YB + (unsigned int)((rt * 16 + li) * 512) +
+                                ((((unsigned int)(wave * 4 + ct * 2 + (lg >> 1))) ^ swz) << 4) + (unsigned int)((lg & 1) * 8);
+        asm volatile("ds_read_b64 %0, %1" : "=v"(hx[ct][rt]) : "v"(ad) : "memory");
+      }
+    asm volatile("s_waitcnt lgkmcnt(0)" : "+v"(hx[0][0]), "+v"(hx[0][1]), "+v"(hx[1][0]), "+v"(hx[1][1]));
+#pragma unroll
+    for (int ct = 0; ct < 2; ++ct)
+#pragma unroll
+      for (int rt = 0; rt < 2; ++rt) {
+        union { i64 l; bf16x4_t b; } uh, uo;
+        uh.l = hx[ct][rt];
+#pragma unroll
+        for (int r = 0; r < 4; ++r) {
+          const float x = (float)uh.b[r];
+          float v = dacc[ct][rt][r] * gelu_grad_t<false>(x);
+          if (nz > 0.f) v = x != 0.f ? v * nz : 0.f;
+          uo.b[r] = (T)v;
+        }
+        const unsigned int ad = scr0 + (unsigned int)(((rt * 16 + li) * C::SLD + ct * 16 + 4 * lg) * 2);
+        asm volatile("ds_write_b64 %0, %1" ::"v"(ad), "v"(uo.l) : "memory");
+      }
+
+    {
+      i64 xb[2][2], ya[8][2];
+      rd256(xb[0][0], xb[0][1], sofs0, 2 * wave);
+      rd256(xb[1][0], xb[1][1], sofs0, 2 * wave + 1);
+      rd128(ya[0][0], ya[0][1], sofs0, 0);
+      asm volatile("s_waitcnt lgkmcnt(2)" : "+v"(xb[0][0]), "+v"(xb[0][1]), "+v"(xb[1][0]), "+v"(xb[1][1]));
+      Frag<T> bf[2];
+      to_frag(bf[0], xb[0][0], xb[0][1], true);
+      to_frag(bf[1], xb[1][0], xb[1][1], true);
+#pragma unroll
+      for (int i = 0; i < 8; ++i) {
+        if (i + 1 < 8) {
+          rd128(ya[i + 1][0], ya[i + 1][1], sofs0, i + 1);
+          asm volatile("s_waitcnt lgkmcnt(2)" : "+v"(ya[i][0]), "+v"(ya[i][1]));
+        } else {
+          asm volatile("s_waitcnt lgkmcnt(0)" : "+v"(ya[i][0]), "+v"(ya[i][1]));
+        }
+        Frag<T> af;
+        to_frag(af, ya[i][0], ya[i][1], false);
+        if (do_cs2 && i == wave) mma(af, ones, cs2);
+#pragma unroll
+        for (int j = 0; j < 2; ++j) mma(af, bf[j], acc2[i][j]);
+      }
+    }
+    {
+      i64 da[2][2], xb[8][2];
+      asm volatile("ds_read_b64_tr_b16 %0, %2\n\tds_read_b64_tr_b16 %1, %2 offset:%3" : "=&v"(da[0][0]), "=&v"(da[0][1]) : "v"(scr_rd), "n"(8 * C::SLD) : "memory");
+      asm volatile("ds_read_b64_tr_b16 %0, %2 offset:32\n\tds_read_b64_tr_b16 %1, %2 offset:%3" : "=&v"(da[1][0]), "=&v"(da[1][1]) : "v"(scr_rd), "n"(8 * C::SLD + 32) : "memory");
+      rd128(xb[0][0], xb[0][1], sofs0 + (unsigned int)(YB + HB), 0);
+      Frag<T> af[2];
+#pragma unroll
+      for (int j = 0; j < 8; ++j) {
+        if (j + 1 < 8) {
+          rd128(xb[j + 1][0], xb[j + 1][1], sofs0 + (unsigned int)(YB + HB), j + 1);
+          asm volatile("s_waitcnt lgkmcnt(2)" : "+v"(xb[j][0]), "+v"(xb[j][1]));
+        } else {
+          asm volatile("s_waitcnt lgkmcnt(0)" : "+v"(xb[j][0]), "+v"(xb[j][1]));
+        }
+        if (j == 0) {
+#pragma unroll
+          for (int i = 0; i < 2; ++i) {
+            asm volatile("" : "+v"(da[i][0]), "+v"(da[i][1]));
+            to_frag(af[i], da[i][0], da[i][1], false);
+            if (do_cs1) mma(af[i], ones, cs1[i]);
+          }
+        }
+        Frag<T> bf;
+        to_frag(bf, xb[j][0], xb[j][1], false);
+#pragma unroll
+        for (int i = 0; i < 2; ++i) mma(af[i], bf, acc1[i][j]);
+      }
+    }
+  }
+  const int wo = (4 * hf + (wave >> 1)) * 64 + lane, wh = (wave & 1) * 2;
+  float* __restrict__ p2 = a.partials + (size_t)rb * (128 * 512) + wo;
+  float* __restrict__ p1 = a1.partials + (size_t)rb * (512 * 128) + wo;
+#pragma unroll
+  for (int i = 0; i < 8; ++i)
+#pragma unroll
+    for (int j = 0; j < 2; ++j)
+#pragma unroll
+      for (int r = 0; r < 4; ++r) {
+        p2[((i * 4 + wh + j) * 4 + r) * 512] = acc2[i][j][r];
+        p1[(((wh + j) * 8 + i) * 4 + r) * 512] = acc1[j][i][r];
+      }
+  if (li == 0) {
+    if (do_cs2) {
+#pragma unroll
+      for (int r = 0; r < 4; ++r) rg_acc(a.colsum + wave * 16 + 4 * lg + r, cs2[r] * a.scale);
+    }
+    if (do_cs1) {
+#pragma unroll
+      for (int i = 0; i < 2; ++i)
+#pragma unroll
+        for (int r = 0; r < 4; ++r) rg_acc(a1.colsum + hf * C::HF + wave * 32 + i * 16 + 4 * lg + r, cs1[i][r] * a1.scale);
+    }
+  }
+}
+
 struct rg_tn_layer_args {
   rg_gemm_tn_args p[4];
   int end[4];
+  const void* W2t;
+  float nz;
 };
 __global__ __launch_bounds__(512) void gemm_tn_layer_x3_kernel(rg_tn_layer_args m) {
   const int bid = (int)blockIdx.x;
@@ -421,7 +695,10 @@
 }
 __global__ __launch_bounds__(512) void gemm_tn_layer_kernel(rg_tn_layer_args m) {
   const int bid = (int)blockIdx.x;
-  if (bid < m.end[0]) tn_dma_body<128, 512, true>(m.p[0], bid, m.end[0]);
+  if (bid < m.end[0]) {
+    if (m.W2t) tn_ffn_body(m.p[0], m.p[1], m.W2t, m.nz, bid, m.end[0]);
+    else tn_dma_body<128, 512, true>(m.p[0], bid, m.end[0]);
+  }
   else if (bid < m.end[1]) tn_dma_body<512, 128, false>(m.p[1], bid - m.end[0], m.end[1] - m.end[0]);
   else if (bid < m.end[2]) tn_dma_body<384, 128, false>(m.p[2], bid - m.end[1], m.end[2] - m.end[1]);
   else tn_dma_body<128, 128, false>(m.p[3], bid - m.end[2], m.end[3] - m.end[2]);
@@ -601,46 +878,73 @@
   return layer_ring(i) + (ct / 16) * per * 4;
 }
 
-extern "C" int rg_gemm_tn_layer_supported(const rg_gemm_tn_args* p, const int* wgs, int dtype) {
+static int ffn_ranges(const rg_gemm_tn_args& a, int wg) {
+  const int nchunks = (a.T + TnFfn::CT - 1) / TnFfn::CT, nb = wg / 2;
+  return nb > nchunks ? nchunks : nb;
+}
+static int ffn_lds(const rg_gemm_tn_args& a, int wg) {
+  const int nchunks = (a.T + TnFfn::CT - 1) / TnFfn::CT, nb = ffn_ranges(a, wg);
+  return TnFfn::RING + (TnFfn::CT / 16) * ((nchunks + nb - 1) / nb) * 4;
+}
+
+static int layer_supported(const rg_gemm_tn_args* p, const int* wgs, int dtype, bool ffn) {
   if (!p || !wgs || (dtype != RG_BF16 && dtype != RG_X3) || (dtype == RG_BF16 && !tn_use_dma())) return 0;
   int tot = 0;
+  if (ffn) {
+    const rg_gemm_tn_args &a = p[0], &b = p[1];
+    if (dtype != RG_BF16 || a.T <= 0 || b.T != a.T || b.live16 != a.live16 || wgs[0] < 2 || (wgs[0] & 1) || b.Y) return 0;
+    if ((long long)a.T * a.ldx * 2 >= (1ll << 32)) return 0;
+  }
   for (int i = 0; i < 4; ++i) {
     const rg_gemm_tn_args& a = p[i];
     if (a.T == 0) continue;
     if (a.N1 != LAYER_N1[i] || a.N2 != LAYER_N2[i] || (a.prologue_x == RG_PRO_GELU) != (i == 0)) return 0;
+    if (ffn && i == 1) {
+      if (!a.partials || !a.X || !a.dW || (a.ldx & 7) || !a.use_tr || a.colsum_T > 0) return 0;
+      continue;
+    }
     if (!rg_gemm_tn_big_select(&a, dtype) || !a.partials || !a.Y || !a.X || !a.dW || wgs[i] <= 0) return 0;
-    if (layer_lds(a, i, wgs[i], dtype) > 160 * 1024) return 0;
+    if ((ffn && i == 0 ? ffn_lds(a, wgs[0]) : layer_lds(a, i, wgs[i], dtype)) > 160 * 1024) return 0;
     tot += wgs[i];
   }
   return tot <= 256;
 }
+extern "C" int rg_gemm_tn_layer_supported(const rg_gemm_tn_args* p, const int* wgs, int dtype) { return layer_supported(p, wgs, dtype, false); }
+extern "C" int rg_gemm_tn_layer_ffn_supported(const rg_gemm_tn_args* p, const int* wgs, int dtype) { return layer_supported(p, wgs, dtype, true); }
 
 extern "C" size_t rg_gemm_tn_layer_workspace(int slot, int wgs) { return (size_t)wgs * LAYER_N1[slot] * LAYER_N2[slot] * sizeof(float); }
 
-extern "C" int rg_gemm_tn_layer(const rg_gemm_tn_args* p, const int* wgs, int dtype, void* stream) {
-  if (!rg_gemm_tn_layer_supported(p, wgs, dtype)) return rg_set_error_msg(RG_ERR_UNSUPPORTED, "gemm_tn_layer: needs the bf16 / bf16x3 tier and the four layer "
-                                                                     "shapes (128x512 gelu, 512x128, 384x128, 128x128; T >= 8192; partials)");
+static int layer_launch(const rg_gemm_tn_args* p, const int* wgs, const void* W2t, float nz, int dtype, void* stream) {
+  const bool ffn = W2t != nullptr;
   hipStream_t s = (hipStream_t)stream;
   rg_tn_layer_args m;
   rg_tn_layer_reduce_args r;
+  m.W2t = W2t;
+  m.nz = nz;
   int tot = 0, rtot = 0, smem = 0;
   for (int i = 0; i < 4; ++i) {
     m.p[i] = p[i];
     r.p[i] = p[i];
     const int ct = layer_ct(i, dtype);
     int g = p[i].T > 0 ? wgs[i] : 0;
-    if (p[i].T > 0) {
+    int gr = g;
+    if (ffn && i <= 1) {
+      gr = ffn_ranges(p[0], wgs[0]);
+      g = i == 0 ? 2 * gr : 0;
+      if (i == 0) smem = ffn_lds(p[0], wgs[0]);
+    } else if (p[i].T > 0) {
       const int nchunks = (p[i].T + ct - 1) / ct;
       if (g > nchunks) g = nchunks;
+      gr = g;
       const int need = layer_lds(p[i], i, g, dtype);
       if (need > smem) smem = need;
     }
     tot += g;
     m.end[i] = tot;
-    r.grid1[i] = g;
+    r.grid1[i] = gr;
     r.ct[i] = ct;
     r.gx[i] = LAYER_N1[i] * LAYER_N2[i] / 256;
-    r.gy[i] = g == 0 ? 0 : (r.gx[i] >= 256 ? 4 : (r.gx[i] >= 128 ? 8 : 16));
+    r.gy[i] = gr == 0 ? 0 : (r.gx[i] >= 256 ? 4 : (r.gx[i] >= 128 ? 8 : 16));
     rtot += r.gx[i] * r.gy[i];
     r.end[i] = rtot;
   }
@@ -657,3 +961,16 @@
   RG_CHECK_LAUNCH();
   return 0;
 }
+
+extern "C" int rg_gemm_tn_layer(const rg_gemm_tn_args* p, const int* wgs, int dtype, void* stream) {
+  if (!rg_gemm_tn_layer_supported(p, wgs, dtype)) return rg_set_error_msg(RG_ERR_UNSUPPORTED, "gemm_tn_layer: needs the bf16 / bf16x3 tier and the four layer "
+                                                                     "shapes (128x512 gelu, 512x128, 384x128, 128x128; T >= 8192; partials)");
+  return layer_launch(p, wgs, nullptr, 0.f, dtype, stream);
+}
+
+extern "C" int rg_gemm_tn_layer_ffn(const rg_gemm_tn_args* p, const int* wgs, const void* W2t_packed, float nz_scale, int dtype, void* stream) {
+  if (!W2t_packed || !rg_gemm_tn_layer_ffn_supported(p, wgs, dtype))
+    return rg_set_error_msg(RG_ERR_UNSUPPORTED, "gemm_tn_layer_ffn: needs the bf16 tier, slots 0 and 1 on the same rows and list, p[1].Y == NULL, "
+                                                "an even wgs[0] >= 2, the packed W2^T, partials for both");
+  return layer_launch(p, wgs, W2t_packed, nz_scale, dtype, stream);
+}
diff --git a/recguru_amd/hip.py b/recguru_amd/hip.py
--- a/recguru_amd/hip.py
+++ b/recguru_amd/hip.py
@@ -77,7 +77,7 @@
            "rg_outer_posmask", "rg_interpolate", "rg_gp_penalty", "rg_sum", "rg_adam", "rg_cast",
            "rg_item_loss_fwd", "rg_item_loss_bwd", "rg_post_attn_fwd",
            "rg_attn_lastq_fwd", "rg_attn_lastq_bwd",
-           "rg_cross_drop_scale", "rg_seq_wsum", "rg_gemm_nt_plan", "rg_gemm_tn_plan", "rg_gemm_tn_workspace", "rg_gemm_tn_layer", "rg_gemm_tn_layer_supported", "rg_gemm_tn_layer_workspace", "rg_ln_bwd_workspace", "rg_cast_multi",
+           "rg_cross_drop_scale", "rg_seq_wsum", "rg_gemm_nt_plan", "rg_gemm_tn_plan", "rg_gemm_tn_workspace", "rg_gemm_tn_layer", "rg_gemm_tn_layer_supported", "rg_gemm_tn_layer_ffn", "rg_gemm_tn_layer_ffn_supported", "rg_gemm_tn_layer_workspace", "rg_ln_bwd_workspace", "rg_cast_multi",
            "rg_item_loss_bwd_binned_workspace", "rg_item_loss_bwd_binned", "rg_adam_multi", "rg_rank_scores",
            "rg_assemble_batch", "rg_sample_negatives", "rg_sample_negatives_alias", "rg_dropout", "rg_cross_rows", "rg_live_tiles",
            "rg_adam_multi_dev", "rg_disc_rows", "rg_disc_supported", "rg_attn_fwd_x_supported", "rg_pad_mask", "rg_last_rows",
@@ -399,7 +399,19 @@
     return LAYER_SLOTS.index(key) if (key in LAYER_SLOTS and ok and Y.shape[0] >= 8192) else None
 
 
-def gemm_tn_layer(probs):
+def gemm_tn_layer_ffn_ok(dl2, h1, y, live):
+    if dl2.dtype != torch.bfloat16 or dl2.shape[1] != 128 or h1.shape[1] != 512 or y.shape[1] != 128 or dl2.shape[0] < 8192:
+        return False
+    args = _TnLayerArgs()
+    T = dl2.shape[0]
+    one = ctypes.c_void_p(1)
+    args.p[0] = GemmTnArgs(_p(dl2), _rowmajor(dl2), _p(h1), _rowmajor(h1), one, 512, None, T, 128, 512, PRO_GELU, 1.0, 0, 1, _p(live), one, 0)
+    args.p[1] = GemmTnArgs(None, 512, _p(y), _rowmajor(y), one, 128, None, T, 512, 128, PRO_NONE, 1.0, 0, 1, _p(live), one, 0)
+    cw = (ctypes.c_int * 4)(LAYER_WGS & ~1, 0, 0, 0)
+    return bool(lib().rg_gemm_tn_layer_ffn_supported(ctypes.byref(args), cw, BF16))
+
+
+def gemm_tn_layer(probs, ffn=None):
     args = _TnLayerArgs()
     w = [0.0] * 4
     sc = _DetScope() if DETERMINISTIC else None
@@ -410,16 +422,24 @@
         if sc is not None:
             dW, colsum = sc.take(dW), sc.take(colsum)
         N1, N2, pro = LAYER_SLOTS[i]
+        T = X.shape[0]
+        if ffn is not None and i == 1:
+            assert Y is None and X.shape == (probs[0][0].shape[0], N2) and live is probs[0][4]
+            args.p[i] = GemmTnArgs(None, N1, _p(X), _rowmajor(X), _p(dW), _rowmajor(dW), _p(colsum), T, N1, N2, pro, 1.0, 0, 1, _p(live), None, 0)
+            continue
         assert Y.shape[1] == N1 and X.shape == (Y.shape[0], N2) and Y.dtype == X.dtype
         args.p[i] = GemmTnArgs(_p(Y), _rowmajor(Y), _p(X), _rowmajor(X), _p(dW), _rowmajor(dW), _p(colsum), Y.shape[0], N1, N2,
                                pro, 1.0, 0, 1, _p(live), None, 0)
-        w[i] = Y.shape[0] * (N1 + N2) * (0.6 if live is not None else 1.0) * LAYER_COST[Y.dtype == torch.float32][i]
+        cols, cost = (N1 + N2, LAYER_COST[Y.dtype == torch.float32][i]) if ffn is None or i else (FFN_MERGE_COLS, FFN_MERGE_COST)
+        w[i] = T * cols * (0.6 if live is not None else 1.0) * cost
     tot = sum(w)
     if tot == 0:
         return True
     wgs = [max(8, int(round(LAYER_WGS * x / tot))) if x > 0 else 0 for x in w]
     while sum(wgs) > LAYER_WGS:
         wgs[wgs.index(max(wgs))] -= 1
+    if ffn is not None:
+        return _gemm_tn_layer_ffn(probs, args, wgs, ffn, sc)
     fn = lib().rg_gemm_tn_layer_workspace
     fn.restype = ctypes.c_size_t
     need = [int(fn(i, wgs[i])) for i in range(4)]
@@ -442,6 +462,41 @@
         if sc is not None:
             sc.commit()
     return True
+
+
+FFN_MERGE_COLS = 2 * 128 + 512 + 2 * 128
+FFN_MERGE_COST = float(os.environ.get("RG_TN_FFN_COST", "1.45"))
+
+
+def _gemm_tn_layer_ffn(probs, args, wgs, ffn, sc):
+    W2t, nz = ffn
+    assert W2t.dtype == torch.bfloat16 and W2t.numel() == 512 * 128 and W2t.is_contiguous()
+    fn = lib().rg_gemm_tn_layer_workspace
+    fn.restype = ctypes.c_size_t
+    dev = probs[0][0].device
+    try:
+        for attempt in (0, 1):
+            if attempt:
+                for i in (2, 3):
+                    args.p[i] = GemmTnArgs()
+                wgs = [LAYER_WGS, 0, 0, 0]
+            wgs[0] = max(2, wgs[0] & ~1)
+            wgs[1] = 0
+            need = [int(fn(0, wgs[0] // 2)), int(fn(1, wgs[0] // 2)), int(fn(2, wgs[2])), int(fn(3, wgs[3]))]
+            ws = _tn_workspace(dev, sum(need), "tn_layer")
+            off = 0
+            for i in range(4):
+                if need[i]:
+                    args.p[i].partials = ws.data_ptr() + off
+                    off += need[i]
+            cw = (ctypes.c_int * 4)(*wgs)
+            if sum(wgs) <= LAYER_WGS and lib().rg_gemm_tn_layer_ffn_supported(ctypes.byref(args), cw, BF16):
+                _check(lib().rg_gemm_tn_layer_ffn(ctypes.byref(args), cw, ctypes.c_void_p(_p(W2t)), ctypes.c_float(nz), BF16, _stream()), "rg_gemm_tn_layer_ffn")
+                return attempt == 0
+        raise RuntimeError("recguru_amd: the merged FFN weight-gradient slot was promised (gemm_tn_layer_ffn_ok) and then declined")
+    finally:
+        if sc is not None:
+            sc.commit()
 
 
 def attn_fwd(qkv, key_ids, pad_value, causal, H, need_lse=True, drop_p=0.0, seed=0, rowmask=None, x_masked=False, bqkv=None,
@@ -1172,13 +1227,17 @@
     return bool(lib().rg_ffn_bwd_data_supported(int(d), int(dff)))
 
 
-def ffn_bwd_data(dl2, dz, h1, W2t, W1t, nz_scale=0.0, live=None, w_packed=False, ln=None):
+def ffn_bwd_data(dl2, dz, h1, W2t, W1t, nz_scale=0.0, live=None, w_packed=False, ln=None, store_dh1=True):
     src = ln[0] if ln is not None else dl2
     M, d = src.shape
     dff = h1.shape[1]
-    dh1 = torch.empty(M, dff, device=src.device, dtype=src.dtype)
-    if POISON_UNWRITTEN and live is not None:
-        dh1.fill_(float("nan"))
+    dh1 = None
+    if store_dh1:
+        dh1 = torch.empty(M, dff, device=src.device, dtype=src.dtype)
+        if POISON_UNWRITTEN and live is not None:
+            dh1.fill_(float("nan"))
+    else:
+        assert ln is not None and src.dtype == torch.bfloat16 and dff == 512 and w_packed
     dy = torch.empty(M, d, device=src.device, dtype=src.dtype)
     a = FfnBwdArgs(_p(dl2), _p(dz), _p(h1), _p(W2t), _p(W1t), _p(dh1), _p(dy), M, d, dff, 1 if w_packed else 0,
                    float(nz_scale), _p(live))
@@ -1338,7 +1397,7 @@
     M, d = src.shape
     dff = h1.shape[1]
     return ("ffn_bwd_data_kernel<%s>" % _tn(src), 4.0 * M * d * dff,
-            M * ((4 if k.get("ln") is not None else 3) * d + 2 * dff) * _esize(src))
+            M * ((4 if k.get("ln") is not None else 3) * d + (2 if k.get("store_dh1", True) else 1) * dff) * _esize(src))
 
 
 def _work_lastq_x_fwd(x, q_last, *a, **k):
@@ -1365,17 +1424,24 @@
     return "item_loss_scatter_binned_kernel", 2.0 * pairs * d, pairs * (d * _esize(h) + 2 * 12 + 2 * 8)
 
 
-def _work_gemm_tn_layer(probs):
+def _work_gemm_tn_layer(probs, ffn=None):
     fl, by, refs = [], [], []
     for i, pr in enumerate(probs):
         if pr is None:
             continue
         Y, X, dW, colsum, live = pr
+        if ffn is not None and i <= 1:
+            if i == 0:
+                T = Y.shape[0]
+                fl.append(3 * 2.0 * T * 128 * 512)
+                by.append(T * (128 + 512 + 128) * _esize(Y) + 3 * 128 * 512 * 4 - 128 * 512 * 2)
+                refs.append(live)
+            continue
         T, N1, N2 = Y.shape[0], Y.shape[1], X.shape[1]
         fl.append(2.0 * T * N1 * N2)
         by.append(T * (N1 + N2) * _esize(Y) + N1 * N2 * 4)
         refs.append(live)
-    x3 = any(pr is not None and pr[0].dtype == torch.float32 for pr in probs)
+    x3 = any(pr is not None and pr[1].dtype == torch.float32 for pr in probs)
     return "gemm_tn_layer_x3_kernel" if x3 else "gemm_tn_layer_kernel", fl, by, refs
 
 
diff --git a/recguru_amd/ops.py b/recguru_amd/ops.py
--- a/recguru_amd/ops.py
+++ b/recguru_amd/ops.py
@@ -273,21 +273,44 @@
 
 
 def _flush_tn(batch):
-    slots, rest = [None] * 4, []
+    slots, rest, ffn = [None] * 4, [], None
     for e in batch:
+        if isinstance(e, _FfnPair) and ffn is None:
+            ffn = (e.W2t, e.nz)
+            slots[0], slots[1] = (e.dl2, e.h1, e.dW2, e.db2, e.live), (None, e.y, e.dW1, e.db1, e.live)
+    for e in batch:
+        if isinstance(e, _FfnPair):
+            assert ffn is not None and slots[0][0] is e.dl2, "one merged FFN pair per layer batch"
+            continue
         Y, X, dW, colsum, pro, live = e
         i = hip.gemm_tn_layer_slot(Y, X, pro)
         if i is None or slots[i] is not None:
             rest.append(e)
         else:
             slots[i] = (Y, X, dW, colsum, live)
-    if sum(x is not None for x in slots) >= 2 and hip.gemm_tn_layer(slots):
+    if ffn is not None:
+        if hip.gemm_tn_layer(slots, ffn=ffn):
+            slots = [None] * 4
+        slots[0] = slots[1] = None
+    elif sum(x is not None for x in slots) >= 2 and hip.gemm_tn_layer(slots):
         slots = [None] * 4
     for i, x in enumerate(slots):
         if x is not None:
             hip.gemm_tn(x[0], x[1], x[2], x[3], prologue_x=hip.LAYER_SLOTS[i][2], live=x[4])
     for Y, X, dW, colsum, pro, live in rest:
         hip.gemm_tn(Y, X, dW, colsum, prologue_x=pro, live=live)
+
+
+class _FfnPair(object):
+    def __init__(self, **kw):
+        self.__dict__.update(kw)
+
+
+def _ffn_merge_ok(dl2_like, h1, y, live, W2t):
+    batch = getattr(_TN_TLS, "batch", None)
+    if batch is None or _MIXED or W2t.dtype != torch.bfloat16 or any(isinstance(e, _FfnPair) for e in batch):
+        return False
+    return hip.gemm_tn_layer_ffn_ok(dl2_like, h1, y, live)
 
 
 def _tn(Y, X, dW, colsum=None, prologue_x=hip.PRO_NONE, live=None):
@@ -649,6 +672,7 @@
 
 FUSE_FFN_BWD = True
 FUSE_FFN_BWD_LN = True
+FFN_DW1_RECOMPUTE = True
 
 
 def _ffn_block_bwd(dout, y, out, saved, rowmask, prm, drop_p=0.0, seed_h1=0, seed_out=0):
@@ -660,9 +684,14 @@
     (dW2, rW2), (db2, rb2) = _gt(W2), _gt(b2)
     (dW1, rW1), (db1, rb1) = _gt(W1), _gt(b1)
     if FUSE_FFN_BWD and FUSE_FFN_BWD_LN and hip.ffn_bwd_data_supported(d, dff):
-        dh1, dy, dl2 = hip.ffn_bwd_data(None, None, h1, shadow(W2, transpose=True, pack=True, split=True), shadow(W1, transpose=True, pack=True, split=True),
+        W2t = shadow(W2, transpose=True, pack=True, split=True)
+        merge = FFN_DW1_RECOMPUTE and dff == 512 and _ffn_merge_ok(dout, h1, y, live, W2t)
+        dh1, dy, dl2 = hip.ffn_bwd_data(None, None, h1, W2t, shadow(W1, transpose=True, pack=True, split=True),
                                         nz_scale=_inv_keep(drop_p), live=live, w_packed=True,
-                                        ln=(dout, out, rstd, g.detach(), be.detach(), rowmask, dg, dbe, drop_p, seed_out))
+                                        ln=(dout, out, rstd, g.detach(), be.detach(), rowmask, dg, dbe, drop_p, seed_out), store_dh1=not merge)
+        if merge:
+            _TN_TLS.batch.append(_FfnPair(dl2=dl2, h1=h1, y=y, W2t=W2t, nz=_inv_keep(drop_p), dW2=dW2, db2=db2, dW1=dW1, db1=db1, live=live))
+            return dy, (rW1, rb1, rW2, rb2, rg, rbe)
         _tn(dl2, h1, dW2, db2, prologue_x=hip.PRO_GELU, live=live)
         _tn(dh1, y, dW1, db1, live=live)
         return dy, (rW1, rb1, rW2, rb2, rg, rbe)
```

After: 835,900 user-sequences/sec. 3.6% lower.
